# pbluc/avrecode-ms

Hardware: AMD Instinct MI355X
Metric: H.264 bytes/s recompressed (CABAC re-encode of recorded bin streams, bit-exact vs CPU) (higher is better)
Workload: dtype u32

## Files before the change

avrecode-ms_amd/__init__.py:

```python
from __future__ import annotations

import contextlib
import ctypes
import os
import shutil
import subprocess
import sys
from ctypes import POINTER, c_char_p, c_float, c_int, c_int32, c_size_t, c_uint8, c_uint16, c_uint32, c_uint64, c_void_p

_HERE = os.path.dirname(os.path.abspath(__file__))
_CSRC = os.path.join(_HERE, "csrc")
LIB_PATH = os.path.join(_HERE, "libavrecode_hip.so")
HOOKS_LIB_PATH = os.path.join(_HERE, "libavrecode_hip_hooks.so")
HEADER_PATH = os.path.join(os.path.dirname(_HERE), "include", "avrecode_ms_amd.h")

KIND_CABAC, KIND_RANGE, KIND_CABAC_CODES, KIND_CABAC8 = 0, 1, 2, 3
KIND_RANGE_KEYS, EST_KEYS = 4, 1026
SEL_BYPASS, SEL_TERMINATE = 1024, 1025
SEL8_BYPASS, SEL8_TERMINATE, MAX_STATES8 = 126, 127, 126
SLICE_OK, SLICE_ZERO_PROB, SLICE_OVERFLOW, SLICE_BAD_RECORD = 0, 1, 2, 3
NOP_CABAC, NOP_RANGE = 1026 << 1, 0
CHUNK_BINS, SORT_BLOCK_BINS = 1024, 4096

_SOURCES = ["avr_kernels.hip", "avr_k1p.hip", "avr_k2p.hip", "avr_est.hip", "avr_api.cpp"]
_DEPS = _SOURCES + ["avr_coder.h", "avr_est.h", "avr_div.h", "avr_internal.h", "avr_k1p.h", "avr_k2p.h", "avr_synth.h", "avr_tables.h"]


class AvrError(RuntimeError):
    """Raised for every negative return code of the C ABI (message = avr_last_error())."""


def build_native(force: bool = False, verbose: bool = False) -> str:
    deps = [os.path.join(_CSRC, d) for d in _DEPS] + [HEADER_PATH]
    if not force and os.path.exists(LIB_PATH) and os.path.exists(HOOKS_LIB_PATH):
        if all(min(os.path.getmtime(LIB_PATH), os.path.getmtime(HOOKS_LIB_PATH)) >= os.path.getmtime(d) for d in deps):
            return LIB_PATH
    hipcc = shutil.which("hipcc") or "/opt/rocm/bin/hipcc"
    if not os.path.exists(hipcc):
        if os.path.exists(LIB_PATH):
            return LIB_PATH
        raise AvrError("hipcc not found and no prebuilt libavrecode_hip.so")
    objdir = os.path.join(_HERE, "build")
    os.makedirs(objdir, exist_ok=True)
    flags = ["--offload-arch=gfx950", "-O3", "-std=c++17", "-fPIC", "-Wall"]
    jobs = []
    for variant, extra in (("", []), (".hooks", ["-DAVR_TEST_HOOKS"])):
        for src in _SOURCES:
            obj = os.path.join(objdir, src + variant + ".o")
            jobs.append((obj, [hipcc] + flags + extra + ["-c", "-o", obj, os.path.join(_CSRC, src)]))
    if verbose:
        for _, cmd in jobs:
            print(" ".join(cmd))
    procs = [subprocess.Popen(cmd) for _, cmd in jobs]
    if any(p.wait() != 0 for p in procs):
        raise AvrError("hipcc failed")
    for variant, path in (("", LIB_PATH), (".hooks", HOOKS_LIB_PATH)):
        objs = [os.path.join(objdir, src + variant + ".o") for src in _SOURCES]
        subprocess.run([hipcc, "--offload-arch=gfx950", "-shared", "-fPIC", "-o", path + ".tmp"] + objs, check=True)
        os.replace(path + ".tmp", path)
    return LIB_PATH


RECODE_PATH = os.path.join(_HERE, "recode")
_HOST = os.path.join(_CSRC, "host")


def build_recode(force: bool = False, verbose: bool = False) -> str:
    deps = [os.path.join(_HOST, f) for f in ("recode_main.cpp", "avr_h264.h", "avr_h264_tables.h", "avr_recode.h", "avr_host.h", "avr_model.h")]
    deps += [HEADER_PATH, LIB_PATH]
    if not force and os.path.exists(RECODE_PATH) and all(os.path.getmtime(RECODE_PATH) >= os.path.getmtime(d) for d in deps):
        return RECODE_PATH
    cxx = shutil.which("g++") or shutil.which("hipcc")
    if not cxx:
        if os.path.exists(RECODE_PATH):
            return RECODE_PATH
        raise AvrError("no C++ compiler and no prebuilt recode binary")
    cmd = [cxx, "-O2", "-pthread", "-std=c++17", "-I" + _CSRC, "-I/opt/rocm/include", "-D__HIP_PLATFORM_AMD__", "-o", RECODE_PATH + ".tmp",
           os.path.join(_HOST, "recode_main.cpp"), "-L" + _HERE, "-lavrecode_hip", "-Wl,-rpath,$ORIGIN"]
    if verbose:
        print(" ".join(cmd))
    subprocess.run(cmd, check=True)
    os.replace(RECODE_PATH + ".tmp", RECODE_PATH)
    return RECODE_PATH


class ChunkPlan(ctypes.Structure):
    _fields_ = [("res_off", c_void_p), ("chunk_base", c_void_p), ("chunk_slice", c_void_p), ("blk_base", c_void_p),
                ("blk_slice", c_void_p), ("dig_off", c_void_p), ("res_total", c_uint64), ("dig_total", c_uint64),
                ("total_chunks", c_uint32), ("total_blocks", c_uint32)]


class ChunkedPart(ctypes.Structure):
    _fields_ = [("rec_off", c_void_p), ("n_bins", c_void_p), ("n_slices", c_size_t), ("init_states", c_void_p),
                ("plan", c_void_p), ("workspace", c_void_p), ("workspace_bytes", c_size_t),
                ("out_off", c_void_p), ("out_len", c_void_p), ("status", c_void_p), ("final_states", c_void_p),
                ("rows_hint", c_uint32), ("counts", c_void_p)]


MAX_PARTS = 8


class SynthConfig(ctypes.Structure):
    _fields_ = [("workload", c_int), ("scale_permille", c_uint32), ("seed", c_uint64),
                ("first_slice", c_uint64), ("n_states", c_uint32)]


_lib = None

_u8p, _u16p, _u32p, _u64p, _i32p = (POINTER(c_uint8), POINTER(c_uint16), POINTER(c_uint32),
                                    POINTER(c_uint64), POINTER(c_int32))
SIGNATURES = {
    "avr_last_error": (c_char_p, []),
    "avr_version": (c_char_p, []),
    "avr_device_count": (c_int, []),
    "avr_cabac_lps_range_table": (_u8p, []),
    "avr_cabac_mlps_state_table": (_u8p, []),
    "avr_batch_create": (c_void_p, [c_int, c_size_t, c_size_t]),
    "avr_batch_destroy": (None, [c_void_p]),
    "avr_batch_reset": (c_int, [c_void_p]),
    "avr_batch_add_slice_cabac": (c_int, [c_void_p, c_void_p, c_size_t, c_void_p, c_size_t]),
    "avr_batch_add_slice_range": (c_int, [c_void_p, c_void_p, c_size_t]),
    "avr_batch_add_slice_codes": (c_int, [c_void_p, c_void_p, c_size_t]),
# ... 4 lines not shown
    "avr_range_resolve_workspace_bytes": (c_size_t, [c_size_t, c_size_t, c_void_p]),
    "avr_range_resolve_device": (c_int, [c_int, c_void_p, c_void_p, c_void_p, c_void_p, c_size_t, c_void_p, c_size_t, c_void_p, c_void_p,
                                         c_void_p, c_void_p, c_size_t, c_void_p, c_void_p]),
    "avr_batch_reserve_slice": (c_int, [c_void_p, c_int, c_size_t, c_void_p, c_size_t, POINTER(c_void_p)]),
    "avr_batch_submit": (c_int, [c_void_p]),
    "avr_batch_wait": (c_int, [c_void_p]),
    "avr_batch_run": (c_int, [c_void_p]),
    "avr_batch_get": (c_int, [c_void_p, c_size_t, POINTER(c_void_p), POINTER(c_size_t), POINTER(c_int)]),
    "avr_batch_get_states": (c_int, [c_void_p, c_size_t, POINTER(c_void_p), POINTER(c_size_t)]),
    "avr_batch_timings": (c_int, [c_void_p, POINTER(c_float)]),
    "avr_batch_run_info": (c_int, [c_void_p, POINTER(ctypes.c_uint32)]),
    "avr_multi_create": (c_void_p, [c_void_p, c_size_t, c_size_t, c_size_t]),
    "avr_multi_destroy": (None, [c_void_p]),
    "avr_multi_add_slice_cabac": (c_int, [c_void_p, c_void_p, c_size_t, c_void_p, c_size_t]),
    "avr_multi_add_slice_range": (c_int, [c_void_p, c_void_p, c_size_t]),
    "avr_multi_add_slice_codes": (c_int, [c_void_p, c_void_p, c_size_t]),
    "avr_multi_add_slice_cabac8": (c_int, [c_void_p, c_void_p, c_size_t, c_void_p, c_size_t]),
    "avr_multi_run": (c_int, [c_void_p]),
    "avr_multi_get": (c_int, [c_void_p, c_size_t, POINTER(c_void_p), POINTER(c_size_t), POINTER(c_int)]),
    "avr_multi_placement": (c_int, [c_void_p, c_size_t]),
    "avr_multi_load": (c_int, [c_void_p, c_void_p]),
    "avr_pack_tiles_device": (c_int, [c_int, c_void_p, c_int, c_size_t, c_void_p, c_void_p, c_void_p, c_void_p, c_size_t,
                                      c_void_p, c_void_p, c_void_p]),
    "avr_pack_tiles8_device": (c_int, [c_int, c_void_p, c_size_t, c_void_p, c_void_p, c_void_p, c_void_p, c_size_t,
                                       c_void_p, c_void_p, c_void_p]),
    "avr_cabac_encode_tiles_device": (c_int, [c_int, c_void_p, c_void_p, c_void_p, c_void_p, c_void_p, c_size_t,
                                              c_void_p, c_size_t, c_void_p, c_void_p, c_void_p, c_void_p, c_void_p]),
    "avr_pack_tiles8_narrow_device": (c_int, [c_int, c_void_p, c_size_t, c_void_p, c_void_p, c_void_p, c_void_p, c_size_t,
                                              c_void_p, c_void_p, c_void_p]),
    "avr_cabac8_encode_tiles_device": (c_int, [c_int, c_void_p, c_void_p, c_void_p, c_void_p, c_void_p, c_size_t,
                                               c_void_p, c_size_t, c_void_p, c_void_p, c_void_p, c_void_p, c_void_p]),
    "avr_range_encode_tiles_device": (c_int, [c_int, c_void_p, c_void_p, c_void_p, c_void_p, c_void_p, c_size_t,
                                              c_void_p, c_void_p, c_void_p, c_void_p]),
    "avr_cabac_chunked_workspace_bytes": (c_size_t, [c_size_t, c_size_t, c_void_p]),
    "avr_cabac_encode_chunked_device": (c_int, [c_int, c_void_p, c_void_p, c_void_p, c_void_p, c_size_t, c_void_p, c_size_t,
                                                c_void_p, c_void_p, c_size_t, c_void_p, c_void_p, c_void_p, c_void_p,
                                                c_void_p]),
    "avr_cabac8_chunked_workspace_bytes": (c_size_t, [c_size_t, c_size_t, c_void_p]),
    "avr_cabac8_encode_chunked_device": (c_int, [c_int, c_void_p, c_void_p, c_void_p, c_void_p, c_size_t, c_void_p, c_size_t,
                                                 c_void_p, c_void_p, c_size_t, c_void_p, c_void_p, c_void_p, c_void_p,
                                                 c_void_p]),
    "avr_cabac_encode_chunked_device_hinted": (c_int, [c_int, c_void_p, c_void_p, c_void_p, c_void_p, c_size_t, c_void_p, c_size_t,
                                                       c_void_p, c_void_p, c_size_t, c_void_p, c_void_p, c_void_p, c_void_p,
                                                       c_void_p, c_uint32, c_void_p]),
    "avr_cabac_encode_chunked_second_pass_device": (c_int, [c_int, c_void_p, c_void_p, c_void_p, c_void_p, c_size_t, c_void_p, c_size_t,
                                                            c_void_p, c_void_p, c_size_t, c_void_p, c_void_p, c_void_p, c_void_p,
                                                            c_void_p]),
    "avr_cabac_encode_tiles_device_hinted": (c_int, [c_int, c_void_p, c_void_p, c_void_p, c_void_p, c_void_p, c_size_t,
                                                     c_void_p, c_size_t, c_void_p, c_void_p, c_void_p, c_void_p, c_void_p,
                                                     c_uint32, c_void_p]),
    "avr_cabac_encode_chunked_device_parts": (c_int, [c_int, c_void_p, c_void_p, c_size_t, c_void_p, c_void_p, c_size_t]),
    "avr_range_chunked_workspace_bytes": (c_size_t, [c_size_t, c_void_p, ctypes.c_uint64]),
    "avr_range_encode_chunked_device": (c_int, [c_int, c_void_p, c_void_p, c_void_p, c_void_p, c_size_t, c_void_p, c_void_p, c_size_t,
                                                c_void_p, c_void_p, ctypes.c_uint64, c_void_p, c_void_p]),
    "avr_cabac_resolve_workspace_bytes": (c_size_t, [c_size_t, c_size_t, c_void_p]),
    "avr_cabac_resolve_device": (c_int, [c_int, c_void_p, c_void_p, c_void_p, c_void_p, c_size_t, c_void_p, c_size_t,
                                         c_void_p, c_void_p, c_size_t, c_void_p, c_void_p, c_void_p]),
    "avr_cabac_resolved_workspace_bytes": (c_size_t, [c_size_t, c_void_p]),
    "avr_cabac_encode_resolved_device": (c_int, [c_int, c_void_p, c_void_p, c_void_p, c_size_t, c_void_p, c_void_p, c_size_t,
                                                 c_void_p, c_void_p, c_void_p, c_void_p]),
    "avr_cabac_encode_codes_device": (c_int, [c_int, c_void_p, c_void_p, c_void_p, c_void_p, c_void_p, c_size_t,
                                              c_void_p, c_void_p, c_void_p, c_void_p]),
    "avr_cabac_encode_slices_device": (c_int, [c_int, c_void_p, c_void_p, c_void_p, c_void_p, c_void_p, c_size_t,
                                               c_void_p, c_size_t, c_void_p, c_void_p, c_void_p, c_void_p, c_void_p]),
    "avr_range_encode_slices_device": (c_int, [c_int, c_void_p, c_void_p, c_void_p, c_void_p, c_void_p, c_size_t,
                                               c_void_p, c_void_p, c_void_p, c_void_p]),
# ... 292 lines not shown
```

avrecode-ms_amd/csrc/avr_api.cpp:

```cpp
#include <hip/hip_runtime.h>

#include <algorithm>
#include <cstdarg>
#include <cstdio>
#include <cstdlib>
#include <cstring>
#include <mutex>
#include <new>
#include <numeric>
#include <string>
#include <thread>
#include <vector>

#include "avr_internal.h"
#include "avr_synth.h"
#include "avr_tables.h"

namespace {

thread_local char g_err[512] = "";

int fail(int code, const char *fmt, ...) {
    va_list ap;
    va_start(ap, fmt);
// ... 138 lines not shown
const Env &env() {
    static const Env e = [] {
        Env v{0, false, false};
        if (const char *p = getenv("AVR_K1_PATH")) v.k1_path = strcmp(p, "chunked") == 0 ? 2 : strcmp(p, "serial") == 0 ? 1 : 0;
        v.no_dense = getenv("AVR_NO_DENSE") != nullptr;
        v.no_hint = getenv("AVR_BATCH_NO_HINT") != nullptr;
        return v;
    }();
    return e;
}
#ifdef AVR_TEST_HOOKS
TestHooks &test_hooks() { static TestHooks h{}; return h; }
#endif
}

extern "C" {

#ifdef AVR_TEST_HOOKS
int avr_test_hook_set(const char *name, uint32_t value) {
    avr::TestHooks &h = avr::test_hooks();
    if (!name) return fail(AVR_ERR_INVALID, "null hook name");
    if (!strcmp(name, "k1p_force_retry_every")) h.k1p_force_retry_every = value;
    else if (!strcmp(name, "census_stride")) h.census_stride = value;
    else if (!strcmp(name, "chain_lanes")) h.chain_lanes = value;
    else if (!strcmp(name, "k1_form_ref")) h.k1_form_ref = value;
    else if (!strcmp(name, "k1_emit_lds")) h.k1_emit_lds = value;
    else if (!strcmp(name, "k1_path")) h.k1_path = value;
    else if (!strcmp(name, "no_dense")) h.no_dense = value;
    else if (!strcmp(name, "no_hint")) h.no_hint = value;
    else if (!strcmp(name, "k2p_seg_len")) h.k2p_seg_len = value;
    else if (!strcmp(name, "local_waves")) h.local_waves = value;
    else if (!strcmp(name, "k2p_wave")) h.k2p_wave = value;
    else if (!strcmp(name, "k1p_keep_retry")) h.k1p_keep_retry = value;
    else if (!strcmp(name, "k1_waves")) h.k1_waves = value;
    else if (!strcmp(name, "k1_fwd")) h.k1_fwd = value;
    else if (!strcmp(name, "k1_words8")) h.k1_words8 = value;
    else if (!strcmp(name, "chain_nsegs")) h.chain_nsegs = value;
    else if (!strcmp(name, "chain_whole")) h.chain_whole = value;
    else if (!strcmp(name, "chain_segments")) h.chain_segments = value;
    else if (!strcmp(name, "chain_force_redo")) h.chain_force_redo = value;
    else if (!strcmp(name, "reset")) h = avr::TestHooks{};
    else return fail(AVR_ERR_INVALID, "unknown test hook %s", name);
    return AVR_OK;
}
#endif

const char *avr_last_error(void) { return g_err; }
const char *avr_version(void) { return "avrecode-ms_amd 0.1 (gfx950)"; }

int avr_device_count(void) {
    int n = 0;
    if (hipGetDeviceCount(&n) != hipSuccess) return 0;
    return n;
}

const uint8_t *avr_cabac_lps_range_table(void) { return kTables.lps_range; }
const uint8_t *avr_cabac_mlps_state_table(void) { return kTables.mlps_state; }


avr_batch *avr_batch_create(int device, size_t max_slices, size_t max_bins) {
    if (max_slices == 0 || max_slices > 0x7fffffffu) { fail(AVR_ERR_INVALID, "max_slices out of range"); return nullptr; }
    if (select_device(device) != AVR_OK) return nullptr;
    avr_batch *b = new (std::nothrow) avr_batch;
    if (!b) { fail(AVR_ERR_NOMEM, "out of host memory"); return nullptr; }
    b->device = device;
    b->max_slices = max_slices;
// ... 269 lines not shown
    return AVR_OK;
}

static int submit_impl(avr_batch *b, bool use_hint) {
    const size_t n = b->n_bins.size();
    const uint32_t n32 = uint32_t(n);
    if (b->kind == AVR_KIND_CABAC_CODES) return submit_codes(b, n32);
    const size_t ns = b->n_states;
    const bool cabac = b->kind == AVR_KIND_CABAC;

    std::vector<uint32_t> order;
    std::vector<uint64_t> tile_off;
    std::vector<uint64_t> &out_off = b->out_off;
    out_off.assign(n + 1, 0);
    plan_tiles(b->n_bins, order, tile_off, b->recs8 ? 16 : 8);
    for (size_t i = 0; i < n; i++) out_off[i + 1] = out_off[i] + ((uint64_t(b->n_bins[i]) + 16 + 7) & ~uint64_t(7));
    const uint64_t total_recs = b->rec_off.back(), total_chunks = tile_off.back(), total_out = out_off.back();
    const size_t n_tiles = tile_off.size() - 1;
    bool chunked = n <= 32768 && b->total_bins / n >= 8192;
    if (avr::k1_path()) chunked = avr::k1_path() == 2;
    b->last_path = chunked;

    int rc;
    if ((b->recs8 ? (rc = b->d_recs8.reserve(total_recs + 16)) : (rc = b->d_recs.reserve(total_recs))) || (!chunked && (rc = b->d_tiles.reserve(total_chunks))) ||
        (rc = b->d_rec_off.reserve(n + 1)) || (rc = b->d_tile_off.reserve(n_tiles + 1)) ||
        (rc = b->d_out_off.reserve(n + 1)) || (rc = b->d_dense_off.reserve(n + 1)) ||
        (rc = b->d_n_bins.reserve(n)) || (rc = b->d_order.reserve(n)) || (rc = b->d_out_len.reserve(n)) ||
        (rc = b->d_status.reserve(n)) || (rc = b->d_out.reserve(total_out)) ||
        (rc = b->h_out_len.reserve(n)) || (rc = b->h_status.reserve(n)) || (rc = b->h_ndense.reserve(16)))
        return rc;
    if (cabac && ((rc = b->d_states.reserve(n * std::max<size_t>(ns, 1))) || (rc = b->d_final.reserve(n * std::max<size_t>(ns, 1))) ||
                  (rc = b->h_final.reserve(n * std::max<size_t>(ns, 1)))))
        return rc;
    const size_t n_chunks_max = size_t(b->total_bins / AVR_CHUNK_BINS) + n + 1, n_blks_max = size_t(b->total_bins / AVR_SORT_BLOCK_BINS) + n + 1;
    const size_t n_groups = b->group_first.size();
    if ((rc = b->h_plan.reserve(64 * 16 + (n + 1) * 64 + (n_tiles + 1) * 8 + (chunked ? (n_chunks_max + n_blks_max) * 4 : 0) +
                                (b->keys ? (n_chunks_max + n + n_groups + 3) * 4 + 256 : 0)))) return rc;
    if (b->keys && (rc = b->d_keys.reserve(total_recs))) return rc;

    hipStream_t s = b->stream;
    b->plan_used = 0;
    const avr::DenseHint hint{use_hint ? std::min<uint32_t>(b->dense_hint, uint32_t(ns)) : 0u, b->h_ndense.p, b->h_ndense.p + 1};
    b->hint_used = hint.rows;
    b->h_ndense.p[0] = b->h_ndense.p[1] = 0;
    if (b->recs8) {
        b->hint_used = 0;
        b->h_ndense.p[0] = uint32_t(ns);
    }
    AVR_HIP(hipEventRecord(b->ev[0], s));
    if (b->recs8) AVR_HIP(hipMemcpyAsync(b->d_recs8.p, b->h_recs.p, total_recs, hipMemcpyHostToDevice, s));
    else AVR_HIP(hipMemcpyAsync(b->keys ? b->d_keys.p : b->d_recs.p, b->h_recs.p, total_recs * sizeof(uint16_t), hipMemcpyHostToDevice, s));
    AVR_STAGE(b->d_rec_off.p, b->rec_off.data(), n + 1);
    AVR_STAGE(b->d_out_off.p, out_off.data(), n + 1);
    AVR_STAGE(b->d_n_bins.p, b->n_bins.data(), n);
    if (!chunked) {
        AVR_STAGE(b->d_tile_off.p, tile_off.data(), n_tiles + 1);
        AVR_STAGE(b->d_order.p, order.data(), n);
    }
    if (cabac && ns) AVR_HIP(hipMemcpyAsync(b->d_states.p, b->h_states.p, n * ns, hipMemcpyHostToDevice, s));
    AVR_HIP(hipEventRecord(b->ev[1], s));
    AVR_HIP(hipMemsetAsync(b->d_status.p, 0, n * sizeof(int32_t), s));
    if (b->keys && (rc = resolve_keys(b, n32))) return rc;
    if (chunked && !cabac) {
        std::vector<uint32_t> chunk_base(n + 1, 0), chunk_slice;
        for (size_t i = 0; i < n; i++) {
            const uint32_t nc = uint32_t(std::max<uint64_t>(1, (uint64_t(b->n_bins[i]) + AVR_CHUNK_BINS - 1) / AVR_CHUNK_BINS));
            chunk_base[i + 1] = chunk_base[i] + nc;
            chunk_slice.insert(chunk_slice.end(), nc, uint32_t(i));
        }
        const size_t ws = avr::k2p_workspace_bytes(n, chunk_base.back(), total_out);
        if ((rc = b->d_chunk_base.reserve(n + 1)) || (rc = b->d_chunk_slice.reserve(chunk_slice.size())) || (rc = b->d_workspace.reserve(ws + 256)))
            return rc;
        AVR_STAGE(b->d_chunk_base.p, chunk_base.data(), n + 1);
        AVR_STAGE(b->d_chunk_slice.p, chunk_slice.data(), chunk_slice.size());
        AVR_HIP(hipEventRecord(b->ev[2], s));
        uint8_t *wsp = reinterpret_cast<uint8_t *>((reinterpret_cast<uintptr_t>(b->d_workspace.p) + 255) & ~uintptr_t(255));
        AVR_HIP(avr::launch_k2p(s, b->d_recs.p, b->d_rec_off.p, b->d_n_bins.p, n32, b->d_chunk_base.p, b->d_chunk_slice.p,
                                chunk_base.back(), total_out, wsp, b->d_out.p, b->d_out_off.p, b->d_out_len.p, b->d_status.p));
    } else if (chunked) {
        std::vector<uint64_t> res_off(n + 1, 0), dig_off(n + 1, 0);
        std::vector<uint32_t> chunk_base(n + 1, 0), blk_base(n + 1, 0), chunk_slice, blk_slice;
        for (size_t i = 0; i < n; i++) {
            const uint64_t nb = b->n_bins[i];
            res_off[i + 1] = res_off[i] + ((nb + 15) & ~uint64_t(15)) + 16;
            dig_off[i + 1] = dig_off[i] + nb / 2 + 8;
            const uint32_t nc = uint32_t(std::max<uint64_t>(1, (nb + AVR_CHUNK_BINS - 1) / AVR_CHUNK_BINS));
            const uint32_t nk = uint32_t(std::max<uint64_t>(1, (nb + AVR_SORT_BLOCK_BINS - 1) / AVR_SORT_BLOCK_BINS));
            chunk_base[i + 1] = chunk_base[i] + nc;
            blk_base[i + 1] = blk_base[i] + nk;
            chunk_slice.insert(chunk_slice.end(), nc, uint32_t(i));
            blk_slice.insert(blk_slice.end(), nk, uint32_t(i));
        }
        if ((rc = b->d_res_off.reserve(n + 1)) || (rc = b->d_dig_off.reserve(n + 1)) || (rc = b->d_chunk_base.reserve(n + 1)) ||
            (rc = b->d_blk_base.reserve(n + 1)) || (rc = b->d_chunk_slice.reserve(chunk_slice.size())) ||
            (rc = b->d_blk_slice.reserve(blk_slice.size())))
            return rc;
        avr_chunk_plan plan{b->d_res_off.p, b->d_chunk_base.p, b->d_chunk_slice.p, b->d_blk_base.p, b->d_blk_slice.p, b->d_dig_off.p,
                            res_off.back(), dig_off.back(), chunk_base.back(), blk_base.back()};
        const size_t ws = avr::k1p_workspace_bytes(n, uint32_t(ns), &plan);
        if ((rc = b->d_workspace.reserve(ws + 256))) return rc;
        b->plan = plan;
        AVR_STAGE(b->d_res_off.p, res_off.data(), n + 1);
        AVR_STAGE(b->d_dig_off.p, dig_off.data(), n + 1);
        AVR_STAGE(b->d_chunk_base.p, chunk_base.data(), n + 1);
        AVR_STAGE(b->d_blk_base.p, blk_base.data(), n + 1);
        AVR_STAGE(b->d_chunk_slice.p, chunk_slice.data(), chunk_slice.size());
        AVR_STAGE(b->d_blk_slice.p, blk_slice.data(), blk_slice.size());
        AVR_HIP(hipEventRecord(b->ev[2], s));
        uint8_t *wsp = reinterpret_cast<uint8_t *>((reinterpret_cast<uintptr_t>(b->d_workspace.p) + 255) & ~uintptr_t(255));
        if (b->recs8)
            AVR_HIP(avr::launch_k1p8(s, b->d_recs8.p, b->d_rec_off.p, b->d_n_bins.p, n32, b->d_states.p, uint32_t(ns), &plan, wsp,
                                     b->d_out.p, b->d_out_off.p, b->d_out_len.p, b->d_status.p, b->d_final.p));
        else
            AVR_HIP(avr::launch_k1p(s, b->d_recs.p, b->d_rec_off.p, b->d_n_bins.p, n32, b->d_states.p, uint32_t(ns), &plan, wsp,
                                    b->d_out.p, b->d_out_off.p, b->d_out_len.p, b->d_status.p, b->d_final.p, &hint));
    } else {
        if (b->recs8)
            AVR_HIP(avr::launch_pack_tiles8_narrow(s, uint32_t(ns), b->d_recs8.p, b->d_rec_off.p, b->d_n_bins.p, b->d_order.p, n32,
                                                   b->d_tile_off.p, b->d_tiles.p, b->d_status.p));
        else
            AVR_HIP(avr::launch_pack_tiles(s, b->kind, uint32_t(ns), b->d_recs.p, b->d_rec_off.p, b->d_n_bins.p, b->d_order.p, n32,
                                           b->d_tile_off.p, b->d_tiles.p, b->d_status.p));
        AVR_HIP(hipEventRecord(b->ev[2], s));
        if (b->recs8)
            AVR_HIP(avr::launch_cabac8_encode(s, b->d_tiles.p, b->d_tile_off.p, b->d_n_bins.p, b->d_order.p, n32, b->d_states.p,
                                              uint32_t(ns), b->d_out.p, b->d_out_off.p, b->d_out_len.p, b->d_status.p, b->d_final.p));
        else if (cabac)
            AVR_HIP(avr::launch_cabac_encode(true, s, b->d_tiles.p, b->d_tile_off.p, b->d_n_bins.p, b->d_order.p, n32, b->d_states.p,
                                             uint32_t(ns), b->d_out.p, b->d_out_off.p, b->d_out_len.p, b->d_status.p, b->d_final.p,
                                             AVR_SLICE_OK, true, &hint));
        else
// ... 329 lines not shown
                                   uint8_t *out, const uint64_t *out_off, uint32_t *out_len, int32_t *status, uint8_t *final_states) {
    if (int rc = check_common(tile_off, n_bins, out_off, n_slices)) return rc;
    if (n_states > AVR_MAX_STATES8)
        return fail(AVR_ERR_INVALID, "n_states %zu > %d: one-byte records name at most %d contexts", n_states, AVR_MAX_STATES8, AVR_MAX_STATES8);
    if (n_slices && (!tiles || !out || !out_len || !status || (n_states && !init_states))) return fail(AVR_ERR_INVALID, "null device pointer");
    if (reinterpret_cast<uintptr_t>(tiles) & 15) return fail(AVR_ERR_INVALID, "tiles is not 16-byte aligned");
    if (int rc = select_device(device)) return rc;
    AVR_HIP(avr::launch_cabac8_encode(static_cast<hipStream_t>(stream), tiles, tile_off, n_bins, order, uint32_t(n_slices), init_states,
                                      uint32_t(n_states), out, out_off, out_len, status, final_states));
    return AVR_OK;
}

int avr_cabac_encode_tiles_device(int device, void *stream, const void *tiles, const uint64_t *tile_off, const uint32_t *n_bins,
                                  const uint32_t *order, size_t n_slices, const uint8_t *init_states, size_t n_states,
                                  uint8_t *out, const uint64_t *out_off, uint32_t *out_len, int32_t *status, uint8_t *final_states) {
    if (int rc = check_common(tile_off, n_bins, out_off, n_slices)) return rc;
    if (n_states > AVR_MAX_STATES) return fail(AVR_ERR_INVALID, "n_states %zu > %d", n_states, AVR_MAX_STATES);
    if (int rc = select_device(device)) return rc;
    AVR_HIP(avr::launch_cabac_encode(true, static_cast<hipStream_t>(stream), tiles, tile_off, n_bins, order, uint32_t(n_slices),
                                     init_states, uint32_t(n_states), out, out_off, out_len, status, final_states));
    return AVR_OK;
}

int avr_range_encode_tiles_device(int device, void *stream, const void *tiles, const uint64_t *tile_off, const uint32_t *n_bins,
                                  const uint32_t *order, size_t n_slices, uint8_t *out, const uint64_t *out_off,
                                  uint32_t *out_len, int32_t *status) {
    if (int rc = check_common(tile_off, n_bins, out_off, n_slices)) return rc;
    if (int rc = select_device(device)) return rc;
    AVR_HIP(avr::launch_range_encode(true, static_cast<hipStream_t>(stream), tiles, tile_off, n_bins, order, uint32_t(n_slices),
                                     out, out_off, out_len, status));
    return AVR_OK;
}

size_t avr_cabac_chunked_workspace_bytes(size_t n_slices, size_t n_states, const avr_chunk_plan *plan) {
    if (!plan || n_states > AVR_MAX_STATES) return 0;
    return avr::k1p_workspace_bytes(n_slices, uint32_t(n_states), plan);
}

int avr_cabac_encode_chunked_device(int device, void *stream, const uint16_t *recs, const uint64_t *rec_off, const uint32_t *n_bins,
                                    size_t n_slices, const uint8_t *init_states, size_t n_states, const avr_chunk_plan *plan,
                                    void *workspace, size_t workspace_bytes, uint8_t *out, const uint64_t *out_off,
                                    uint32_t *out_len, int32_t *status, uint8_t *final_states) {
    if (int rc = check_common(rec_off, n_bins, out_off, n_slices)) return rc;
    if (n_states > AVR_MAX_STATES) return fail(AVR_ERR_INVALID, "n_states %zu > %d", n_states, AVR_MAX_STATES);
    if (!plan || (n_slices && (!plan->res_off || !plan->chunk_base || !plan->chunk_slice || !plan->blk_base || !plan->blk_slice ||
                               !plan->dig_off || !workspace || !status)))
        return fail(AVR_ERR_INVALID, "null plan pointer");
    if (workspace_bytes < avr::k1p_workspace_bytes(n_slices, uint32_t(n_states), plan))
        return fail(AVR_ERR_CAPACITY, "workspace of %zu bytes is smaller than avr_cabac_chunked_workspace_bytes()", workspace_bytes);
    if (int rc = select_device(device)) return rc;
    AVR_HIP(avr::launch_k1p(static_cast<hipStream_t>(stream), recs, rec_off, n_bins, uint32_t(n_slices), init_states,
                            uint32_t(n_states), plan, workspace, out, out_off, out_len, status, final_states));
    return AVR_OK;
}

size_t avr_cabac8_chunked_workspace_bytes(size_t n_slices, size_t n_states, const avr_chunk_plan *plan) {
    if (!plan || n_states > AVR_MAX_STATES8) return 0;
    return avr::k1p_workspace_bytes(n_slices, uint32_t(n_states), plan);
}

int avr_cabac8_encode_chunked_device(int device, void *stream, const uint8_t *recs8, const uint64_t *rec_off, const uint32_t *n_bins,
                                     size_t n_slices, const uint8_t *init_states, size_t n_states, const avr_chunk_plan *plan,
                                     void *workspace, size_t workspace_bytes, uint8_t *out, const uint64_t *out_off,
                                     uint32_t *out_len, int32_t *status, uint8_t *final_states) {
    if (int rc = check_common(rec_off, n_bins, out_off, n_slices)) return rc;
    if (int rc = check_recs8(recs8, rec_off, n_states)) return rc;
    if (n_slices && (!recs8 || !out || !out_len || (n_states && !init_states))) return fail(AVR_ERR_INVALID, "null device pointer");
    if (!plan || (n_slices && (!plan->res_off || !plan->chunk_base || !plan->chunk_slice || !plan->dig_off || !workspace || !status)))
        return fail(AVR_ERR_INVALID, "null plan pointer");
    if (workspace_bytes < avr::k1p_workspace_bytes(n_slices, uint32_t(n_states), plan))
        return fail(AVR_ERR_CAPACITY, "workspace of %zu bytes is smaller than avr_cabac8_chunked_workspace_bytes()", workspace_bytes);
    if (int rc = select_device(device)) return rc;
    AVR_HIP(avr::launch_k1p8(static_cast<hipStream_t>(stream), recs8, rec_off, n_bins, uint32_t(n_slices), init_states,
                             uint32_t(n_states), plan, workspace, out, out_off, out_len, status, final_states));
    return AVR_OK;
}

static int check_chunked(const uint64_t *rec_off, const uint32_t *n_bins, const uint64_t *out_off, size_t n_slices, size_t n_states,
                         const avr_chunk_plan *plan, void *workspace, size_t workspace_bytes, const int32_t *status) {
    if (int rc = check_common(rec_off, n_bins, out_off, n_slices)) return rc;
    if (n_states > AVR_MAX_STATES) return fail(AVR_ERR_INVALID, "n_states %zu > %d", n_states, AVR_MAX_STATES);
    if (!plan || (n_slices && (!plan->res_off || !plan->chunk_base || !plan->chunk_slice || !plan->blk_base || !plan->blk_slice ||
                               !plan->dig_off || !workspace || !status)))
        return fail(AVR_ERR_INVALID, "null plan pointer");
    if (workspace_bytes < avr::k1p_workspace_bytes(n_slices, uint32_t(n_states), plan))
        return fail(AVR_ERR_CAPACITY, "workspace of %zu bytes is smaller than avr_cabac_chunked_workspace_bytes()", workspace_bytes);
    return AVR_OK;
}

int avr_cabac_encode_chunked_device_hinted(int device, void *stream, const uint16_t *recs, const uint64_t *rec_off, const uint32_t *n_bins,
                                           size_t n_slices, const uint8_t *init_states, size_t n_states, const avr_chunk_plan *plan,
                                           void *workspace, size_t workspace_bytes, uint8_t *out, const uint64_t *out_off,
                                           uint32_t *out_len, int32_t *status, uint8_t *final_states, uint32_t rows_hint, uint32_t *counts) {
    if (!counts) return fail(AVR_ERR_INVALID, "null counts");
    if (int rc = check_chunked(rec_off, n_bins, out_off, n_slices, n_states, plan, workspace, workspace_bytes, status)) return rc;
    if (int rc = select_device(device)) return rc;
    counts[0] = counts[1] = 0;
    if (n_slices == 0) return AVR_OK;
    const avr::DenseHint hint{std::min<uint32_t>(rows_hint, uint32_t(n_states)), counts, counts + 1};
    AVR_HIP(avr::launch_k1p(static_cast<hipStream_t>(stream), recs, rec_off, n_bins, uint32_t(n_slices), init_states,
                            uint32_t(n_states), plan, workspace, out, out_off, out_len, status, final_states, &hint));
    return AVR_OK;
}

int avr_cabac_encode_chunked_second_pass_device(int device, void *stream, const uint16_t *recs, const uint64_t *rec_off, const uint32_t *n_bins,
                                                size_t n_slices, const uint8_t *init_states, size_t n_states, const avr_chunk_plan *plan,
                                                void *workspace, size_t workspace_bytes, uint8_t *out, const uint64_t *out_off,
                                                uint32_t *out_len, int32_t *status, uint8_t *final_states) {
    if (int rc = check_chunked(rec_off, n_bins, out_off, n_slices, n_states, plan, workspace, workspace_bytes, status)) return rc;
    if (int rc = select_device(device)) return rc;
    if (n_slices == 0) return AVR_OK;
    AVR_HIP(avr::launch_k1p_retry(static_cast<hipStream_t>(stream), recs, rec_off, n_bins, uint32_t(n_slices), init_states,
                                  uint32_t(n_states), plan, workspace, out, out_off, out_len, status, final_states));
    return AVR_OK;
}

int avr_cabac_encode_tiles_device_hinted(int device, void *stream, const void *tiles, const uint64_t *tile_off, const uint32_t *n_bins,
// ... 58 lines not shown

int avr_cabac_encode_chunked_device_parts(int device, void *stream, const uint16_t *recs, size_t n_states, uint8_t *out,
                                          const avr_chunked_part *parts, size_t n_parts) {
    if (!parts || n_parts == 0 || n_parts > AVR_MAX_PARTS) return fail(AVR_ERR_INVALID, "1 .. %d parts", AVR_MAX_PARTS);
    for (size_t i = 0; i < n_parts; i++) {
        const avr_chunked_part &q = parts[i];
        if (!q.counts) return fail(AVR_ERR_INVALID, "part %zu: null counts", i);
        if (int rc = check_chunked(q.rec_off, q.n_bins, q.out_off, q.n_slices, n_states, q.plan, q.workspace, q.workspace_bytes, q.status)) return rc;
    }
    if (int rc = select_device(device)) return rc;
    hipStream_t main = static_cast<hipStream_t>(stream);
    PartStreams *ps = nullptr;
    if (n_parts > 1) {
        AVR_HIP(part_streams(main, &ps));
        AVR_HIP(hipEventRecord(ps->fork, main));
    }
    for (size_t i = 0; i < n_parts; i++) {
        const avr_chunked_part &q = parts[i];
        hipStream_t s = i == 0 ? main : ps->side[i - 1];
        if (i) AVR_HIP(hipStreamWaitEvent(s, ps->fork, 0));
        q.counts[0] = q.counts[1] = 0;
        if (q.n_slices) {
            const avr::DenseHint hint{std::min<uint32_t>(q.rows_hint, uint32_t(n_states)), q.counts, q.counts + 1, uint32_t(n_parts)};
            AVR_HIP(avr::launch_k1p(s, recs, q.rec_off, q.n_bins, uint32_t(q.n_slices), q.init_states, uint32_t(n_states), q.plan,
                                    q.workspace, out, q.out_off, q.out_len, q.status, q.final_states, &hint));
        }
        if (i) AVR_HIP(hipEventRecord(ps->done[i - 1], s));
    }
    for (size_t i = 1; i < n_parts; i++) AVR_HIP(hipStreamWaitEvent(main, ps->done[i - 1], 0));
    return AVR_OK;
}

size_t avr_range_chunked_workspace_bytes(size_t n_slices, const avr_chunk_plan *plan, uint64_t out_total) {
    if (!plan) return 0;
    return avr::k2p_workspace_bytes(n_slices, plan->total_chunks, out_total);
}

int avr_range_encode_chunked_device(int device, void *stream, const uint16_t *recs, const uint64_t *rec_off, const uint32_t *n_bins,
                                    size_t n_slices, const avr_chunk_plan *plan, void *workspace, size_t workspace_bytes,
                                    uint8_t *out, const uint64_t *out_off, uint64_t out_total, uint32_t *out_len, int32_t *status) {
    if (int rc = check_common(rec_off, n_bins, out_off, n_slices)) return rc;
    if (!plan || (n_slices && (!plan->chunk_base || !plan->chunk_slice || !workspace || !status || !out || !out_len)))
        return fail(AVR_ERR_INVALID, "null plan / workspace / output pointer");
    if (workspace_bytes < avr::k2p_workspace_bytes(n_slices, plan->total_chunks, out_total))
        return fail(AVR_ERR_CAPACITY, "workspace of %zu bytes is smaller than avr_range_chunked_workspace_bytes()", workspace_bytes);
    if (int rc = select_device(device)) return rc;
    AVR_HIP(avr::launch_k2p(static_cast<hipStream_t>(stream), recs, rec_off, n_bins, uint32_t(n_slices), plan->chunk_base,
                            plan->chunk_slice, plan->total_chunks, out_total, workspace, out, out_off, out_len, status));
    return AVR_OK;
}

size_t avr_range_resolve_workspace_bytes(size_t n_slices, size_t n_groups, const avr_chunk_plan *plan) {
    if (!plan) return 0;
    return avr::est_workspace_bytes(n_slices, n_groups, plan->total_chunks);
}

int avr_range_resolve_device(int device, void *stream, const uint16_t *keys, const uint64_t *rec_off, const uint32_t *n_bins,
                             size_t n_slices, const uint32_t *group_first, size_t n_groups, const uint8_t *est_in, uint8_t *est_out,
                             const avr_chunk_plan *plan, void *workspace, size_t workspace_bytes, uint16_t *recs_out, int32_t *status) {
    if (int rc = check_common(rec_off, n_bins, keys, n_slices)) return rc;
    if (n_groups > 0x7fffffffu) return fail(AVR_ERR_INVALID, "n_groups out of range");
    if (n_slices && (n_groups == 0 || n_groups > n_slices))
        return fail(AVR_ERR_INVALID, "n_groups %zu: a batch of %zu slices has between 1 and %zu groups", n_groups, n_slices, n_slices);
    if (n_slices && (!group_first || !recs_out || !status)) return fail(AVR_ERR_INVALID, "null device pointer");
    if (!plan || (n_slices && (!plan->chunk_base || !plan->chunk_slice))) return fail(AVR_ERR_INVALID, "null plan pointer");
    if (n_slices && !workspace) return fail(AVR_ERR_INVALID, "null workspace");
    if (workspace_bytes < avr::est_workspace_bytes(n_slices, n_groups, plan->total_chunks))
        return fail(AVR_ERR_INVALID, "workspace of %zu bytes is smaller than avr_range_resolve_workspace_bytes()", workspace_bytes);
    if (n_slices && recs_out == keys) return fail(AVR_ERR_INVALID, "recs_out must not alias keys");
    if ((reinterpret_cast<uintptr_t>(keys) | reinterpret_cast<uintptr_t>(recs_out)) & 15)
        return fail(AVR_ERR_INVALID, "keys / recs_out not 16-byte aligned");
    if ((reinterpret_cast<uintptr_t>(est_in) | reinterpret_cast<uintptr_t>(est_out)) & 1)
        return fail(AVR_ERR_INVALID, "est_in / est_out not 2-byte aligned");
    if (reinterpret_cast<uintptr_t>(workspace) & 255) return fail(AVR_ERR_INVALID, "workspace not 256-byte aligned");
    if (int rc = select_device(device)) return rc;
    AVR_HIP(avr::launch_est_resolve(static_cast<hipStream_t>(stream), keys, rec_off, n_bins, uint32_t(n_slices), group_first,
                                    uint32_t(n_groups), est_in, est_out, plan->chunk_base, plan->chunk_slice, plan->total_chunks,
                                    workspace, recs_out, status));
    return AVR_OK;
}

static int check_plan(const avr_chunk_plan *plan, size_t n_slices, bool need_blocks) {
    if (!plan || (n_slices && (!plan->res_off || !plan->chunk_base || !plan->chunk_slice || !plan->dig_off ||
                               (need_blocks && (!plan->blk_base || !plan->blk_slice)))))
        return fail(AVR_ERR_INVALID, "null plan pointer");
    return AVR_OK;
}

size_t avr_cabac_resolve_workspace_bytes(size_t n_slices, size_t n_states, const avr_chunk_plan *plan) {
    if (!plan || n_states > AVR_MAX_STATES) return 0;
    return avr::k1p_resolve_workspace_bytes(n_slices, uint32_t(n_states), plan);
}

int avr_cabac_resolve_device(int device, void *stream, const uint16_t *recs, const uint64_t *rec_off, const uint32_t *n_bins,
                             size_t n_slices, const uint8_t *init_states, size_t n_states, const avr_chunk_plan *plan,
                             void *workspace, size_t workspace_bytes, uint8_t *codes, int32_t *status, uint8_t *final_states) {
    if (int rc = check_common(rec_off, n_bins, codes, n_slices)) return rc;
    if (n_states > AVR_MAX_STATES) return fail(AVR_ERR_INVALID, "n_states %zu > %d", n_states, AVR_MAX_STATES);
    if (int rc = check_plan(plan, n_slices, true)) return rc;
    if (n_slices && (!workspace || !status)) return fail(AVR_ERR_INVALID, "null workspace / status");
    if (workspace_bytes < avr::k1p_resolve_workspace_bytes(n_slices, uint32_t(n_states), plan))
        return fail(AVR_ERR_CAPACITY, "workspace smaller than avr_cabac_resolve_workspace_bytes()");
    if (int rc = select_device(device)) return rc;
    AVR_HIP(avr::launch_k1p_resolve(static_cast<hipStream_t>(stream), recs, rec_off, n_bins, uint32_t(n_slices), init_states,
                                    uint32_t(n_states), plan, workspace, codes, status, final_states));
    return AVR_OK;
}

size_t avr_cabac_resolved_workspace_bytes(size_t n_slices, const avr_chunk_plan *plan) {
    return plan ? avr::k1p_code_workspace_bytes(n_slices, plan) : 0;
}

int avr_cabac_encode_resolved_device(int device, void *stream, const uint8_t *codes, const uint32_t *n_bins, size_t n_slices,
                                     const avr_chunk_plan *plan, void *workspace, size_t workspace_bytes, uint8_t *out,
                                     const uint64_t *out_off, uint32_t *out_len, int32_t *status) {
    if (int rc = check_common(codes, n_bins, out_off, n_slices)) return rc;
    if (int rc = check_plan(plan, n_slices, false)) return rc;
    if (n_slices && (!workspace || !status)) return fail(AVR_ERR_INVALID, "null workspace / status");
    if (workspace_bytes < avr::k1p_code_workspace_bytes(n_slices, plan))
        return fail(AVR_ERR_CAPACITY, "workspace smaller than avr_cabac_resolved_workspace_bytes()");
    if (int rc = select_device(device)) return rc;
    AVR_HIP(avr::launch_k1p_code(static_cast<hipStream_t>(stream), codes, n_bins, uint32_t(n_slices), plan, workspace, out, out_off,
                                 out_len, status));
    return AVR_OK;
}

int avr_cabac_encode_codes_device(int device, void *stream, const uint8_t *codes, const uint64_t *res_off, const uint32_t *n_bins,
                                  const uint32_t *order, size_t n_slices, uint8_t *out, const uint64_t *out_off,
                                  uint32_t *out_len, int32_t *status) {
    if (int rc = check_common(codes, n_bins, out_off, n_slices)) return rc;
    if (n_slices && (!res_off || !status || !out_len)) return fail(AVR_ERR_INVALID, "null device pointer");
    if (int rc = select_device(device)) return rc;
    AVR_HIP(avr::launch_cabac_encode_codes(static_cast<hipStream_t>(stream), codes, res_off, n_bins, order, uint32_t(n_slices), out,
                                           out_off, out_len, status));
    return AVR_OK;
}

int avr_cabac_encode_slices_device(int device, void *stream, const uint16_t *recs, const uint64_t *rec_off, const uint32_t *n_bins,
                                   const uint32_t *order, size_t n_slices, const uint8_t *init_states, size_t n_states,
                                   uint8_t *out, const uint64_t *out_off, uint32_t *out_len, int32_t *status, uint8_t *final_states) {
    if (int rc = check_common(rec_off, n_bins, out_off, n_slices)) return rc;
    if (n_states > AVR_MAX_STATES) return fail(AVR_ERR_INVALID, "n_states %zu > %d", n_states, AVR_MAX_STATES);
    if (int rc = select_device(device)) return rc;
// ... 132 lines not shown
```

avrecode-ms_amd/csrc/avr_internal.h:

```cpp
#pragma once
#include <hip/hip_runtime.h>
#include <stdint.h>

#include "../../include/avrecode_ms_amd.h"

#define AVR_NOP_CABAC2  (AVR_NOP_CABAC | (AVR_NOP_CABAC << 16))
#define AVR_SLICE_RETRY_SERIAL 100
#define AVR_SLICE_RETRY_CENSUS 101
#define AVR_SLICE_DONE         102

namespace avr {

struct Env { int k1_path; bool no_dense, no_hint; };
const Env &env();
struct TestHooks {
    uint32_t k1p_force_retry_every;
    uint32_t census_stride;
    uint32_t chain_lanes;
    uint32_t k1_form_ref;
    uint32_t k1_emit_lds;
    uint32_t k1_path, no_dense, no_hint;
    uint32_t chain_segments;
    uint32_t chain_whole;
    uint32_t chain_force_redo;
    uint32_t k2p_seg_len;
    uint32_t local_waves;
    uint32_t chain_nsegs;
    uint32_t k1_fwd;
    uint32_t k1_words8;
    uint32_t k1_waves;
    uint32_t k2p_wave;
    uint32_t k1p_keep_retry;
};
#ifdef AVR_TEST_HOOKS
TestHooks &test_hooks();
#else
inline const TestHooks &test_hooks() { static const TestHooks none{}; return none; }
#endif
inline int k1_path() { return test_hooks().k1_path ? int(test_hooks().k1_path) : env().k1_path; }
inline bool no_dense() { return test_hooks().no_dense || env().no_dense; }
inline bool no_hint() { return test_hooks().no_hint || env().no_hint; }

struct DenseHint { uint32_t rows; uint32_t *host_count; uint32_t *host_retry; uint32_t sharing = 0; };

void forget_stream(hipStream_t s);
void forget_part_streams(hipStream_t s);

hipError_t launch_cabac_encode(bool tiled, hipStream_t s, const void *recs, const uint64_t *off,
                               const uint32_t *n_bins, const uint32_t *order, uint32_t n_slices,
                               const uint8_t *init_states, uint32_t n_states, uint8_t *out,
                               const uint64_t *out_off, uint32_t *out_len, int32_t *status,
                               uint8_t *final_states, int32_t want_status = AVR_SLICE_OK, bool dense = true,
                               const DenseHint *hint = nullptr);
hipError_t launch_densemap(hipStream_t s, const uint32_t *used, uint16_t *table, uint16_t *index, uint32_t *n_dense);
hipError_t launch_range_encode(bool tiled, hipStream_t s, const void *recs, const uint64_t *off,
                               const uint32_t *n_bins, const uint32_t *order, uint32_t n_slices,
                               uint8_t *out, const uint64_t *out_off, uint32_t *out_len,
                               int32_t *status);
hipError_t launch_pack_tiles(hipStream_t s, int kind, uint32_t n_states, const uint16_t *recs,
                             const uint64_t *rec_off, const uint32_t *n_bins, const uint32_t *order,
                             uint32_t n_slices, const uint64_t *tile_off, void *tiles, int32_t *status);
hipError_t launch_synth_count(hipStream_t s, int workload, uint32_t scale, uint64_t seed,
                              uint64_t first_slice, int kind, uint32_t n_slices, uint32_t *n_bins);
hipError_t launch_synth_tiles(hipStream_t s, int workload, uint32_t scale, uint64_t seed,
                              uint64_t first_slice, int kind, uint32_t n_slices, const uint32_t *order,
                              const uint64_t *tile_off, void *tiles, uint8_t *init_states,
                              uint32_t n_states);

hipError_t launch_pack_tiles8(hipStream_t s, uint32_t n_states, const uint8_t *recs8, const uint64_t *rec_off, const uint32_t *n_bins,
                              const uint32_t *order, uint32_t n_slices, const uint64_t *tile_off, void *tiles, int32_t *status);
hipError_t launch_pack_tiles8_narrow(hipStream_t s, uint32_t n_states, const uint8_t *recs8, const uint64_t *rec_off, const uint32_t *n_bins,
                                     const uint32_t *order, uint32_t n_slices, const uint64_t *tile_off, void *tiles, int32_t *status);
hipError_t launch_cabac8_encode(hipStream_t s, const void *tiles, const uint64_t *tile_off, const uint32_t *n_bins, const uint32_t *order,
                                uint32_t n_slices, const uint8_t *init_states, uint32_t n_states, uint8_t *out, const uint64_t *out_off,
                                uint32_t *out_len, int32_t *status, uint8_t *final_states);
hipError_t launch_context_census(hipStream_t s, const uint16_t *recs, uint64_t n, uint32_t *bitmap);
hipError_t launch_context_remap(hipStream_t s, uint16_t *recs, uint64_t n, const uint16_t *table);
hipError_t launch_states_permute(hipStream_t s, const uint8_t *src, uint32_t n_src, uint8_t *dst, uint32_t n_dst,
                                 const uint16_t *index, uint32_t n_index, uint64_t n_slices, int scatter);
hipError_t launch_compact(hipStream_t s, const uint8_t *out, const uint64_t *out_off, const uint32_t *out_len,
                          const uint64_t *dense_off, uint32_t n_slices, uint8_t *dense);

size_t k1p_workspace_bytes(size_t n_slices, uint32_t n_states, const avr_chunk_plan *pl);
hipError_t launch_k1p(hipStream_t s, const uint16_t *recs, const uint64_t *rec_off, const uint32_t *n_bins,
                      uint32_t n_slices, const uint8_t *init_states, uint32_t n_states, const avr_chunk_plan *pl,
                      void *workspace, uint8_t *out, const uint64_t *out_off, uint32_t *out_len, int32_t *status,
                      uint8_t *final_states, const DenseHint *hint = nullptr);
hipError_t launch_k1p_retry(hipStream_t s, const uint16_t *recs, const uint64_t *rec_off, const uint32_t *n_bins,
                            uint32_t n_slices, const uint8_t *init_states, uint32_t n_states, const avr_chunk_plan *pl,
                            void *workspace, uint8_t *out, const uint64_t *out_off, uint32_t *out_len, int32_t *status,
                            uint8_t *final_states);
hipError_t launch_k1p8(hipStream_t s, const uint8_t *recs8, const uint64_t *rec_off, const uint32_t *n_bins,
                       uint32_t n_slices, const uint8_t *init_states, uint32_t n_states, const avr_chunk_plan *pl,
                       void *workspace, uint8_t *out, const uint64_t *out_off, uint32_t *out_len, int32_t *status,
                       uint8_t *final_states);
size_t k1p_resolve_workspace_bytes(size_t n_slices, uint32_t n_states, const avr_chunk_plan *pl);
hipError_t launch_k1p_resolve(hipStream_t s, const uint16_t *recs, const uint64_t *rec_off, const uint32_t *n_bins,
                              uint32_t n_slices, const uint8_t *init_states, uint32_t n_states, const avr_chunk_plan *pl,
                              void *workspace, uint8_t *codes, int32_t *status, uint8_t *final_states);
size_t k1p_code_workspace_bytes(size_t n_slices, const avr_chunk_plan *pl);
hipError_t launch_k1p_code(hipStream_t s, const uint8_t *codes, const uint32_t *n_bins, uint32_t n_slices,
                           const avr_chunk_plan *pl, void *workspace, uint8_t *out, const uint64_t *out_off,
                           uint32_t *out_len, int32_t *status);
hipError_t launch_cabac_encode_codes(hipStream_t s, const uint8_t *codes, const uint64_t *res_off, const uint32_t *n_bins,
                                     const uint32_t *order, uint32_t n_slices, uint8_t *out, const uint64_t *out_off,
                                     uint32_t *out_len, int32_t *status, int32_t want_status = AVR_SLICE_OK);
size_t k2p_workspace_bytes(size_t n_slices, uint32_t total_chunks, uint64_t out_total);
hipError_t launch_k2p(hipStream_t s, const uint16_t *recs, const uint64_t *rec_off, const uint32_t *n_bins, uint32_t n_slices,
                      const uint32_t *chunk_base, const uint32_t *chunk_slice, uint32_t total_chunks, uint64_t out_total,
                      void *workspace, uint8_t *out, const uint64_t *out_off, uint32_t *out_len, int32_t *status);
size_t est_workspace_bytes(size_t n_slices, size_t n_groups, uint32_t total_chunks);
hipError_t launch_est_resolve(hipStream_t s, const uint16_t *keys, const uint64_t *rec_off, const uint32_t *n_bins, uint32_t n_slices,
                              const uint32_t *group_first, uint32_t n_groups, const uint8_t *est_in, uint8_t *est_out,
                              const uint32_t *chunk_base, const uint32_t *chunk_slice, uint32_t total_chunks, void *workspace,
                              uint16_t *recs_out, int32_t *status);
// ... 6 lines not shown
```

avrecode-ms_amd/csrc/avr_k1p.h:

```cpp
#pragma once
#include <stdint.h>

#if defined(__HIPCC__)
#define AVR_HD __host__ __device__ inline
#else
#define AVR_HD inline
#endif

namespace avr {
namespace k1p {

#if defined(__HIP_DEVICE_COMPILE__)
#define AVR_PIN2(a, b) asm volatile("" : "+v"(a), "+v"(b))
#else
#define AVR_PIN2(a, b) ((void)0)
#endif

constexpr uint32_t kChunk = 1024;
constexpr uint32_t kNone = 0xffffffffu;
constexpr uint32_t kMaxStretch = 16 * kChunk;
constexpr uint32_t kCodeBypass = 252;
constexpr uint32_t kCodePad = 252;

struct alignas(16) U4 { uint32_t x, y, z, w; };

AVR_HD int clz32(uint32_t x) {
#if defined(__HIP_DEVICE_COMPILE__)
    return __clz(x);
#else
    return x ? __builtin_clz(x) : 32;
#endif
}

AVR_HD uint32_t code_sym(uint32_t c) { return ((c >> 1) ^ c) & 1u; }
AVR_HD bool code_is_bypass(uint32_t c) { return (c >> 1) == 126u; }
AVR_HD bool code_is_boundary(uint32_t c) { return code_sym(c) && !code_is_bypass(c); }
AVR_HD uint32_t code_terminate(uint32_t b) { return 255u - b; }
AVR_HD uint32_t code_context(uint32_t s, uint32_t bin) { return s >= 126 ? 255u - ((bin ^ s) & 1u) : (s << 1) | bin; }

AVR_HD uint32_t post_lps_range(uint32_t row, uint32_t q, uint32_t *shift) {
    const uint32_t rl = (row >> (8 * q)) & 0xffu;
    const uint32_t sh = uint32_t(clz32(rl)) - 23;
    *shift = sh;
    return rl << sh;
}

struct CodeEntry { uint32_t row, meta; };
AVR_HD CodeEntry code_entry(uint32_t c, const uint32_t *rows ) {
    if (code_is_bypass(c)) return CodeEntry{0u, 0x100u | ((c & 1u) << 1)};
    return CodeEntry{rows[c >> 2], code_sym(c) * 3u};
}
// ... 21 lines not shown
    *R = x << sh;
    return sh + (e.meta >> 8);
}

struct alignas(16) CodeEntryC { uint32_t row, side, k, adj; };
AVR_HD CodeEntryC code_entry_c(const CodeEntry &e) {
    const uint32_t sym = e.meta & 1u, adds = (e.meta >> 1) & 1u, byp = e.meta >> 8;
    return CodeEntryC{e.row, sym ? ~0u : 0u, adds ? (byp ? 1u : 2u) : 0u, byp - 23u};
}
AVR_HD uint32_t step_range_c(const CodeEntryC &e, uint32_t *R, uint32_t *v) {
    const uint32_t rl = lps_range(e.row, *R);
    const uint32_t rm = *R - rl;
    const uint32_t x = (rl & e.side) | (rm & ~e.side);
    const uint32_t lz = uint32_t(clz32_nz(x));
    *v = mul24(rm, e.k);
    *R = x << (lz - 23);
    return lz + e.adj;
}


struct Stretch {
    uint32_t first;
    uint32_t end;
    uint32_t t_exit[4];
    uint16_t r_exit[4];
    uint8_t exit_q;
    uint8_t too_long;
    uint8_t pad[2];
};

struct LinearCodes {
    const uint8_t *p;
    AVR_HD U4 load16(uint32_t i) const { return *reinterpret_cast<const U4 *>(p + i); }
    AVR_HD uint32_t byte(uint32_t i) const { return p[i]; }
};

template <class Src, class F>
AVR_HD void for_codes_in(const Src &src, uint32_t from, uint32_t n, F &&f) {
    for (uint32_t base = from & ~15u; base < n; base += 16) {
        const U4 v = src.load16(base);
        uint32_t w0 = v.x, w1 = v.y, w2 = v.z, w3 = v.w;
#if defined(__HIP_DEVICE_COMPILE__)
#pragma unroll 1
#endif
        for (uint32_t k = 0; k < 4; k++) {
            const uint32_t d = w0;
            w0 = w1; w1 = w2; w2 = w3;
            const uint32_t i = base + 4 * k;
            if (i + 0 - from < n - from && f(i + 0, d & 0xffu)) return;
            if (i + 1 - from < n - from && f(i + 1, (d >> 8) & 0xffu)) return;
            if (i + 2 - from < n - from && f(i + 2, (d >> 16) & 0xffu)) return;
            if (i + 3 - from < n - from && f(i + 3, d >> 24)) return;
        }
    }
}
template <class F>
AVR_HD void for_codes(const uint8_t *res, uint32_t from, uint32_t n, F &&f) { for_codes_in(LinearCodes{res}, from, n, f); }

template <class G, class G4>
AVR_HD void for_codes_all(const uint8_t *res, uint32_t from, uint32_t to, G &&g, G4 &&g4) {
    if (from >= to) return;
    auto group16 = [&](const U4 &v) {
        uint32_t w0 = v.x, w1 = v.y, w2 = v.z, w3 = v.w;
#if defined(__HIP_DEVICE_COMPILE__)
#pragma unroll 1
#endif
// ... 1 lines not shown
            const uint32_t d = w0;
            w0 = w1; w1 = w2; w2 = w3;
            g4(d);
        }
    };
    const uint32_t head_end = ((from + 15) & ~15u) < to ? ((from + 15) & ~15u) : to;
    for_codes(res, from, head_end, [&](uint32_t, uint32_t c) { g(c); return false; });
    uint32_t base = head_end;
    for (; (base & 63) && base + 16 <= to; base += 16) group16(*reinterpret_cast<const U4 *>(res + base));
    if (base + 64 <= to) {
        const U4 *p = reinterpret_cast<const U4 *>(res + base);
        U4 v0 = p[0], v1 = p[1], v2 = p[2], v3 = p[3];
        for (; base + 64 <= to; base += 64) {
            const U4 *q = reinterpret_cast<const U4 *>(res + (base + 128 <= to ? base + 64 : base));
            const U4 n0 = q[0], n1 = q[1], n2 = q[2], n3 = q[3];
            group16(v0); group16(v1); group16(v2); group16(v3);
            v0 = n0; v1 = n1; v2 = n2; v3 = n3;
        }
    }
    for (; base + 16 <= to; base += 16) group16(*reinterpret_cast<const U4 *>(res + base));
    if (base < to) for_codes(res, base, to, [&](uint32_t, uint32_t c) { g(c); return false; });
}

AVR_HD void code_entries4(const CodeEntry *codes, uint32_t d, CodeEntry e[4]) {
    e[0] = codes[d & 0xffu]; e[1] = codes[(d >> 8) & 0xffu]; e[2] = codes[(d >> 16) & 0xffu]; e[3] = codes[d >> 24];
    AVR_PIN2(e[0].row, e[0].meta); AVR_PIN2(e[1].row, e[1].meta); AVR_PIN2(e[2].row, e[2].meta); AVR_PIN2(e[3].row, e[3].meta);
}
AVR_HD void code_entries4(const CodeEntryC *codes, uint32_t d, CodeEntryC e[4]) {
    e[0] = codes[d & 0xffu]; e[1] = codes[(d >> 8) & 0xffu]; e[2] = codes[(d >> 16) & 0xffu]; e[3] = codes[d >> 24];
    AVR_PIN2(e[0].row, e[0].side); AVR_PIN2(e[1].row, e[1].side); AVR_PIN2(e[2].row, e[2].side); AVR_PIN2(e[3].row, e[3].side);
}

AVR_HD void b1_stretch(const uint8_t *res, uint32_t n, uint32_t chunk, const CodeEntry *codes, uint32_t max_stretch,
                       Stretch *o) {
    const uint32_t lo = chunk * kChunk, limit = lo + kChunk;
    uint32_t R[4], T[4] = {0, 0, 0, 0};
    uint32_t i;
    o->too_long = 0;
    o->exit_q = 0;
    o->pad[0] = o->pad[1] = 0;
    if (chunk == 0) {
        o->first = 0;
        R[0] = R[1] = R[2] = R[3] = 510;
        i = 0;
    } else {
        uint32_t f = kNone;
        const uint32_t hi = limit < n ? limit : n;
        for_codes(res, lo, hi, [&](uint32_t idx, uint32_t c) { if (code_is_boundary(c)) { f = idx; return true; } return false; });
        if (f == kNone) {
            o->first = kNone; o->end = 0;
            for (int q = 0; q < 4; q++) { o->t_exit[q] = 0; o->r_exit[q] = 0; }
            return;
        }
        o->first = f;
        const uint32_t row = codes[res[f]].row;
        for (uint32_t q = 0; q < 4; q++) { uint32_t sh; R[q] = post_lps_range(row, q, &sh); }
        i = f + 1;
    }
    bool closed = false;
    auto merged = [&]() { return R[0] == R[1] && R[1] == R[2] && R[2] == R[3]; };
    auto code_by_code = [&](uint32_t stop) {
        if (i >= stop) return;
        uint32_t i_next = stop;
        for_codes(res, i, stop, [&](uint32_t idx, uint32_t c) {
            if (merged()) { i_next = idx; return true; }
            const bool closing = idx >= limit && code_is_boundary(c);
            if (closing)
                for (uint32_t q = 0; q < 4; q++) o->exit_q |= uint8_t(((R[q] >> 6) & 3) << (2 * q));
// ... 115 lines not shown
    };
    auto digits = [&]() {
        while (sp >= 15) {
            const uint32_t d = uint32_t(L2 >> (sp + 1));
            L2 &= (uint64_t(2) << sp) - 1;
            put(d);
            sp -= 16;
        }
    };
    auto digits2 = [&]() {
        const int s1 = sp + 1;
        const uint32_t nd = uint32_t(s1 > 0 ? s1 : 0) >> 4, ks = 16 + (uint32_t(s1) & 15u);
        const uint64_t t = L2 >> ks;
        const uint32_t a = nd == 2 ? uint32_t(t >> 16) : uint32_t(t), b = uint32_t(t) & 0xffffu;
        L2 = uint32_t(L2) & (nd ? (1u << ks) - 1 : ~0u);
        sp -= int(16 * nd);
        if constexpr (staged) { S.push2(nd, a, b); j += nd; S.look(g0 + j); }
        else { if (nd) put(a); if (nd == 2) put(b); }
    };
    const uint32_t to = st.end;
    if (from < to) {
        auto four = [&](uint32_t d) {
            CodeEntryC e[4];
            code_entries4(codes, d, e);
            bin_e(e[0]); bin_e(e[1]); bin_e(e[2]); bin_e(e[3]);
            digits2();
        };
        auto group16 = [&](const U4 &v) { four(v.x); four(v.y); four(v.z); four(v.w); };
        const uint32_t head_end = ((from + 15) & ~15u) < to ? ((from + 15) & ~15u) : to;
        for_codes_in(src, from, head_end, [&](uint32_t, uint32_t c) { bin(c); digits(); return false; });
        uint32_t base = head_end;
        for (; (base & 63) && base + 16 <= to; base += 16) group16(src.load16(base));
        U4 v0{0, 0, 0, 0}, v1 = v0, v2 = v0, v3 = v0;
        if (base + 64 <= to) { v0 = src.load16(base); v1 = src.load16(base + 16); v2 = src.load16(base + 32); v3 = src.load16(base + 48); }
        for (; base + 64 <= to; base += 64) {
            const uint32_t w[16] = {v0.x, v0.y, v0.z, v0.w, v1.x, v1.y, v1.z, v1.w, v2.x, v2.y, v2.z, v2.w, v3.x, v3.y, v3.z, v3.w};
            const uint32_t nb = base + 128 <= to ? base + 64 : base;
            v0 = src.load16(nb); v1 = src.load16(nb + 16); v2 = src.load16(nb + 32); v3 = src.load16(nb + 48);
#if defined(__HIP_DEVICE_COMPILE__)
#pragma unroll 4
#endif
            for (uint32_t k = 0; k < 16; k++) four(w[k]);
        }
        for (; base + 16 <= to; base += 16) group16(src.load16(base));
        if (base < to) for_codes_in(src, base, to, [&](uint32_t, uint32_t c) { bin(c); digits(); return false; });
    }
    if constexpr (staged) S.flush(g0 + j);
    else S.flush();
    if (sp >= 0) {
        S.add(g0 + j, uint32_t(L2 >> (sp + 1)));
        S.add(g0 + j + 1, uint32_t(L2 & ((uint64_t(2) << sp) - 1)) << (15 - sp));
    } else {
        S.add(g0 + j, uint32_t(L2 << (-sp - 1)) );
    }
}

template <class Adder>
AVR_HD void c_stretch(const uint8_t *res, const Stretch &st, const Entry &en, uint32_t chunk,
                      const CodeEntryC *codes, Adder &S) {
    c_stretch_in(LinearCodes{res}, st, en, chunk, codes, S);
}


AVR_HD uint32_t d_finish(uint32_t low, uint32_t range, uint8_t tail[5], uint32_t *carry) {
    for (uint32_t stop = 1u << 30; stop > 0; stop >>= 1) {
        const uint32_t x = (low | stop) & ~(stop - 1);
        if (stop < range && low <= x && x < uint32_t(low + range)) { low = x; break; }
    }
    uint32_t n = 0, cy = 0;
    while (low != 0 && n < 5) {
        if (low >= 0x80000000u) { cy = 1; low -= 0x80000000u; }
// ... 28 lines not shown
```

avrecode-ms_amd/csrc/avr_k1p.hip:

```cpp
#include <hip/hip_runtime.h>

#include <mutex>
#include <stdint.h>
#include <stdlib.h>
#include <type_traits>

#include "avr_coder.h"
#include "avr_internal.h"
#include "avr_k1p.h"
#include "avr_tables.h"

namespace avr {

static __device__ const CabacTables d_tables = make_cabac_tables();

using namespace k1p;

constexpr uint32_t kSortBlock = AVR_SORT_BLOCK_BINS;

struct Plan {
    const uint16_t *recs;
    const uint64_t *rec_off;
    const uint32_t *n_bins;
    const uint64_t *res_off;
    const uint32_t *chunk_base, *chunk_slice;
    const uint32_t *blk_base, *blk_slice;
    const uint64_t *dig_off;
    uint32_t n_states;
    uint32_t ns_full;
    const uint16_t *table;
    const uint16_t *index;
    const uint8_t *recs8;
};
constexpr uint32_t kNotUsed = 0xffffu;

struct TileCodes {
    const uint8_t *base;
    uint32_t chunk0;
    __device__ __forceinline__ size_t at(uint32_t i) const {
        const uint32_t gc = chunk0 + (i >> 10), g = (i >> 4) & 63u;
        return ((size_t(gc >> 6) * 64 + g) * 64 + (gc & 63u)) * 16;
    }
    __device__ __forceinline__ U4 load16(uint32_t i) const { return *reinterpret_cast<const U4 *>(base + at(i)); }
    __device__ __forceinline__ uint32_t byte(uint32_t i) const { return base[at(i) + (i & 15u)]; }
};
__host__ __device__ inline uint64_t tile_codes_bytes(uint32_t total_chunks) { return (uint64_t(total_chunks) + 63) / 64 * 64 * 1024; }


constexpr uint32_t kCensusBlocks = 32;
__global__ __launch_bounds__(256) void k_k1p_census(Plan p, uint32_t total_blocks, const int32_t *status, uint32_t *used, uint32_t stride) {
    __shared__ uint8_t flag[AVR_MAX_STATES];
    __shared__ uint32_t bm[32];
    for (uint32_t k = threadIdx.x; k < AVR_MAX_STATES / 4; k += 256) reinterpret_cast<uint32_t *>(flag)[k] = 0;
    if (threadIdx.x < 32) bm[threadIdx.x] = 0;
    __syncthreads();
    const uint32_t b = blockIdx.x * kCensusBlocks + (threadIdx.x >> 3), t = threadIdx.x & 7, nk = p.ns_full;
    if (b < total_blocks) {
        const uint32_t s = p.blk_slice[b];
        if (status[s] == AVR_SLICE_OK) {
            const uint32_t n = p.n_bins[s], i0 = (b - p.blk_base[s]) * kSortBlock;
            const uint32_t i1 = i0 + kSortBlock < n ? i0 + kSortBlock : n;
            const uint16_t *r = p.recs + p.rec_off[s];
            for (uint32_t l = b % stride; l < kSortBlock / 64; l += stride) {
                const uint32_t i = i0 + l * 64 + t * 8;
                if (i >= i1) continue;
                const uint4 v = *reinterpret_cast<const uint4 *>(r + i);
                const uint32_t w[4] = {v.x, v.y, v.z, v.w};
#pragma unroll
                for (uint32_t j = 0; j < 8; j++) {
                    const uint32_t sel = ((w[j >> 1] >> ((j & 1) * 16)) & 0xffffu) >> 1;
                    if (i + j < i1 && sel < nk) flag[sel] = 1;
                }
            }
        }
    }
    __syncthreads();
// ... 86 lines not shown
template <class SelT, bool R8>
__global__ __launch_bounds__(512) void k_k1p_local(Plan p, uint32_t total_chunks, int32_t *status, uint32_t *lbits,
                                                   uint16_t *lend, uint32_t *n_retry) {
    extern __shared__ uint32_t local_lds[];
    constexpr uint32_t kSelTab = R8 ? 128 : 2048;
    __shared__ SelT sel_tab[kSelTab];
    const uint32_t nk = p.n_states, lane = threadIdx.x & 63, wv = threadIdx.x >> 6;
    const uint32_t cnt_rows = (nk + 5) / 2;
    const uint32_t wave_dwords = (33 + cnt_rows) * 64;
    uint32_t *bits = local_lds + wv * wave_dwords;
    uint32_t *cnt = bits + 33 * 64;
    for (uint32_t sel = threadIdx.x; sel < kSelTab; sel += blockDim.x) {
        uint32_t k;
        if (R8) k = sel < nk ? sel : sel == AVR_SEL8_TERMINATE ? nk : sel == AVR_SEL8_BYPASS ? nk + 1 : nk + 3;
        else if (sel < 1024u) {
            const uint32_t d = p.table[sel];
            k = d < nk ? d : sel < p.ns_full ? nk + 2 : nk + 3;
        } else k = sel == AVR_SEL_TERMINATE ? nk : sel == AVR_SEL_BYPASS ? nk + 1 : nk + 3;
        sel_tab[sel] = SelT((k >> 1) * 256u | (k & 1u) * 16u);
    }
    for (uint32_t i = lane; i < wave_dwords; i += 64) bits[i] = 0;
    __syncthreads();
    const uint32_t gc0 = (blockIdx.x * (blockDim.x >> 6) + wv) * 64, gc = gc0 + lane;
    uint32_t i0 = 0, i1 = 0, n = 0, s = 0;
    bool mine = false;
    const uint16_t *r = p.recs;
    const uint8_t *r8 = p.recs8;
    uint32_t misaligned = 0;
    if (gc < total_chunks) {
        s = p.chunk_slice[gc];
        if (status[s] == AVR_SLICE_OK) {
            mine = true;
            n = p.n_bins[s];
            i0 = (gc - p.chunk_base[s]) * kChunk;
            i1 = i0 + kChunk < n ? i0 + kChunk : n;
            if (i0 > i1) i0 = i1;
            if (R8) {
                const uint64_t off = p.rec_off[s];
                misaligned = uint32_t(off & 15u);
                r8 = p.recs8 + (off & ~uint64_t(15));
            } else {
                r = p.recs + p.rec_off[s];
            }
        }
    }
    uint32_t *my_cnt = cnt + lane;
    uint32_t *my_bits = bits + lane;
    uint8_t *cnt_b = reinterpret_cast<uint8_t *>(my_cnt), *bits_b = reinterpret_cast<uint8_t *>(my_bits);
    auto for_groups = [&](auto &&f) { for_record_groups(r, i0, i1, f); };
    uint32_t high = 0;
    const uint32_t k_pad = nk + 1;
    const uint32_t e_pad = (k_pad >> 1) * 256u | (k_pad & 1u) * 16u;
    auto group8 = [&](uint32_t base, const U4 &v, auto masked, uint32_t e[16], uint32_t bin[16]) {
        const uint32_t w[4] = {v.x, v.y, v.z, v.w};
#pragma unroll
        for (uint32_t j = 0; j < 16; j++) {
            const uint32_t b = (w[j >> 2] >> (8 * (j & 3))) & 0xffu;
            e[j] = sel_tab[b >> 1];
            if (decltype(masked)::value) e[j] = base + j < i1 ? e[j] : e_pad;
            bin[j] = b & 1u;
        }
    };
    if (R8) for_record_groups8(r8, i0, i1, [&](uint32_t base, const U4 &v, auto masked) {
        uint32_t e[16], bin[16];
        group8(base, v, masked, e, bin);
#pragma unroll
        for (uint32_t j = 0; j < 16; j++)
            __hip_atomic_fetch_add(reinterpret_cast<uint32_t *>(cnt_b + (e[j] & ~255u)), 1u << (e[j] & 31u), __ATOMIC_RELAXED,
// ... 79 lines not shown
    }
    {
        uint32_t *dst = lbits + size_t(gc0) * 32;
        const uint32_t lim = gc0 < total_chunks ? (total_chunks - gc0 < 64 ? total_chunks - gc0 : 64) * 32 : 0;
        for (uint32_t f = lane; f < lim; f += 64) dst[f] = bits[64 * (f & 31u) + (f >> 5)];
    }
    if (nk) {
        uint16_t *dst = lend + size_t(gc0) * nk;
        const uint32_t lim = gc0 < total_chunks ? (total_chunks - gc0 < 64 ? total_chunks - gc0 : 64) * nk : 0;
        uint32_t ch = lane / nk, k = lane - ch * nk;
        const uint32_t dch = 64 / nk, dk = 64 - dch * nk;
        for (uint32_t f = lane; f < lim; f += 64) {
            dst[f] = uint16_t(cnt[64 * (k >> 1) + ch] >> (16 * (k & 1u)));
            ch += dch; k += dk;
            if (k >= nk) { k -= nk; ch++; }
        }
    }
}

constexpr uint32_t kChainLanes = 22, kChainWaves = 8;
__global__ __launch_bounds__(64 * kChainWaves) void k_k1p_ctxchain(Plan p, uint32_t n_slices, uint32_t groups, uint32_t chain_lanes, const int32_t *status,
                                                      const uint8_t *tng, const uint32_t *lbits, const uint16_t *lend,
                                                      const uint8_t *init_states, uint8_t *est, uint8_t *final_states) {
    __shared__ uint8_t tn[kTnBytes];
    for (uint32_t i = threadIdx.x; i < kTnBytes / 16; i += 64 * kChainWaves) reinterpret_cast<uint4 *>(tn)[i] = reinterpret_cast<const uint4 *>(tng)[i];
    __syncthreads();
    const uint32_t wave = blockIdx.x * kChainWaves + (threadIdx.x >> 6), lane = threadIdx.x & 63;
    const uint32_t nk = p.n_states, pair = wave * 64 + lane;
    const uint32_t s = groups ? wave / groups : pair / nk, k = groups ? (wave - s * groups) + lane * groups : pair - s * nk;
    if ((groups && lane >= chain_lanes) || s >= n_slices || status[s] != AVR_SLICE_OK || k >= nk) return;
    const uint32_t col = p.index ? p.index[k] : k, row4 = ((nk + 3) >> 2) << 2;
    if (col >= p.ns_full) return;
    uint32_t st = init_states[size_t(s) * p.ns_full + col] & 127u;
    const uint32_t c0 = p.chunk_base[s], nc = (p.n_bins[s] + kChunk - 1) / kChunk;
    const uint16_t *le = lend + size_t(c0) * nk + k;
    const uint32_t *bw_ahead = lbits + size_t(c0) * 32;
    const uint32_t *bw_cur = bw_ahead;
    uint8_t *eo = est + size_t(c0) * row4 + k;
    auto ends = [&]() {
        const uint32_t e1 = le[0], em = le[-1];
        le += nk;
        return make_uint2(k ? em : 0u, e1);
    };
    auto window = [&](const uint32_t *bw, uint32_t pos) {
        const uint32_t wi = (pos >> 5) & 31u;
        return make_uint4(bw[wi], bw[wi + 1], bw[wi + 2], bw[wi + 3]);
    };
    uint2 e0 = ends(), e1 = ends(), e2 = ends(), e3 = ends();
    uint4 w0 = window(bw_ahead, e0.x), w1 = window(bw_ahead + 32, e1.x);
    bw_ahead += 64;
    for (uint32_t c = 0; c < nc; c++) {
        const uint2 e4 = ends();
        const uint4 w2 = window(bw_ahead, e2.x);
        bw_ahead += 32;
        *eo = uint8_t(st);
        eo += row4;
        uint32_t pos = e0.x;
        const uint32_t end = e0.y;
        uint32_t left = (end > pos && st < 126) ? end - pos : 0u;
        const uint32_t sh = pos & 31u;
        auto four = [&](uint32_t avail) {
#pragma unroll
            for (uint32_t i = 0; i < 4; i++) {
                if (i && !__any(left != 0)) break;
                const uint32_t n = left < 8u ? left : 8u;
                uint32_t off = (128u << n) - 128u + (avail & ((1u << n) - 1u));
                asm volatile("" : "+v"(off));
// ... 62 lines not shown
    four(__builtin_amdgcn_alignbit(w0.y, w0.x, sh));
    if (__any(left != 0)) {
        four(__builtin_amdgcn_alignbit(w0.z, w0.y, sh));
        if (__any(left != 0)) {
            pos += 64;
            uint32_t avail = __builtin_amdgcn_alignbit(w0.w, w0.z, sh);
            uint32_t have = 32;
            while (left) {
                if (have == 0) {
                    const uint32_t wi = (pos >> 5) & 31u;
                    avail = __builtin_amdgcn_alignbit(bw_cur[wi + 1], bw_cur[wi], pos & 31u);
                    have = 32;
                }
                const uint32_t n = left < 8u ? left : 8u;
                uint32_t off = (128u << n) - 128u + (avail & ((1u << n) - 1u));
                asm volatile("" : "+v"(off));
#pragma unroll
                for (int q = 0; q < NS; q++) st[q] = tn[(st[q] << n) + off];
                avail >>= 8;
                left -= n; pos += n; have -= 8;
            }
        }
    }
}

struct ChainLane { uint32_t s, k, seg, c_begin, c_end, nc, col; };
__device__ __forceinline__ bool chain_lane(const Plan &p, uint32_t n_slices, uint32_t n_segs, const int32_t *status, ChainLane *o) {
    const uint32_t wave = blockIdx.x * kSegWaves + (threadIdx.x >> 6), lane = threadIdx.x & 63, nk = p.n_states;
    const uint32_t seg = wave % n_segs, pair = (wave / n_segs) * 64 + lane;
    const uint32_t s = pair / nk, k = pair - s * nk;
    if (s >= n_slices || status[s] != AVR_SLICE_OK) return false;
    const uint32_t col = p.index ? p.index[k] : k;
    if (col >= p.ns_full) return false;
    const uint32_t nc = (p.n_bins[s] + kChunk - 1) / kChunk, seg_len = (nc + n_segs - 1) / n_segs;
    const uint32_t c_begin = seg * seg_len < nc ? seg * seg_len : nc, c_end = c_begin + seg_len < nc ? c_begin + seg_len : nc;
    *o = ChainLane{s, k, seg, c_begin, c_end, nc, col};
    return true;
}

__global__ __launch_bounds__(64 * kSegWaves) void k_k1p_chain_seg(Plan p, uint32_t n_slices, uint32_t n_segs, const int32_t *status,
                                                       const uint8_t *tng, const uint32_t *lbits, const uint16_t *lend, uint8_t *est, SegSummary *summ) {
    __shared__ uint8_t tn[kTnBytes];
    for (uint32_t i = threadIdx.x; i < kTnBytes / 16; i += 64 * kSegWaves) reinterpret_cast<uint4 *>(tn)[i] = reinterpret_cast<const uint4 *>(tng)[i];
    __syncthreads();
    ChainLane L;
    if (!chain_lane(p, n_slices, n_segs, status, &L)) return;
    const uint32_t nk = p.n_states, row4 = ((nk + 3) >> 2) << 2, k = L.k;
    const uint32_t c0 = p.chunk_base[L.s] + L.c_begin, n_ch = L.c_end - L.c_begin;
    const uint16_t *le = lend + size_t(c0) * nk + k;
    const uint32_t *bw_ahead = lbits + size_t(c0) * 32, *bw_cur = bw_ahead;
    uint8_t *eo = est + size_t(c0) * row4 + k;
    auto ends = [&]() { const uint32_t e1 = le[0], em = le[-1]; le += nk; return make_uint2(k ? em : 0u, e1); };
    auto window = [&](const uint32_t *bw, uint32_t pos) { const uint32_t wi = (pos >> 5) & 31u; return make_uint4(bw[wi], bw[wi + 1], bw[wi + 2], bw[wi + 3]); };
    uint2 e0 = ends(), e1 = ends(), e2 = ends(), e3 = ends();
    uint4 w0 = window(bw_ahead, e0.x), w1 = window(bw_ahead + 32, e1.x);
    bw_ahead += 64;
    uint32_t st[2] = {124u, 125u};
    uint32_t met_chunk = n_ch, n_bins = 0;
    uint64_t bits0 = 0, bits1 = 0;
    for (uint32_t c = 0; c < n_ch; c++) {
        const uint2 e4 = ends();
        const uint4 w2 = window(bw_ahead, e2.x);
        bw_ahead += 32;
        if (st[0] == st[1]) {
            *eo = uint8_t(st[0]);
            met_chunk = met_chunk < c ? met_chunk : c;
        }
// ... 82 lines not shown
    const uint32_t exit_state = chain_chunks<true>(tn, lbits, lend, est, nk, row4, k, c_slice + L.c_begin, stop, entry);
    if (final_states && (L.c_end == L.nc) && (L.c_begin < L.nc || L.seg == 0))
        final_states[size_t(L.s) * p.ns_full + L.col] = uint8_t(stop < n_ch ? me.exit_state : exit_state);
}

__device__ __forceinline__ CodeEntry device_code_entry(uint32_t c);
__device__ __forceinline__ uint2 device_codes2(uint32_t c);

constexpr uint32_t kStBypass = 128, kStTerminate = 129, kStPad = 130, kStNone = 131, kReplayStates = 132;

typedef uint16_t u16x2 __attribute__((ext_vector_type(2)));
__device__ __forceinline__ uint32_t pk_sub(uint32_t a, uint32_t b) { return __builtin_bit_cast(uint32_t, __builtin_bit_cast(u16x2, a) - __builtin_bit_cast(u16x2, b)); }
__device__ __forceinline__ uint32_t pk_add(uint32_t a, uint32_t b) { return __builtin_bit_cast(uint32_t, __builtin_bit_cast(u16x2, a) + __builtin_bit_cast(u16x2, b)); }
__device__ __forceinline__ uint32_t pk_shl(uint32_t a, uint32_t b) { return __builtin_bit_cast(uint32_t, __builtin_bit_cast(u16x2, a) << __builtin_bit_cast(u16x2, b)); }
__device__ __forceinline__ uint32_t pk_shr8(uint32_t a) { return (a >> 8) & 0x00ff00ffu; }
__device__ __forceinline__ uint32_t step_pair(uint32_t &Rp, uint32_t row, uint32_t rown, uint32_t shrow, bool sym, uint32_t extra) {
    const uint32_t sel = ((Rp >> 6) & 0x00030003u) | 0x0c000c00u;
    const uint32_t rl = __builtin_amdgcn_perm(row, row, sel);
    const uint32_t rm = pk_sub(Rp, rl);
    const uint32_t shm = pk_shr8(rm) ^ 0x00010001u;
    const uint32_t rn = __builtin_amdgcn_perm(rown, rown, sel) | 0x01000100u;
    const uint32_t shl = __builtin_amdgcn_perm(shrow, shrow, sel);
    Rp = sym ? rn : pk_shl(rm, shm);
    return (sym ? shl : shm) + extra;
}

struct B1Walk {
    uint32_t i0, i1, limit, n, max_stretch;
    const uint2 *codes2;
    uint32_t mode, Rp0, Rp1, Tp0, Tp1, T[4], Rm, Tm, end;
    bool merged;
    Stretch o;

    __device__ __forceinline__ void init(uint32_t chunk, uint32_t i0_, uint32_t i1_, uint32_t n_, uint32_t max_stretch_, const uint2 *codes2_) {
        i0 = i0_; i1 = i1_; limit = i0_ + kChunk; n = n_; max_stretch = max_stretch_; codes2 = codes2_;
        mode = 0; Rp0 = Rp1 = 0x01fe01feu; Tp0 = Tp1 = 0; T[0] = T[1] = T[2] = T[3] = 0; Rm = 510; Tm = 0; end = 0;
        merged = false;
        o.first = kNone; o.end = 0; o.exit_q = 0; o.too_long = 0; o.pad[0] = o.pad[1] = 0;
        for (int q = 0; q < 4; q++) { o.t_exit[q] = 0; o.r_exit[q] = 0; }
        if (chunk == 0) { o.first = 0; mode = 2; merged = true; }
    }
    __device__ __forceinline__ void flush_t() {
        T[0] += Tp0 & 0xffffu; T[1] += Tp0 >> 16; T[2] += Tp1 & 0xffffu; T[3] += Tp1 >> 16;
        Tp0 = Tp1 = 0;
    }
    __device__ __forceinline__ bool met() const { return Rp0 == Rp1 && (Rp0 >> 16) == (Rp0 & 0xffffu); }
    __device__ __forceinline__ void one(uint32_t idx, const uint4 &e) {
        const CodeEntry ce{e.x, e.y >> 16};
        const bool boundary = ce.meta & 1u;
        if (mode == 0) {
            if (idx < i1 && boundary) {
                o.first = idx;
                const uint32_t rown = codes2[(e.y >> 8) & 0xffu].x;
                Rp0 = __builtin_amdgcn_perm(rown, rown, 0x0c010c00u) | 0x01000100u;
                Rp1 = __builtin_amdgcn_perm(rown, rown, 0x0c030c02u) | 0x01000100u;
                mode = 1;
            }
        } else if (mode == 1) {
            const bool closing = idx >= limit && boundary;
            if (closing)
                o.exit_q |= uint8_t(((Rp0 >> 6) & 3u) | ((Rp0 >> 22) & 3u) << 2 | ((Rp1 >> 6) & 3u) << 4 | ((Rp1 >> 22) & 3u) << 6);
            const uint2 e2 = codes2[(e.y >> 8) & 0xffu];
            const uint32_t extra = (ce.meta >> 8) * 0x00010001u;
            Tp0 = pk_add(Tp0, step_pair(Rp0, ce.row, e2.x, e2.y, boundary, extra));
            Tp1 = pk_add(Tp1, step_pair(Rp1, ce.row, e2.x, e2.y, boundary, extra));
            if (closing) { end = idx + 1; mode = 3; }
            else if (met()) { Rm = Rp0 & 0xffffu; mode = 2; merged = true; }
        } else if (mode == 2) {
// ... 62 lines not shown
        if (R8) {
            kk = sel < nk ? sel : sel == AVR_SEL8_BYPASS ? nk + 1 : sel == AVR_SEL8_TERMINATE ? nk + 2 : nk + 4;
        } else {
            const uint32_t over = (sel < 1023u ? 1023u : sel > 1027u ? 1027u : sel) - 1023u;
            const uint32_t dense = sel < 1024u ? uint32_t(p.table[sel]) : kNotUsed;
            kk = (dense < nk ? dense : nk) + over;
        }
        sel_off[sel] = ((kk & ~3u) << 6) + (kk & 3u);
    }
    for (uint32_t i = threadIdx.x; i < 2 * kReplayStates; i += blockDim.x) {
        const uint32_t st = i >> 1, bin = i & 1u;
        uint32_t next, code;
        if (st < 128) {
            const uint32_t nx = d_tables.packed[st][1];
            next = ((bin ^ st) & 1u) ? (nx >> 8) & 0xffu : nx & 0xffu;
            code = code_context(st, bin);
        } else {
            next = st;
            code = st == kStBypass ? kCodeBypass | bin : st == kStTerminate ? code_terminate(bin) : kCodePad;
        }
        const CodeEntry ce = device_code_entry(code);
        const CodeEntryC cc = code_entry_c(ce);
        info[i] = make_uint4(ce.row, next | code << 8 | ce.meta << 16, cc.side, cc.adj);
    }
    __syncthreads();
    const uint32_t gc = blockIdx.x * blockDim.x + threadIdx.x;
    if (gc >= total_chunks) return;
    const uint32_t s = p.chunk_slice[gc];
    Stretch o;
    o.first = kNone; o.end = 0; o.exit_q = 0; o.too_long = 0; o.pad[0] = o.pad[1] = 0;
    for (int q = 0; q < 4; q++) { o.t_exit[q] = 0; o.r_exit[q] = 0; }
    if (status[s] != AVR_SLICE_OK) { stretch[gc] = o; return; }
    const uint32_t c = gc - p.chunk_base[s];
    const uint32_t n = p.n_bins[s], i0 = c * kChunk;
    const uint32_t i1 = i0 + kChunk < n ? i0 + kChunk : n;
    {
        const uint32_t nkw = (nk + 3) >> 2;
        const uint32_t *e = est + size_t(gc) * nkw;
        for (uint32_t kw = 0; kw < nkw; kw++) *reinterpret_cast<uint32_t *>(stb + kw * 256) = e[kw];
        const uint32_t pseudo[5] = {kStNone, kStBypass, kStTerminate, kStPad, kStNone};
#pragma unroll
        for (uint32_t j = 0; j < 5; j++) stb[((nk + j) >> 2) * 256 + ((nk + j) & 3)] = uint8_t(pseudo[j]);
    }
    const uint16_t *r = p.recs + p.rec_off[s];
    uint8_t *ro = TILE_CODES ? res + ((size_t(gc >> 6) * 64) * 64 + (gc & 63u)) * 16 : res + p.res_off[s];
    auto put16 = [&](uint32_t i, const U4 &v) {
        if (TILE_CODES) *reinterpret_cast<U4 *>(ro + size_t((i - i0) >> 4) * 1024) = v;
        else *reinterpret_cast<U4 *>(ro + i) = v;
    };
    B1Walk b1;
    b1.init(c, i0, i1, n, max_stretch, codes2);
    auto eight = [&](const U4 &v, uint32_t &c0, uint32_t &c1, uint4 e[8]) {
        const uint32_t w[4] = {v.x, v.y, v.z, v.w};
        uint32_t off[8];
#pragma unroll
        for (uint32_t j = 0; j < 8; j++) off[j] = sel_off[((w[j >> 1] >> ((j & 1) * 16)) >> 1) & 0x7ffu];
#pragma unroll
        for (uint32_t j = 0; j < 8; j++) {
            const uint32_t bin = (w[j >> 1] >> ((j & 1) * 16)) & 1u;
            uint8_t *sp = stb + off[j];
            const uint32_t st = *sp;
            e[j] = info[(st << 1) | bin];
            *sp = uint8_t(e[j].y);
        }
        c0 = __builtin_amdgcn_perm(e[1].y, e[0].y, 0x0c0c0501u) | __builtin_amdgcn_perm(e[3].y, e[2].y, 0x05010c0cu);
        c1 = __builtin_amdgcn_perm(e[5].y, e[4].y, 0x0c0c0501u) | __builtin_amdgcn_perm(e[7].y, e[6].y, 0x05010c0cu);
    };
    if (R8) {
        const uint32_t pad_off = (((nk + 3) & ~3u) << 6) + ((nk + 3) & 3u);
        auto eight8 = [&](uint32_t lo, uint32_t hi, uint32_t base, uint32_t lim, auto masked, uint32_t &c0, uint32_t &c1, uint4 e[8]) {
            uint32_t off[8], bin[8];
#pragma unroll
            for (uint32_t j = 0; j < 8; j++) {
                const uint32_t b = ((j < 4 ? lo : hi) >> (8 * (j & 3))) & 0xffu;
                off[j] = sel_off[b >> 1];
                if (decltype(masked)::value) off[j] = base + j < lim ? off[j] : pad_off;
                bin[j] = b & 1u;
            }
#pragma unroll
            for (uint32_t j = 0; j < 8; j++) {
                uint8_t *sp = stb + off[j];
                const uint32_t st = *sp;
                e[j] = info[(st << 1) | bin[j]];
                *sp = uint8_t(e[j].y);
            }
            c0 = __builtin_amdgcn_perm(e[1].y, e[0].y, 0x0c0c0501u) | __builtin_amdgcn_perm(e[3].y, e[2].y, 0x05010c0cu);
            c1 = __builtin_amdgcn_perm(e[5].y, e[4].y, 0x0c0c0501u) | __builtin_amdgcn_perm(e[7].y, e[6].y, 0x05010c0cu);
        };
        auto sixteen8 = [&](uint32_t base, const U4 &v, auto masked) {
            U4 a;
            uint4 e[8];
            eight8(v.x, v.y, base, i1, masked, a.x, a.y, e); b1.group(base, e);
            eight8(v.z, v.w, base + 8, i1, masked, a.z, a.w, e); b1.group(base + 8, e);
            put16(base, a);
        };
        const uint8_t *r8 = p.recs8 + (p.rec_off[s] & ~uint64_t(15));
        if (i0 < n) {
            for_record_groups8(r8, i0, i1, sixteen8);
            b1.chunk_done();
            for (uint32_t i = i0 + kChunk; b1.mode != 3 && i < n; i += 8) {
                const uint2 v = *reinterpret_cast<const uint2 *>(r8 + i);
                uint32_t c0, c1;
                uint4 e[8];
                eight8(v.x, v.y, i, n, std::true_type{}, c0, c1, e);
                b1.tail(i, e);
            }
        }
        stretch[gc] = b1.finish();
        return;
    }
    uint32_t i = i0;
    if (i0 < n) {
        U4 v0{0, 0, 0, 0}, v1 = v0, v2 = v0, v3 = v0;
        const uint32_t last = i + 32 <= i1 ? i0 + ((i1 - i0) / 32u - 1u) * 32u : i0;
        if (i + 32 <= i1) {
            const U4 *q = reinterpret_cast<const U4 *>(r + i);
            v0 = q[0]; v1 = q[1]; v2 = q[2]; v3 = q[3];
        }
        for (; i + 32 <= i1; i += 32) {
            const U4 *qn = reinterpret_cast<const U4 *>(r + (i + 32 <= last ? i + 32 : last));
            const U4 n0 = qn[0], n1 = qn[1], n2 = qn[2], n3 = qn[3];
            U4 a, b;
            uint4 e[8];
            eight(v0, a.x, a.y, e); b1.group(i, e);
            eight(v1, a.z, a.w, e); b1.group(i + 8, e);
            eight(v2, b.x, b.y, e); b1.group(i + 16, e);
            eight(v3, b.z, b.w, e); b1.group(i + 24, e);
            put16(i, a);
            put16(i + 16, b);
            v0 = n0; v1 = n1; v2 = n2; v3 = n3;
        }
        for (; i < i1; i += 16) {
            const U4 *q = reinterpret_cast<const U4 *>(r + i);
            const U4 nop{AVR_NOP_CABAC2, AVR_NOP_CABAC2, AVR_NOP_CABAC2, AVR_NOP_CABAC2};
            const U4 t0 = q[0], t1 = i + 8 < i1 ? q[1] : nop;
            U4 a;
            uint4 e[8];
            eight(t0, a.x, a.y, e); b1.group(i, e);
            eight(t1, a.z, a.w, e); b1.group(i + 8, e);
            put16(i, a);
        }
        b1.chunk_done();
        for (i = i0 + kChunk; b1.mode != 3 && i < n; i += 8) {
            uint32_t c0, c1;
            uint4 e[8];
            eight(*reinterpret_cast<const U4 *>(r + i), c0, c1, e);
            b1.tail(i, e);
        }
    }
    stretch[gc] = b1.finish();
}


__device__ __forceinline__ CodeEntry device_code_entry(uint32_t c) {
    if (code_is_bypass(c)) return CodeEntry{0u, 0x100u | ((c & 1u) << 1)};
    return CodeEntry{d_tables.packed[2 * (c >> 2)][0], code_sym(c) * 3u};
}

__device__ __forceinline__ uint2 device_codes2(uint32_t c) {
    const uint32_t row = device_code_entry(c).row;
    uint32_t rown = 0, shrow = 0;
    for (uint32_t q = 0; q < 4; q++) {
        const uint32_t rl = (row >> (8 * q)) & 0xffu;
        if (rl) { uint32_t sh; const uint32_t rn = post_lps_range(row, q, &sh); rown |= (rn & 0xffu) << (8 * q); shrow |= sh << (8 * q); }
    }
    return make_uint2(rown, shrow);
}

__global__ __launch_bounds__(256) void k_k1p_b1(Plan p, uint32_t total_chunks, const uint8_t *res,
                                                const int32_t *status, Stretch *st, uint32_t max_stretch, uint8_t *tile) {
    __shared__ uint4 cinfo[256];
    __shared__ uint2 codes2[256];
    {
        const CodeEntry ce = device_code_entry(threadIdx.x);
        const CodeEntryC cc = code_entry_c(ce);
        cinfo[threadIdx.x] = make_uint4(ce.row, threadIdx.x << 8 | ce.meta << 16, cc.side, cc.adj);
        codes2[threadIdx.x] = device_codes2(threadIdx.x);
    }
    __syncthreads();
    const uint32_t gc = blockIdx.x * 256 + threadIdx.x;
    if (gc >= total_chunks) return;
    const uint32_t slice = p.chunk_slice[gc];
    if (status[slice] != AVR_SLICE_OK) { st[gc].first = kNone; st[gc].too_long = 0; return; }
    const uint32_t c = gc - p.chunk_base[slice], n = p.n_bins[slice], i0 = c * kChunk;
    const uint32_t i1 = i0 + kChunk < n ? i0 + kChunk : n;
    const uint8_t *r = res + p.res_off[slice];
    B1Walk b1;
    b1.init(c, i0, i1, n, max_stretch, codes2);
    auto eight = [&](uint32_t lo, uint32_t hi, uint4 e[8]) {
#pragma unroll
        for (uint32_t j = 0; j < 8; j++) e[j] = cinfo[((j < 4 ? lo : hi) >> (8 * (j & 3))) & 0xffu];
    };
    uint8_t *to = tile ? tile + ((size_t(gc >> 6) * 64) * 64 + (gc & 63u)) * 16 : nullptr;
    auto sixteen = [&](uint32_t base, const U4 &v) {
        if (to) *reinterpret_cast<U4 *>(to + size_t((base - i0) >> 4) * 1024) = v;
        uint4 e[8];
        eight(v.x, v.y, e); b1.group(base, e);
        eight(v.z, v.w, e); b1.group(base + 8, e);
    };
    uint32_t i = i0;
    if (i0 < n) {
        U4 v0{0, 0, 0, 0}, v1 = v0, v2 = v0, v3 = v0;
        if (i + 64 <= i1) { const U4 *q = reinterpret_cast<const U4 *>(r + i); v0 = q[0]; v1 = q[1]; v2 = q[2]; v3 = q[3]; }
        for (; i + 64 <= i1; i += 64) {
            const U4 *qn = reinterpret_cast<const U4 *>(r + (i + 128 <= i1 ? i + 64 : i));
            const U4 n0 = qn[0], n1 = qn[1], n2 = qn[2], n3 = qn[3];
            sixteen(i, v0); sixteen(i + 16, v1); sixteen(i + 32, v2); sixteen(i + 48, v3);
            v0 = n0; v1 = n1; v2 = n2; v3 = n3;
        }
        for (; i < i1; i += 16) sixteen(i, *reinterpret_cast<const U4 *>(r + i));
        b1.chunk_done();
        for (i = i0 + kChunk; b1.mode != 3 && i < n; i += 16) {
            const U4 v = *reinterpret_cast<const U4 *>(r + i);
            uint4 e[8];
            eight(v.x, v.y, e); b1.tail(i, e);
            if (b1.mode != 3) { eight(v.z, v.w, e); b1.tail(i + 8, e); }
        }
    }
    st[gc] = b1.finish();
}

constexpr uint32_t kB2Tile = 1024, kB2Seg = 16;

__global__ __launch_bounds__(256) void k_k1p_b2(Plan p, const int32_t *status, const Stretch *st, Entry *en,
                                                SliceTotals *tot, uint32_t *S) {
    __shared__ Stretch tile[kB2Tile];
    __shared__ Entry ent[kB2Tile];
    __shared__ uint8_t xq[kB2Tile], qin[kB2Tile];
    __shared__ uint8_t segmap[256], segin[kB2Tile / kB2Seg];
    __shared__ uint32_t wsum[4];
    __shared__ uint32_t carry[4];
    const uint32_t s = blockIdx.x, t = threadIdx.x, lane = t & 63, w = t >> 6;
    if (status[s] != AVR_SLICE_OK) {
        if (t == 0) { tot[s].t_total = 0; tot[s].r_final = 510; tot[s].bad = 0; tot[s].pad = 0; }
        return;
    }
    const uint32_t c0 = p.chunk_base[s], nc = p.chunk_base[s + 1] - c0;
    if (t == 0) { carry[0] = 0; carry[1] = 0; carry[2] = 510; carry[3] = 0; }
    for (uint32_t base = 0; base < nc; base += kB2Tile) {
        const uint32_t cnt = nc - base < kB2Tile ? nc - base : kB2Tile;
        const uint32_t *src = reinterpret_cast<const uint32_t *>(st + c0 + base);
        uint32_t *dst = reinterpret_cast<uint32_t *>(tile);
        for (uint32_t i = t; i < cnt * (sizeof(Stretch) / 4); i += 256) dst[i] = src[i];
        __syncthreads();
        for (uint32_t c = t; c < kB2Tile; c += 256) xq[c] = c < cnt && tile[c].first != kNone ? tile[c].exit_q : uint8_t(0xE4);
// ... 88 lines not shown
            LdsWord *r = ring + k * 64;
            if (first + k < g0 + 2) { atomicAdd((uint32_t *)&S[first + k], r[0]); k++; }
            else if (a == 0 && left >= 4) { *(uint4 *)(S + first + k) = make_uint4(r[0], r[64], r[128], r[192]); k += 4; }
            else if (last || (a != 0 && left >= 4 - a)) { S[first + k] = r[0]; k++; }
            else break;
        }
        cnt -= k;
        if (k != 0) {
#pragma unroll 1
            for (uint32_t m = 0; m < cnt; m++) ring[m * 64] = ring[(k + m) * 64];
        }
        return cnt;
    }
    __device__ void add(uint32_t i, uint32_t v) { atomicAdd(&S[i], v); }
};

template <bool TILE_CODES>
__global__ __launch_bounds__(256, 7) void k_k1p_c(Plan p, uint32_t total_chunks, const uint8_t *res,
                                                  const Stretch *st, const Entry *en, const SliceTotals *tot,
                                                  uint32_t *S) {
    __shared__ CodeEntryC codes[256];
    __shared__ uint32_t ring[kRing * 256];
    codes[threadIdx.x] = code_entry_c(device_code_entry(threadIdx.x));
    __syncthreads();
    const uint32_t gc = blockIdx.x * 256 + threadIdx.x;
    if (gc >= total_chunks) return;
    const Stretch o = st[gc];
    if (o.first == kNone) return;
    const uint32_t slice = p.chunk_slice[gc];
    if (tot[slice].bad) return;
    DeviceAdder add;
    add.S = S + p.dig_off[slice];
    add.ring = ring + (threadIdx.x >> 6) * (kRing * 64) + (threadIdx.x & 63u);
    if (TILE_CODES) c_stretch_in(TileCodes{res, p.chunk_base[slice]}, o, en[gc], gc - p.chunk_base[slice], codes, add);
    else c_stretch(res + p.res_off[slice], o, en[gc], gc - p.chunk_base[slice], codes, add);
}


constexpr uint32_t kSeg = 33;
constexpr uint32_t kTile = 256 * kSeg;

__global__ __launch_bounds__(256) void k_k1p_d(Plan p, const SliceTotals *tot, const uint32_t *S,
                                               uint8_t *out, const uint64_t *out_off, uint32_t *out_len,
                                               int32_t *status, uint32_t force_retry_every) {
    __shared__ uint32_t dig[kTile];
    __shared__ uint32_t seg_g[256], seg_cin[256];
    __shared__ uint64_t seg_gm[4], seg_pm[4];
    __shared__ uint32_t sh_carry;
    const uint32_t s = blockIdx.x, t = threadIdx.x;
    if (status[s] != AVR_SLICE_OK) { if (t == 0 && status[s] != AVR_SLICE_DONE) out_len[s] = 0; return; }
    const SliceTotals T = tot[s];
    if (T.bad || (force_retry_every && s % force_retry_every == 0)) { if (t == 0) status[s] = AVR_SLICE_RETRY_SERIAL; return; }
    const uint32_t *Ss = S + p.dig_off[s];
    uint8_t *o = out + out_off[s];
    const uint32_t cap = uint32_t(out_off[s + 1] - out_off[s]);
    const uint32_t nd = ref_digits(T.t_total);
    if (t == 0) {
        const uint32_t low = uint32_t((uint64_t(Ss[nd]) << 15) + (Ss[nd + 1] >> 1));
        const uint32_t range = T.r_final << (22 - T.t_total + 16 * nd);
        uint8_t tail[5];
        uint32_t carry;
        const uint32_t n_tail = d_finish(low, range, tail, &carry);
        for (uint32_t k = 0; k < n_tail; k++) {
            if (2 * nd + k < cap) o[2 * nd + k] = tail[k];
        }
        sh_carry = carry;
        out_len[s] = 2 * nd + n_tail;
// ... 24 lines not shown
            if (v == (t >> 6)) recv = (__builtin_bitreverse64(sum ^ a ^ b2) >> (t & 63)) & 1;
            into = uint32_t(((a & b2) | ((a | b2) & ~sum)) >> 63);
        }
        seg_g[t] = c + ((all_ones && recv) ? 1u : 0u);
        __syncthreads();
        const uint32_t n_seg = (cnt + kSeg - 1) / kSeg;
        seg_cin[t] = t + 1 >= n_seg ? carry_in : seg_g[t + 1];
        if (t == 0) sh_carry = seg_g[0];
        __syncthreads();
        if (t < n_seg && seg_cin[t]) {
            uint32_t c2 = seg_cin[t];
            for (uint32_t i = b; i-- > a && c2;) {
                const uint32_t v = dig[i] + c2;
                dig[i] = v & 0xffffu;
                c2 = v >> 16;
            }
            if (c2 != ((all_ones && recv) ? 1u : 0u)) status[s] = AVR_SLICE_RETRY_SERIAL;
        }
        __syncthreads();
        for (uint32_t i = t; i < cnt; i += 256) {
            const uint32_t v = dig[i], at = 2 * (lo + i);
            if (at + 1 < cap) *reinterpret_cast<uint16_t *>(o + at) = uint16_t((v >> 8) | (v << 8));
        }
        carry_in = sh_carry;
        hi = lo;
        __syncthreads();
    }
}

template <bool TILE>
__global__ __launch_bounds__(64) void k_cabac_encode_codes(const uint8_t *codes_in, const uint64_t *res_off, const uint32_t *chunk_base,
                                                           const uint32_t *n_bins, const uint32_t *order, uint32_t n_slices, uint8_t *out,
                                                           const uint64_t *out_off, uint32_t *out_len, int32_t *status,
                                                           int32_t want_status) {
    __shared__ CodeEntry codes[256];
    for (uint32_t c = threadIdx.x; c < 256; c += 64) codes[c] = device_code_entry(c);
    __syncthreads();
    const uint32_t g = blockIdx.x * 64 + threadIdx.x;
    if (g >= n_slices) return;
    const uint32_t slice = order ? order[g] : g;
    if (status[slice] != want_status) {
        if (want_status == AVR_SLICE_OK) out_len[slice] = 0;
        return;
    }
    const uint32_t n = n_bins[slice];
    const uint8_t *res = TILE ? codes_in : codes_in + res_off[slice];
    const TileCodes tiled{codes_in, TILE ? chunk_base[slice] : 0u};
    auto load16 = [&](uint32_t i) { return TILE ? tiled.load16(i) : *reinterpret_cast<const U4 *>(res + i); };
    auto byte = [&](uint32_t i) { return TILE ? tiled.byte(i) : uint32_t(res[i]); };
    const uint64_t o0 = out_off[slice];
    const uint32_t cap = uint32_t(out_off[slice + 1] - o0);
    CabacEncoder e;
    e.init(0x7F800000u, out + o0, cap);
    auto bin = [&](uint32_t c) {
        const CodeEntry ce = codes[c];
        const int norm = 23 - __builtin_clz(e.range);
        const uint32_t q = (e.range >> (norm + 6)) & 3;
        const uint32_t r_tab = ((ce.row >> (8 * q)) & 0xffu) << norm;
        const uint32_t r1 = (ce.meta >> 8) ? e.range >> 1 : r_tab;
        const uint32_t sym = (ce.meta >> 1) & 1u;
        const uint32_t r0 = e.range - r1;
        e.low += sym ? r0 : 0u;
        e.range = sym ? r1 : r0;
        if (e.range < 0x200u) e.emit_digit();
    };
    uint32_t i = 0;
    if (n >= 16) {
        U4 v = load16(0);
        for (; i + 16 <= n; i += 16) {
            const U4 nx = i + 32 <= n ? load16(i + 16) : v;
            uint32_t w0 = v.x, w1 = v.y, w2 = v.z, w3 = v.w;
#pragma unroll 1
            for (uint32_t k = 0; k < 4; k++) {
                const uint32_t d = w0;
                w0 = w1; w1 = w2; w2 = w3;
                bin(d & 0xffu); bin((d >> 8) & 0xffu); bin((d >> 16) & 0xffu); bin(d >> 24);
            }
            v = nx;
        }
    }
// ... 15 lines not shown
static inline ResolveLayout resolve_layout(size_t n_slices, uint32_t ns, const avr_chunk_plan *pl) {
    ResolveLayout L;
    uint64_t at = 0;
    auto take = [&](uint64_t bytes) { const uint64_t o = at; at += up256(bytes); return o; };
    L.lbits = take(uint64_t(pl->total_chunks + 64) * 128);
    L.lend = take(uint64_t(pl->total_chunks + 64) * ns * 2 + 256) + 128;
    L.est = take(uint64_t(pl->total_chunks) * ((ns + 3) / 4) * 4 + 16);
    L.stretch = take(uint64_t(pl->total_chunks) * sizeof(Stretch));
    L.meta = take(256 + 2048 + 2048 + kTnBytes);
    L.summ = take(uint64_t(n_slices) * ns * kMaxChainSegs * sizeof(SegSummary));
    L.total = at;
    return L;
}

static hipError_t tn_table(hipStream_t s, const uint8_t **out) {
    struct Slot { uint8_t *p = nullptr; hipEvent_t ready = nullptr; };
    static Slot slots[16];
    static std::mutex mu;
    int dev = 0;
    hipError_t e = hipGetDevice(&dev);
    if (e != hipSuccess) return e;
    std::lock_guard<std::mutex> lock(mu);
    Slot &x = slots[dev & 15];
    if (!x.p) {
        uint8_t *buf = nullptr;
        if ((e = hipMalloc(reinterpret_cast<void **>(&buf), kTnBytes + 256)) != hipSuccess) return e;
        if ((e = hipEventCreateWithFlags(&x.ready, hipEventDisableTiming)) != hipSuccess) return e;
        hipLaunchKernelGGL(k_k1p_tn, dim3((kTnBytes + 255) / 256), dim3(256), 0, s, buf);
        if ((e = hipEventRecord(x.ready, s)) != hipSuccess) return e;
        x.p = buf;
    }
    *out = x.p;
    return hipStreamWaitEvent(s, x.ready, 0);
}

static hipError_t launch_resolve(hipStream_t s, Plan p, uint32_t n_slices, const uint8_t *init_states,
                                 const avr_chunk_plan *pl, uint8_t *w, uint8_t *res, int32_t *status, uint8_t *final_states,
                                 uint32_t max_stretch, const Stretch **stretch_out, const DenseHint *hint = nullptr,
                                 uint32_t stride = 1, bool second_pass = false, uint32_t *retry_count = nullptr,
                                 bool tile_codes = false, bool r8 = false) {
    const uint32_t ns = p.ns_full;
    const ResolveLayout L = resolve_layout(n_slices, ns, pl);
    uint32_t *lbits = reinterpret_cast<uint32_t *>(w + L.lbits);
    uint16_t *lend = reinterpret_cast<uint16_t *>(w + L.lend);
    uint8_t *est = w + L.est;
    Stretch *stretch = reinterpret_cast<Stretch *>(w + L.stretch);
    if (stretch_out) *stretch_out = stretch;
    uint32_t *used = reinterpret_cast<uint32_t *>(w + L.meta);
    uint32_t *n_dense = used + 32, *n_retry = used + 33;
    uint16_t *table = reinterpret_cast<uint16_t *>(w + L.meta + 256), *index = table + 1024;
    const uint8_t *tn = nullptr;
    p.table = table;
    p.index = index;
    hipError_t e;
    if ((e = hipMemsetAsync(used, 0, 256, s)) != hipSuccess) return e;
    if (final_states && ns && !second_pass &&
        (e = hipMemcpyAsync(final_states, init_states, size_t(n_slices) * ns, hipMemcpyDeviceToDevice, s)) != hipSuccess)
        return e;
    uint32_t n_states = 0;
    if (r8) {
        n_states = ns;
        p.table = nullptr;
        p.index = nullptr;
        if ((e = tn_table(s, &tn)) != hipSuccess) return e;
    } else {
        hipLaunchKernelGGL(k_k1p_census, dim3((pl->total_blocks + kCensusBlocks - 1) / kCensusBlocks), dim3(256), 0, s, p, pl->total_blocks, status, used, stride);
        hipLaunchKernelGGL(k_k1p_densemap, dim3(1), dim3(1024), 0, s, used, table, index, n_dense);
        if ((e = tn_table(s, &tn)) != hipSuccess) return e;
        if (hint && hint->rows) {
            n_states = hint->rows < ns ? hint->rows : ns;
            if (hint->host_count && (e = hipMemcpyAsync(hint->host_count, n_dense, 4, hipMemcpyDeviceToHost, s)) != hipSuccess) return e;
        } else {
            if ((e = hipMemcpyAsync(&n_states, n_dense, 4, hipMemcpyDeviceToHost, s)) != hipSuccess) return e;
            if ((e = hipStreamSynchronize(s)) != hipSuccess) return e;
            if (hint && hint->host_count) *hint->host_count = n_states;
        }
    }
    p.n_states = n_states;
    {
        const uint32_t per_wave = (33 + (n_states + 5) / 2) * 64 * 4;
        const bool narrow = n_states <= 500;
        const uint32_t kLdsPerCu = 160 * 1024, kStatic = r8 ? 128 * 2 : narrow ? 2048 * 2 : 2048 * 4;
        auto local = r8 ? k_k1p_local<uint16_t, true> : narrow ? k_k1p_local<uint16_t, false> : k_k1p_local<uint32_t, false>;
        uint32_t waves = 1, best = 0;
        for (uint32_t w = 1; w <= 8; w++) {
            const uint32_t need = w * per_wave + kStatic;
            if (need > kLdsPerCu) break;
            const uint32_t resident = kLdsPerCu / need * w;
            if (resident > best) { best = resident; waves = w; }
        }
        if (const uint32_t v = test_hooks().local_waves) waves = v;
        uint32_t lds = waves * per_wave;
        if (lds > 60 * 1024) {
            e = hipFuncSetAttribute(reinterpret_cast<const void *>(local), hipFuncAttributeMaxDynamicSharedMemorySize, int(lds));
            if (e != hipSuccess && waves > 1) {
                (void)hipGetLastError();
                waves = per_wave * 2 <= 60 * 1024 ? 2 : 1;
                lds = waves * per_wave;
                e = lds > 60 * 1024 ? hipFuncSetAttribute(reinterpret_cast<const void *>(local), hipFuncAttributeMaxDynamicSharedMemorySize, int(lds))
                                    : hipSuccess;
            }
            if (e != hipSuccess) return e;
        }
        hipLaunchKernelGGL(local, dim3((pl->total_chunks + 64 * waves - 1) / (64 * waves)), dim3(64 * waves), lds, s, p,
                           pl->total_chunks, status, lbits, lend, n_retry);
        if (stride > 1 && !second_pass) {
            if (hint && hint->rows && hint->host_retry) {
                if ((e = hipMemcpyAsync(hint->host_retry, n_retry, 4, hipMemcpyDeviceToHost, s)) != hipSuccess) return e;
            } else if (retry_count) {
                if ((e = hipMemcpyAsync(retry_count, n_retry, 4, hipMemcpyDeviceToHost, s)) != hipSuccess) return e;
                if ((e = hipStreamSynchronize(s)) != hipSuccess) return e;
            }
        }
    }
    if (n_states > 0) {
        uint32_t chain_lanes = uint32_t((uint64_t(n_slices) * n_states + 2047) / 2048);
        chain_lanes = chain_lanes < kChainLanes ? kChainLanes : chain_lanes > 64 ? 64 : chain_lanes;
        if (const uint32_t v = test_hooks().chain_lanes) chain_lanes = v <= 64 ? v : 64;
        const bool packed = chain_lanes == 64;
        const uint32_t groups = packed ? 0u : (n_states + chain_lanes - 1) / chain_lanes;
        const uint32_t whole_waves = packed ? uint32_t((uint64_t(n_slices) * n_states + 63) / 64) : n_slices * groups;
        const dim3 whole((whole_waves + kChainWaves - 1) / kChainWaves), block(64 * kChainWaves);
        const bool few_lanes = uint64_t(n_slices) * n_states <= 49152;
        const uint32_t pair_waves = uint32_t((uint64_t(n_slices) * n_states + 63) / 64);
        uint32_t n_segs = kChainWaveSlots / (pair_waves * (hint && hint->sharing ? hint->sharing : 1u));
        n_segs = n_segs > kMaxChainSegs ? kMaxChainSegs : n_segs;
        const uint64_t by_length = uint64_t(pl->total_chunks) / (uint64_t(n_slices) * 4);
        if (n_segs > by_length) n_segs = uint32_t(by_length);
        if (const uint32_t v = test_hooks().chain_nsegs) n_segs = v < kMaxChainSegs ? v : kMaxChainSegs;
        if (n_segs >= 2 && !test_hooks().chain_whole && (few_lanes || test_hooks().chain_segments)) {
            SegSummary *summ = reinterpret_cast<SegSummary *>(w + L.summ);
            const dim3 seg_grid((pair_waves * n_segs + kSegWaves - 1) / kSegWaves), seg_block(64 * kSegWaves);
            hipLaunchKernelGGL(k_k1p_chain_seg, seg_grid, seg_block, 0, s, p, n_slices, n_segs, status, tn, lbits, lend, est, summ);
            hipLaunchKernelGGL(k_k1p_chain_fix, seg_grid, seg_block, 0, s, p, n_slices, n_segs, status, tn, lbits, lend, init_states, est, summ,
                               final_states, test_hooks().chain_force_redo);
        } else {
            hipLaunchKernelGGL(k_k1p_ctxchain, whole, block, 0, s, p, n_slices, groups, chain_lanes, status, tn, lbits, lend, init_states, est, final_states);
        }
    }
    const uint32_t per_wave = ((n_states + 8) / 4) * 256;
    const uint32_t replay_waves = per_wave * 4 <= 48 * 1024 ? 4 : per_wave * 2 <= 48 * 1024 ? 2 : 1;
    const uint32_t replay_lds = replay_waves * per_wave;
    auto replay = r8 ? k_k1p_replay<true, true> : tile_codes ? k_k1p_replay<true, false> : k_k1p_replay<false, false>;
    if (replay_lds > 48 * 1024) {
        e = hipFuncSetAttribute(reinterpret_cast<const void *>(replay), hipFuncAttributeMaxDynamicSharedMemorySize, int(replay_lds));
        if (e != hipSuccess) return e;
    }
    hipLaunchKernelGGL(replay, dim3((pl->total_chunks + 64 * replay_waves - 1) / (64 * replay_waves)), dim3(64 * replay_waves),
                       replay_lds, s, p, pl->total_chunks, reinterpret_cast<const uint32_t *>(est), res, status, stretch, max_stretch);
    return hipGetLastError();
}

static hipError_t launch_code(hipStream_t s, const Plan &p, uint32_t n_slices, const avr_chunk_plan *pl, uint8_t *w,
                              const uint8_t *res, uint32_t max_stretch, uint8_t *out, const uint64_t *out_off,
                              uint32_t *out_len, int32_t *status, const Stretch *have = nullptr, bool tile_codes = false) {
    Stretch *st_own = reinterpret_cast<Stretch *>(w);        w += up256(uint64_t(pl->total_chunks) * sizeof(Stretch));
    const Stretch *st = have ? have : st_own;
    Entry *en = reinterpret_cast<Entry *>(w);                w += up256(uint64_t(pl->total_chunks) * sizeof(Entry));
    SliceTotals *tot = reinterpret_cast<SliceTotals *>(w);   w += up256(n_slices * sizeof(SliceTotals));
    uint32_t *S = reinterpret_cast<uint32_t *>(w);               w += up256(pl->dig_total * 4 + 16);
    const uint32_t chunk_blocks = (pl->total_chunks + 255) / 256;
    if (!have) {
        uint8_t *tile = w;
        hipLaunchKernelGGL(k_k1p_b1, dim3(chunk_blocks), dim3(256), 0, s, p, pl->total_chunks, res, status, st_own, max_stretch, tile);
        res = tile;
        tile_codes = true;
    }
    hipLaunchKernelGGL(k_k1p_b2, dim3(n_slices), dim3(256), 0, s, p, status, st, en, tot, S);
    if (tile_codes) hipLaunchKernelGGL(k_k1p_c<true>, dim3(chunk_blocks), dim3(256), 0, s, p, pl->total_chunks, res, st, en, tot, S);
    else hipLaunchKernelGGL(k_k1p_c<false>, dim3(chunk_blocks), dim3(256), 0, s, p, pl->total_chunks, res, st, en, tot, S);
    const uint32_t force_retry_every = test_hooks().k1p_force_retry_every;
    hipLaunchKernelGGL(k_k1p_d, dim3(n_slices), dim3(256), 0, s, p, tot, S, out, out_off, out_len, status, force_retry_every);
    return hipGetLastError();
}

hipError_t launch_densemap(hipStream_t s, const uint32_t *used, uint16_t *table, uint16_t *index, uint32_t *n_dense) {
    hipLaunchKernelGGL(k_k1p_densemap, dim3(1), dim3(1024), 0, s, used, table, index, n_dense);
    return hipGetLastError();
}

hipError_t launch_cabac_encode_codes(hipStream_t s, const uint8_t *codes, const uint64_t *res_off, const uint32_t *n_bins,
                                     const uint32_t *order, uint32_t n_slices, uint8_t *out, const uint64_t *out_off,
                                     uint32_t *out_len, int32_t *status, int32_t want_status) {
    if (n_slices == 0) return hipSuccess;
    hipLaunchKernelGGL(k_cabac_encode_codes<false>, dim3((n_slices + 63) / 64), dim3(64), 0, s, codes, res_off, nullptr, n_bins, order,
                       n_slices, out, out_off, out_len, status, want_status);
    return hipGetLastError();
}

static inline uint64_t resolve_ws_bytes(size_t n_slices, uint32_t n_states, const avr_chunk_plan *pl) {
    return resolve_layout(n_slices, n_states, pl).total;
}

size_t k1p_code_workspace_bytes(size_t n_slices, const avr_chunk_plan *pl);
static inline uint64_t codes_bytes(const avr_chunk_plan *pl) {
    const uint64_t tiled = tile_codes_bytes(pl->total_chunks), linear = pl->res_total + 32;
    return tiled > linear ? tiled : linear;
}
size_t k1p_workspace_bytes(size_t n_slices, uint32_t n_states, const avr_chunk_plan *pl) {
    return size_t(up256(codes_bytes(pl)) + resolve_ws_bytes(n_slices, n_states, pl)) + k1p_code_workspace_bytes(n_slices, pl);
}

constexpr uint32_t kK1pCensusStride = 16;

static uint32_t census_stride() {
    return test_hooks().census_stride ? test_hooks().census_stride : kK1pCensusStride;
}

static hipError_t k1p_pass(hipStream_t s, const Plan &p, uint32_t n_slices, const uint8_t *init_states, uint32_t n_states,
                           const avr_chunk_plan *pl, uint8_t *w, uint8_t *res, uint8_t *out, const uint64_t *out_off, uint32_t *out_len,
                           int32_t *status, uint8_t *final_states, const DenseHint *hint, uint32_t stride, bool second_pass,
                           uint32_t *retry_count) {
    const Stretch *st = nullptr;
    hipError_t e = launch_resolve(s, p, n_slices, init_states, pl, w, res, status, final_states, kMaxStretch, &st, hint, stride, second_pass,
                                  retry_count, true);
    if (e != hipSuccess) return e;
    w += resolve_ws_bytes(n_slices, n_states, pl);
    e = launch_code(s, p, n_slices, pl, w, res, kMaxStretch, out, out_off, out_len, status, st, true);
    if (e != hipSuccess || test_hooks().k1p_keep_retry) return e;
    return launch_cabac_encode(false, s, p.recs, p.rec_off, p.n_bins, nullptr, n_slices, init_states, n_states, out, out_off,
                               out_len, status, nullptr, AVR_SLICE_RETRY_SERIAL);
}

static hipError_t k1p_second_pass(hipStream_t s, const Plan &p, uint32_t n_slices, const uint8_t *init_states, uint32_t n_states,
                                  const avr_chunk_plan *pl, uint8_t *w, uint8_t *res, uint8_t *out, const uint64_t *out_off,
                                  uint32_t *out_len, int32_t *status, uint8_t *final_states, bool code) {
    const dim3 grid((n_slices + 255) / 256), block(256);
    hipLaunchKernelGGL(k_k1p_swap, grid, block, 0, s, status, n_slices, AVR_SLICE_OK, AVR_SLICE_DONE, AVR_SLICE_RETRY_CENSUS, AVR_SLICE_OK);
    hipError_t e = code ? k1p_pass(s, p, n_slices, init_states, n_states, pl, w, res, out, out_off, out_len, status, final_states, nullptr, 1,
                                   true, nullptr)
                        : launch_resolve(s, p, n_slices, init_states, pl, w, res, status, final_states, kMaxStretch, nullptr, nullptr, 1, true);
    if (e != hipSuccess) return e;
    hipLaunchKernelGGL(k_k1p_swap, grid, block, 0, s, status, n_slices, AVR_SLICE_DONE, AVR_SLICE_OK, AVR_SLICE_DONE, AVR_SLICE_OK);
    return hipGetLastError();
}

hipError_t launch_k1p(hipStream_t s, const uint16_t *recs, const uint64_t *rec_off, const uint32_t *n_bins,
                      uint32_t n_slices, const uint8_t *init_states, uint32_t n_states, const avr_chunk_plan *pl,
                      void *workspace, uint8_t *out, const uint64_t *out_off, uint32_t *out_len, int32_t *status,
                      uint8_t *final_states, const DenseHint *hint) {
    if (n_slices == 0) return hipSuccess;
    uint8_t *w = static_cast<uint8_t *>(workspace);
    uint8_t *res = w;                                        w += up256(codes_bytes(pl));
    const Plan p{recs, rec_off, n_bins, pl->res_off, pl->chunk_base, pl->chunk_slice, pl->blk_base, pl->blk_slice,
                 pl->dig_off, 0, n_states, nullptr, nullptr};
    const uint32_t stride = census_stride();
    uint32_t retry = 0;
    if (hint && hint->host_retry) *hint->host_retry = 0;
    hipError_t e = k1p_pass(s, p, n_slices, init_states, n_states, pl, w, res, out, out_off, out_len, status, final_states, hint, stride, false,
                            &retry);
    if (e != hipSuccess || !retry) return e;
    return k1p_second_pass(s, p, n_slices, init_states, n_states, pl, w, res, out, out_off, out_len, status, final_states, true);
}

hipError_t launch_k1p_retry(hipStream_t s, const uint16_t *recs, const uint64_t *rec_off, const uint32_t *n_bins,
                            uint32_t n_slices, const uint8_t *init_states, uint32_t n_states, const avr_chunk_plan *pl,
                            void *workspace, uint8_t *out, const uint64_t *out_off, uint32_t *out_len, int32_t *status,
                            uint8_t *final_states) {
    if (n_slices == 0) return hipSuccess;
    uint8_t *w = static_cast<uint8_t *>(workspace);
    uint8_t *res = w;                                        w += up256(codes_bytes(pl));
    const Plan p{recs, rec_off, n_bins, pl->res_off, pl->chunk_base, pl->chunk_slice, pl->blk_base, pl->blk_slice,
                 pl->dig_off, 0, n_states, nullptr, nullptr};
    return k1p_second_pass(s, p, n_slices, init_states, n_states, pl, w, res, out, out_off, out_len, status, final_states, true);
}

size_t k1p_resolve_workspace_bytes(size_t n_slices, uint32_t n_states, const avr_chunk_plan *pl) {
    return size_t(resolve_ws_bytes(n_slices, n_states, pl));
}
hipError_t launch_k1p_resolve(hipStream_t s, const uint16_t *recs, const uint64_t *rec_off, const uint32_t *n_bins,
                              uint32_t n_slices, const uint8_t *init_states, uint32_t n_states, const avr_chunk_plan *pl,
                              void *workspace, uint8_t *codes, int32_t *status, uint8_t *final_states) {
    if (n_slices == 0) return hipSuccess;
    const Plan p{recs, rec_off, n_bins, pl->res_off, pl->chunk_base, pl->chunk_slice, pl->blk_base, pl->blk_slice,
                 pl->dig_off, 0, n_states, nullptr, nullptr};
    uint8_t *w = static_cast<uint8_t *>(workspace);
    const uint32_t stride = census_stride();
    uint32_t retry = 0;
    hipError_t e = launch_resolve(s, p, n_slices, init_states, pl, w, codes, status, final_states, kMaxStretch, nullptr, nullptr, stride, false,
                                  &retry);
    if (e != hipSuccess || !retry) return e;
    return k1p_second_pass(s, p, n_slices, init_states, n_states, pl, w, codes, nullptr, nullptr, nullptr, status, final_states, false);
}
hipError_t launch_k1p8(hipStream_t s, const uint8_t *recs8, const uint64_t *rec_off, const uint32_t *n_bins,
                       uint32_t n_slices, const uint8_t *init_states, uint32_t n_states, const avr_chunk_plan *pl,
                       void *workspace, uint8_t *out, const uint64_t *out_off, uint32_t *out_len, int32_t *status,
                       uint8_t *final_states) {
    if (n_slices == 0) return hipSuccess;
    uint8_t *w = static_cast<uint8_t *>(workspace);
    uint8_t *res = w;                                        w += up256(codes_bytes(pl));
    const Plan p{nullptr, rec_off, n_bins, pl->res_off, pl->chunk_base, pl->chunk_slice, pl->blk_base, pl->blk_slice,
                 pl->dig_off, n_states, n_states, nullptr, nullptr, recs8};
    const Stretch *st = nullptr;
    hipError_t e = launch_resolve(s, p, n_slices, init_states, pl, w, res, status, final_states, kMaxStretch, &st, nullptr, 1, false,
                                  nullptr, true, true);
    if (e != hipSuccess) return e;
    w += resolve_ws_bytes(n_slices, n_states, pl);
    e = launch_code(s, p, n_slices, pl, w, res, kMaxStretch, out, out_off, out_len, status, st, true);
    if (e != hipSuccess || test_hooks().k1p_keep_retry) return e;
    hipLaunchKernelGGL(k_cabac_encode_codes<true>, dim3((n_slices + 63) / 64), dim3(64), 0, s, res, nullptr, pl->chunk_base, n_bins,
                       nullptr, n_slices, out, out_off, out_len, status, int32_t(AVR_SLICE_RETRY_SERIAL));
    return hipGetLastError();
}

size_t k1p_code_workspace_bytes(size_t n_slices, const avr_chunk_plan *pl) {
    return size_t(up256(uint64_t(pl->total_chunks) * sizeof(Stretch)) + up256(uint64_t(pl->total_chunks) * sizeof(Entry)) +
                  up256(n_slices * sizeof(SliceTotals)) + up256(pl->dig_total * 4 + 16) + up256(tile_codes_bytes(pl->total_chunks)));
}
hipError_t launch_k1p_code(hipStream_t s, const uint8_t *codes, const uint32_t *n_bins, uint32_t n_slices,
                           const avr_chunk_plan *pl, void *workspace, uint8_t *out, const uint64_t *out_off,
                           uint32_t *out_len, int32_t *status) {
    if (n_slices == 0) return hipSuccess;
    const Plan p{nullptr, nullptr, n_bins, pl->res_off, pl->chunk_base, pl->chunk_slice, pl->blk_base, pl->blk_slice,
                 pl->dig_off, 0, 0, nullptr, nullptr};
    hipError_t e = launch_code(s, p, n_slices, pl, static_cast<uint8_t *>(workspace), codes, 0xffffffffu, out, out_off, out_len, status);
    if (e != hipSuccess || test_hooks().k1p_keep_retry) return e;
    return launch_cabac_encode_codes(s, codes, pl->res_off, n_bins, nullptr, n_slices, out, out_off, out_len, status,
                                     AVR_SLICE_RETRY_SERIAL);
}

}
```

avrecode-ms_amd/device.py:

```python
from __future__ import annotations

import ctypes

from . import EST_KEYS, KIND_CABAC, KIND_CABAC8, KIND_RANGE, KIND_RANGE_KEYS, MAX_STATES8, NOP_CABAC, NOP_RANGE, AvrError, SynthConfig, _check, lib


def synth_config(workload: int, scale_permille: int = 1000, first_slice: int = 0) -> SynthConfig:
    cfg = SynthConfig()
    _check(lib().avr_synth_config_init(ctypes.byref(cfg), workload, scale_permille, first_slice))
    return cfg


def _stream_ptr(torch):
    return ctypes.c_void_p(torch.cuda.current_stream().cuda_stream)


def plan_tiles(n_bins, records_per_chunk=8):
    import torch
    n = n_bins.numel()
    order = torch.argsort(n_bins.to(torch.int64), descending=True, stable=True)
    chunks = (n_bins.to(torch.int64)[order] + records_per_chunk - 1) // records_per_chunk
    tile_max = chunks[::64]
    tile_off = torch.zeros(tile_max.numel() + 1, dtype=torch.int64, device=n_bins.device)
    tile_off[1:] = torch.cumsum(tile_max * 64, 0)
# ... 259 lines not shown
                rec_off.data_ptr() + 8 * a, self.n_bins.data_ptr() + 4 * a, p["n"], self.init_states.data_ptr() + ns * a,
                ctypes.addressof(p["plan"]), (p["ws"].data_ptr() + 255) // 256 * 256, p["ws_bytes"],
                self.out_off.data_ptr() + 8 * a, self.out_len.data_ptr() + 4 * a, self.status.data_ptr() + 4 * a,
                (self.final_states.data_ptr() + ns * a) if self.final_states is not None else None,
                rows_hint, self._part_counts.data_ptr() + 8 * i)
        return arr

    def settle(self):
        import torch
        if self._counts is None or self._hinted_path is None:
            return {"rows": 0, "hint": 0, "redone": False}
        if self._hinted_path == "parts":
            used, redone = self.rows_hint, False
            rows = max(int(self._part_counts[2 * i]) for i in range(self.n_parts))
            if used and rows > used:
                self.status.copy_(self._status_before)
                self.rows_hint = 0
                self.encode_chunked()
                torch.cuda.synchronize(self.n_bins.device)
                rows, redone = max(int(self._part_counts[2 * i]) for i in range(self.n_parts)), True
            recs, rec_off = self._slice_major()
            for i, p in enumerate(self._parts):
                if int(self._part_counts[2 * i + 1]):
                    q = self._part_args[i]
                    _check(lib().avr_cabac_encode_chunked_second_pass_device(
                        self.device_index, _stream_ptr(torch), recs.data_ptr(), q.rec_off, q.n_bins, q.n_slices, q.init_states,
                        self.n_states, q.plan, q.workspace, q.workspace_bytes, self.out.data_ptr(), q.out_off, q.out_len, q.status,
                        q.final_states))
                    redone = True
            if redone:
                torch.cuda.synchronize(self.n_bins.device)
            if rows:
                self.rows_hint = min(self.n_states, rows + 8)
            return {"rows": rows, "hint": used, "redone": redone, "parts": self.n_parts}
        rows, left, used = int(self._counts[0]), int(self._counts[1]), self.rows_hint
        redone = False
        if self._hinted_path == "chunked" and used and rows > used:
            self.status.copy_(self._status_before)
            self.rows_hint = 0
            self.encode_chunked()
            torch.cuda.synchronize(self.n_bins.device)
            rows, left, redone = int(self._counts[0]), int(self._counts[1]), True
        if self._hinted_path == "chunked" and left:
            recs, rec_off = self._slice_major()
            p = self._chunk_plan()
            ws_ptr = (p["ws"].data_ptr() + 255) // 256 * 256
            _check(lib().avr_cabac_encode_chunked_second_pass_device(
                self.device_index, _stream_ptr(torch), recs.data_ptr(), rec_off.data_ptr(), self.n_bins.data_ptr(),
                self.n_slices, self.init_states.data_ptr(), self.n_states, ctypes.byref(p["plan"]), ws_ptr, p["ws_bytes"],
                self.out.data_ptr(), self.out_off.data_ptr(), self.out_len.data_ptr(), self.status.data_ptr(),
                self.final_states.data_ptr() if self.final_states is not None else None))
            torch.cuda.synchronize(self.n_bins.device)
            redone = True
        if rows:
            self.rows_hint = min(self.n_states, rows + 8)
        return {"rows": rows, "hint": used, "redone": redone}

    def densify(self):
        import numpy as np
        import torch
        if self.kind != KIND_CABAC or getattr(self, "dense_index", None) is not None:
            return self
        L = lib()
        dev = self.n_bins.device
        sp = _stream_ptr(torch)
        bitmap = torch.zeros(32, dtype=torch.int32, device=dev)
        n_tile_recs = self.tiles.numel() // 2
        _check(L.avr_context_census_device(self.device_index, sp, self.tiles.data_ptr(), n_tile_recs, bitmap.data_ptr()))
        bits = np.unpackbits(bitmap.cpu().numpy().view(np.uint8), bitorder="little")[:1024]
        used = np.nonzero(bits)[0].astype(np.uint16)
        used = used[used < self.n_states] if self.n_states else used
        table = np.zeros(1024, dtype=np.uint16)
        table[used] = np.arange(used.size, dtype=np.uint16)
        d_table = torch.from_numpy(table.view(np.int16)).to(dev)
        d_index = torch.from_numpy(used.view(np.int16)).to(dev)
        _check(L.avr_context_remap_device(self.device_index, sp, self.tiles.data_ptr(), n_tile_recs, d_table.data_ptr()))
        if getattr(self, "rec_flat", None) is not None:
            _check(L.avr_context_remap_device(self.device_index, sp, self.rec_flat.data_ptr(),
                                              int(self.rec_off[-1]), d_table.data_ptr()))
        n_dense = max(int(used.size), 1)
        dense_init = torch.zeros(self.n_slices * n_dense, dtype=torch.uint8, device=dev)
        _check(L.avr_states_permute_device(self.device_index, sp, self.init_states.data_ptr(), self.n_states,
                                           dense_init.data_ptr(), n_dense, d_index.data_ptr(), int(used.size), self.n_slices, 0))
        torch.cuda.synchronize(dev)
        self.full_n_states, self.full_init_states = self.n_states, self.init_states
        self.dense_index, self.init_states, self.n_states = d_index, dense_init, n_dense
        self.final_states = torch.empty(self.n_slices * n_dense, dtype=torch.uint8, device=dev)
        self._plan = None
# ... 2 lines not shown
    def final_states_full(self):
        import torch
        if getattr(self, "dense_index", None) is None:
            return self.final_states
        full = self.full_init_states.clone()
        _check(lib().avr_states_permute_device(self.device_index, _stream_ptr(torch), self.final_states.data_ptr(), self.n_states,
                                               full.data_ptr(), self.full_n_states, self.dense_index.data_ptr(),
                                               self.dense_index.numel(), self.n_slices, 1))
        return full

    def _slice_major(self):
        import torch
        if self.kind == KIND_CABAC8:
            return self.rec8_flat, self.rec8_off
        if getattr(self, "rec_flat", None) is None:
            dev = self.n_bins.device
            nb = self.n_bins.to(torch.int64)
            self.rec_off = torch.cat([torch.zeros(1, dtype=torch.int64, device=dev), torch.cumsum((nb + 7) // 8 * 8, 0)])
            self.rec_flat = torch.empty(int(self.rec_off[-1]) + 8, dtype=torch.int16, device=dev)
            _check(lib().avr_synth_generate_slices_device(
                self.device_index, _stream_ptr(torch), ctypes.byref(self.cfg), self.kind, self.n_slices,
                self.rec_off.data_ptr(), self.rec_flat.data_ptr(), None))
            if getattr(self, "dense_index", None) is not None:
                import numpy as np
                table = np.zeros(1024, dtype=np.uint16)
                idx = self.dense_index.cpu().numpy().view(np.uint16)
                table[idx] = np.arange(idx.size, dtype=np.uint16)
                d_table = torch.from_numpy(table.view(np.int16)).to(dev)
                _check(lib().avr_context_remap_device(self.device_index, _stream_ptr(torch), self.rec_flat.data_ptr(),
                                                      int(self.rec_off[-1]), d_table.data_ptr()))
                torch.cuda.synchronize(dev)
        return self.rec_flat, self.rec_off

    def _plan_of(self, a, b):
        import torch
        from . import CHUNK_BINS, SORT_BLOCK_BINS, ChunkPlan
        dev = self.n_bins.device
        nb = self.n_bins[a:b].to(torch.int64)
        zero = torch.zeros(1, dtype=torch.int64, device=dev)
        ar = torch.arange(b - a, device=dev)
        res_off = torch.cat([zero, torch.cumsum((nb + 15) // 16 * 16 + 16, 0)])
        n_chunks = torch.clamp((nb + CHUNK_BINS - 1) // CHUNK_BINS, min=1)
        n_blocks = torch.clamp((nb + SORT_BLOCK_BINS - 1) // SORT_BLOCK_BINS, min=1)
        chunk_base = torch.cat([zero, torch.cumsum(n_chunks, 0)]).to(torch.int32)
        blk_base = torch.cat([zero, torch.cumsum(n_blocks, 0)]).to(torch.int32)
        dig_off = torch.cat([zero, torch.cumsum(nb // 2 + 8, 0)])
        t = dict(res_off=res_off, chunk_base=chunk_base, blk_base=blk_base, dig_off=dig_off,
                 chunk_slice=torch.repeat_interleave(ar, n_chunks).to(torch.int32),
                 blk_slice=torch.repeat_interleave(ar, n_blocks).to(torch.int32))
        plan = ChunkPlan(t["res_off"].data_ptr(), t["chunk_base"].data_ptr(), t["chunk_slice"].data_ptr(),
                         t["blk_base"].data_ptr(), t["blk_slice"].data_ptr(), t["dig_off"].data_ptr(),
                         int(res_off[-1]), int(dig_off[-1]), int(chunk_base[-1]), int(blk_base[-1]))
        p = dict(tensors=t, plan=plan, first=a, n=b - a)
        if self.kind == KIND_CABAC:
            ws_bytes = lib().avr_cabac_chunked_workspace_bytes(b - a, self.n_states, ctypes.byref(plan))
            p.update(ws_bytes=ws_bytes, ws=torch.empty(ws_bytes + 256, dtype=torch.uint8, device=dev))
        return p

    def set_parts(self, n_parts, weights=None):
        import torch
        from . import CHUNK_BINS, MAX_PARTS
        nb = self.n_bins.to(torch.int64)
        chunks = torch.clamp((nb + CHUNK_BINS - 1) // CHUNK_BINS, min=1)
        total = int(chunks.sum())
        if n_parts == 0:
            waves = (total + 63) // 64
            n_parts = 2 if (waves >= 2048 and self.n_slices >= 64) else 1
        n_parts = max(1, min(int(n_parts), MAX_PARTS, self.n_slices))
        self._parts = None
        self.n_parts = n_parts
        if n_parts > 1 and self.kind == KIND_CABAC and self._counts is not None:
            csum = torch.cumsum(chunks, 0).cpu().numpy()
            import numpy as np
            share = np.cumsum(np.asarray(weights if weights else [1.0] * n_parts, dtype=np.float64))
            share = share / share[-1]
            cuts = [0] + [int(np.searchsorted(csum, total * share[i])) + 1 for i in range(n_parts - 1)] + [self.n_slices]
            cuts = sorted(set(min(max(c, 0), self.n_slices) for c in cuts))
            self._parts = [self._plan_of(a, b) for a, b in zip(cuts[:-1], cuts[1:]) if b > a]
            self.n_parts = len(self._parts)
            self._part_counts = torch.zeros(2 * self.n_parts, dtype=torch.int32).pin_memory()
        return self.n_parts

    def _chunk_plan(self):
        import torch
        from . import CHUNK_BINS, SORT_BLOCK_BINS, ChunkPlan
        if getattr(self, "_plan", None) is None:
            dev = self.n_bins.device
            nb = self.n_bins.to(torch.int64)
            zero = torch.zeros(1, dtype=torch.int64, device=dev)
            ar = torch.arange(self.n_slices, device=dev)
            res_off = torch.cat([zero, torch.cumsum((nb + 15) // 16 * 16 + 16, 0)])
            n_chunks = torch.clamp((nb + CHUNK_BINS - 1) // CHUNK_BINS, min=1)
            n_blocks = torch.clamp((nb + SORT_BLOCK_BINS - 1) // SORT_BLOCK_BINS, min=1)
            chunk_base = torch.cat([zero, torch.cumsum(n_chunks, 0)]).to(torch.int32)
            blk_base = torch.cat([zero, torch.cumsum(n_blocks, 0)]).to(torch.int32)
            dig_off = torch.cat([zero, torch.cumsum(nb // 2 + 8, 0)])
            t = dict(res_off=res_off, chunk_base=chunk_base, blk_base=blk_base, dig_off=dig_off,
                     chunk_slice=torch.repeat_interleave(ar, n_chunks).to(torch.int32),
                     blk_slice=torch.repeat_interleave(ar, n_blocks).to(torch.int32))
            plan = ChunkPlan(t["res_off"].data_ptr(), t["chunk_base"].data_ptr(), t["chunk_slice"].data_ptr(),
                             t["blk_base"].data_ptr(), t["blk_slice"].data_ptr(), t["dig_off"].data_ptr(),
                             int(res_off[-1]), int(dig_off[-1]), int(chunk_base[-1]), int(blk_base[-1]))
            self._plan = dict(tensors=t, plan=plan)
            if self.kind in (KIND_CABAC, KIND_CABAC8):
                ws_of = lib().avr_cabac8_chunked_workspace_bytes if self.kind == KIND_CABAC8 else lib().avr_cabac_chunked_workspace_bytes
                ws_bytes = ws_of(self.n_slices, self.n_states, ctypes.byref(plan))
                self._plan.update(ws_bytes=ws_bytes, ws=torch.empty(ws_bytes + 256, dtype=torch.uint8, device=dev))
        return self._plan

    def encode_chunked(self):
        import torch
        recs, rec_off = self._slice_major()
        p = self._chunk_plan()
        if self.kind == KIND_CABAC8:
            _check(lib().avr_cabac8_encode_chunked_device(
                self.device_index, _stream_ptr(torch), recs.data_ptr(), rec_off.data_ptr(), self.n_bins.data_ptr(),
                self.n_slices, self.init_states.data_ptr(), self.n_states, ctypes.byref(p["plan"]), (p["ws"].data_ptr() + 255) // 256 * 256,
                p["ws_bytes"], self.out.data_ptr(), self.out_off.data_ptr(), self.out_len.data_ptr(), self.status.data_ptr(),
                self.final_states.data_ptr()))
            return
        if self.kind != KIND_CABAC:
            L = lib()
            out_total = int(self.out_off[-1].item()) if "out_total" not in p else p["out_total"]
            p["out_total"] = out_total
            if "ws_k2" not in p:
                n = L.avr_range_chunked_workspace_bytes(self.n_slices, ctypes.byref(p["plan"]), out_total)
                p["ws_k2"] = torch.empty(n + 256, dtype=torch.uint8, device=self.n_bins.device)
                p["ws_k2_bytes"] = n
            ws_ptr = (p["ws_k2"].data_ptr() + 255) // 256 * 256
            _check(L.avr_range_encode_chunked_device(
                self.device_index, _stream_ptr(torch), recs.data_ptr(), rec_off.data_ptr(), self.n_bins.data_ptr(), self.n_slices,
                ctypes.byref(p["plan"]), ws_ptr, p["ws_k2_bytes"], self.out.data_ptr(), self.out_off.data_ptr(), out_total,
                self.out_len.data_ptr(), self.status.data_ptr()))
            return
        ws_ptr = (p["ws"].data_ptr() + 255) // 256 * 256
# ... 95 lines not shown
```

include/avrecode_ms_amd.h:

```cpp
#ifndef AVRECODE_MS_AMD_H
#define AVRECODE_MS_AMD_H

#include <stddef.h>
#include <stdint.h>

#ifdef __cplusplus
extern "C" {
#endif

#define AVR_OK              0
#define AVR_ERR_INVALID    -1
#define AVR_ERR_NO_DEVICE  -2
#define AVR_ERR_HIP        -3
#define AVR_ERR_NOMEM      -4
#define AVR_ERR_CAPACITY   -5

#define AVR_SLICE_OK          0
#define AVR_SLICE_ZERO_PROB   1
#define AVR_SLICE_OVERFLOW    2
#define AVR_SLICE_BAD_RECORD  3

#define AVR_SEL_BYPASS     1024
#define AVR_SEL_TERMINATE  1025
#define AVR_MAX_STATES     1024
// ... 62 lines not shown
                          const uint32_t *order, size_t n_slices,
                          const uint64_t *tile_off, void *tiles, int32_t *status);

int avr_pack_tiles8_device(int device, void *stream, size_t n_states,
                           const uint8_t *recs8, const uint64_t *rec_off, const uint32_t *n_bins,
                           const uint32_t *order, size_t n_slices,
                           const uint64_t *tile_off, void *tiles, int32_t *status);

int avr_cabac_encode_tiles_device(int device, void *stream,
                                  const void *tiles, const uint64_t *tile_off,
                                  const uint32_t *n_bins, const uint32_t *order, size_t n_slices,
                                  const uint8_t *init_states, size_t n_states,
                                  uint8_t *out, const uint64_t *out_off,
                                  uint32_t *out_len, int32_t *status, uint8_t *final_states);

int avr_pack_tiles8_narrow_device(int device, void *stream, size_t n_states,
                                  const uint8_t *recs8, const uint64_t *rec_off, const uint32_t *n_bins,
                                  const uint32_t *order, size_t n_slices,
                                  const uint64_t *tile_off, void *tiles, int32_t *status);
int avr_cabac8_encode_tiles_device(int device, void *stream,
                                   const void *tiles, const uint64_t *tile_off,
                                   const uint32_t *n_bins, const uint32_t *order, size_t n_slices,
                                   const uint8_t *init_states, size_t n_states,
                                   uint8_t *out, const uint64_t *out_off,
                                   uint32_t *out_len, int32_t *status, uint8_t *final_states);

int avr_range_encode_tiles_device(int device, void *stream,
                                  const void *tiles, const uint64_t *tile_off,
                                  const uint32_t *n_bins, const uint32_t *order, size_t n_slices,
                                  uint8_t *out, const uint64_t *out_off,
                                  uint32_t *out_len, int32_t *status);

#define AVR_CHUNK_BINS       1024
#define AVR_SORT_BLOCK_BINS  4096
typedef struct {
    const uint64_t *res_off;
    const uint32_t *chunk_base;
    const uint32_t *chunk_slice;
    const uint32_t *blk_base;
    const uint32_t *blk_slice;
    const uint64_t *dig_off;
    uint64_t res_total;
    uint64_t dig_total;
    uint32_t total_chunks;
    uint32_t total_blocks;
} avr_chunk_plan;

size_t avr_cabac_chunked_workspace_bytes(size_t n_slices, size_t n_states, const avr_chunk_plan *plan);
int avr_cabac_encode_chunked_device(int device, void *stream,
                                    const uint16_t *recs, const uint64_t *rec_off,
                                    const uint32_t *n_bins, size_t n_slices,
                                    const uint8_t *init_states, size_t n_states,
                                    const avr_chunk_plan *plan, void *workspace, size_t workspace_bytes,
                                    uint8_t *out, const uint64_t *out_off,
                                    uint32_t *out_len, int32_t *status, uint8_t *final_states);

size_t avr_cabac8_chunked_workspace_bytes(size_t n_slices, size_t n_states, const avr_chunk_plan *plan);
int avr_cabac8_encode_chunked_device(int device, void *stream,
                                     const uint8_t *recs8, const uint64_t *rec_off,
                                     const uint32_t *n_bins, size_t n_slices,
                                     const uint8_t *init_states, size_t n_states,
                                     const avr_chunk_plan *plan, void *workspace, size_t workspace_bytes,
                                     uint8_t *out, const uint64_t *out_off,
                                     uint32_t *out_len, int32_t *status, uint8_t *final_states);

int avr_cabac_encode_tiles_device_hinted(int device, void *stream,
                                         const void *tiles, const uint64_t *tile_off,
                                         const uint32_t *n_bins, const uint32_t *order, size_t n_slices,
                                         const uint8_t *init_states, size_t n_states,
                                         uint8_t *out, const uint64_t *out_off,
                                         uint32_t *out_len, int32_t *status, uint8_t *final_states,
                                         uint32_t rows_hint, uint32_t *counts);
int avr_cabac_encode_chunked_device_hinted(int device, void *stream,
                                           const uint16_t *recs, const uint64_t *rec_off,
                                           const uint32_t *n_bins, size_t n_slices,
                                           const uint8_t *init_states, size_t n_states,
                                           const avr_chunk_plan *plan, void *workspace, size_t workspace_bytes,
                                           uint8_t *out, const uint64_t *out_off,
                                           uint32_t *out_len, int32_t *status, uint8_t *final_states,
// ... 105 lines not shown
```

Measured before the change: 24.85 billion.

## Pick per-batch CABAC chunk length from a cost model of device wave slots

Makes the chunk length of the chunked CABAC path variable: a multiple of 64 between 512 and 1024, chosen by a host cost model that weighs local and replay wave counts against device wave-slot capacity and the longest per-slice chunk chain. The kernels now index tiles with a reciprocal-multiply division instead of a fixed shift, and grouped 64-byte loads are issued through a single load64 helper. Shorter chunks are meant to fill more wave slots when the batch under-occupies the GPU. The cost is more chunk boundaries, extra index arithmetic in the hot load path, and replanning when the row hint changes.

```diff
diff --git a/avrecode-ms_amd/__init__.py b/avrecode-ms_amd/__init__.py
--- a/avrecode-ms_amd/__init__.py
+++ b/avrecode-ms_amd/__init__.py
@@ -21,6 +21,7 @@
 SLICE_OK, SLICE_ZERO_PROB, SLICE_OVERFLOW, SLICE_BAD_RECORD = 0, 1, 2, 3
 NOP_CABAC, NOP_RANGE = 1026 << 1, 0
 CHUNK_BINS, SORT_BLOCK_BINS = 1024, 4096
+CHUNK_BINS_MIN, CHUNK_BINS_STEP = 512, 64
 
 _SOURCES = ["avr_kernels.hip", "avr_k1p.hip", "avr_k2p.hip", "avr_est.hip", "avr_api.cpp"]
 _DEPS = _SOURCES + ["avr_coder.h", "avr_est.h", "avr_div.h", "avr_internal.h", "avr_k1p.h", "avr_k2p.h", "avr_synth.h", "avr_tables.h"]
@@ -87,7 +88,7 @@
 class ChunkPlan(ctypes.Structure):
     _fields_ = [("res_off", c_void_p), ("chunk_base", c_void_p), ("chunk_slice", c_void_p), ("blk_base", c_void_p),
                 ("blk_slice", c_void_p), ("dig_off", c_void_p), ("res_total", c_uint64), ("dig_total", c_uint64),
-                ("total_chunks", c_uint32), ("total_blocks", c_uint32)]
+                ("total_chunks", c_uint32), ("total_blocks", c_uint32), ("chunk_bins", c_uint32)]
 
 
 class ChunkedPart(ctypes.Structure):
@@ -158,6 +159,7 @@
                                                c_void_p, c_size_t, c_void_p, c_void_p, c_void_p, c_void_p, c_void_p]),
     "avr_range_encode_tiles_device": (c_int, [c_int, c_void_p, c_void_p, c_void_p, c_void_p, c_void_p, c_size_t,
                                               c_void_p, c_void_p, c_void_p, c_void_p]),
+    "avr_cabac_chunk_bins": (c_uint32, [c_int, c_void_p, c_size_t, c_size_t, c_int, c_void_p]),
     "avr_cabac_chunked_workspace_bytes": (c_size_t, [c_size_t, c_size_t, c_void_p]),
     "avr_cabac_encode_chunked_device": (c_int, [c_int, c_void_p, c_void_p, c_void_p, c_void_p, c_size_t, c_void_p, c_size_t,
                                                 c_void_p, c_void_p, c_size_t, c_void_p, c_void_p, c_void_p, c_void_p,
diff --git a/avrecode-ms_amd/csrc/avr_api.cpp b/avrecode-ms_amd/csrc/avr_api.cpp
--- a/avrecode-ms_amd/csrc/avr_api.cpp
+++ b/avrecode-ms_amd/csrc/avr_api.cpp
@@ -194,6 +194,7 @@
     else if (!strcmp(name, "local_waves")) h.local_waves = value;
     else if (!strcmp(name, "k2p_wave")) h.k2p_wave = value;
     else if (!strcmp(name, "k1p_keep_retry")) h.k1p_keep_retry = value;
+    else if (!strcmp(name, "chunk_bins")) h.chunk_bins = value;
     else if (!strcmp(name, "k1_waves")) h.k1_waves = value;
     else if (!strcmp(name, "k1_fwd")) h.k1_fwd = value;
     else if (!strcmp(name, "k1_words8")) h.k1_words8 = value;
@@ -529,7 +530,7 @@
     if (cabac && ((rc = b->d_states.reserve(n * std::max<size_t>(ns, 1))) || (rc = b->d_final.reserve(n * std::max<size_t>(ns, 1))) ||
                   (rc = b->h_final.reserve(n * std::max<size_t>(ns, 1)))))
         return rc;
-    const size_t n_chunks_max = size_t(b->total_bins / AVR_CHUNK_BINS) + n + 1, n_blks_max = size_t(b->total_bins / AVR_SORT_BLOCK_BINS) + n + 1;
+    const size_t n_chunks_max = size_t(b->total_bins / AVR_CHUNK_BINS_MIN) + n + 1, n_blks_max = size_t(b->total_bins / AVR_SORT_BLOCK_BINS) + n + 1;
     const size_t n_groups = b->group_first.size();
     if ((rc = b->h_plan.reserve(64 * 16 + (n + 1) * 64 + (n_tiles + 1) * 8 + (chunked ? (n_chunks_max + n_blks_max) * 4 : 0) +
                                 (b->keys ? (n_chunks_max + n + n_groups + 3) * 4 + 256 : 0)))) return rc;
@@ -577,11 +578,13 @@
     } else if (chunked) {
         std::vector<uint64_t> res_off(n + 1, 0), dig_off(n + 1, 0);
         std::vector<uint32_t> chunk_base(n + 1, 0), blk_base(n + 1, 0), chunk_slice, blk_slice;
+        uint32_t chunk_bins = avr_cabac_chunk_bins(b->device, b->n_bins.data(), n, b->recs8 || !hint.rows ? ns : hint.rows, b->recs8 ? 1 : 2, nullptr);
+        if (!chunk_bins) chunk_bins = AVR_CHUNK_BINS;
         for (size_t i = 0; i < n; i++) {
             const uint64_t nb = b->n_bins[i];
             res_off[i + 1] = res_off[i] + ((nb + 15) & ~uint64_t(15)) + 16;
             dig_off[i + 1] = dig_off[i] + nb / 2 + 8;
-            const uint32_t nc = uint32_t(std::max<uint64_t>(1, (nb + AVR_CHUNK_BINS - 1) / AVR_CHUNK_BINS));
+            const uint32_t nc = uint32_t(std::max<uint64_t>(1, (nb + chunk_bins - 1) / chunk_bins));
             const uint32_t nk = uint32_t(std::max<uint64_t>(1, (nb + AVR_SORT_BLOCK_BINS - 1) / AVR_SORT_BLOCK_BINS));
             chunk_base[i + 1] = chunk_base[i] + nc;
             blk_base[i + 1] = blk_base[i] + nk;
@@ -593,7 +596,7 @@
             (rc = b->d_blk_slice.reserve(blk_slice.size())))
             return rc;
         avr_chunk_plan plan{b->d_res_off.p, b->d_chunk_base.p, b->d_chunk_slice.p, b->d_blk_base.p, b->d_blk_slice.p, b->d_dig_off.p,
-                            res_off.back(), dig_off.back(), chunk_base.back(), blk_base.back()};
+                            res_off.back(), dig_off.back(), chunk_base.back(), blk_base.back(), chunk_bins};
         const size_t ws = avr::k1p_workspace_bytes(n, uint32_t(ns), &plan);
         if ((rc = b->d_workspace.reserve(ws + 256))) return rc;
         b->plan = plan;
@@ -989,8 +992,42 @@
     return AVR_OK;
 }
 
+static bool chunk_bins_ok(const avr_chunk_plan *plan, bool any_length) {
+    const uint32_t v = plan->chunk_bins;
+    if (v == 0 || v == AVR_CHUNK_BINS) return true;
+    return any_length && v >= AVR_CHUNK_BINS_MIN && v < AVR_CHUNK_BINS && v % AVR_CHUNK_BINS_STEP == 0;
+}
+static int check_chunk_bins(const avr_chunk_plan *plan, bool any_length) {
+    if (plan && !chunk_bins_ok(plan, any_length))
+        return any_length ? fail(AVR_ERR_INVALID, "plan.chunk_bins %u: 0, or a multiple of %d in [%d, %d]", plan->chunk_bins, AVR_CHUNK_BINS_STEP,
+                                 AVR_CHUNK_BINS_MIN, AVR_CHUNK_BINS)
+                          : fail(AVR_ERR_INVALID, "plan.chunk_bins %u: this entry takes 0 or %d only", plan->chunk_bins, AVR_CHUNK_BINS);
+    return AVR_OK;
+}
+
+uint32_t avr_cabac_chunk_bins(int device, const uint32_t *n_bins, size_t n_slices, size_t n_states, int record_width, uint32_t *wave_slots) {
+    if (wave_slots) wave_slots[0] = wave_slots[1] = 0;
+    if ((n_slices && !n_bins) || (record_width != 1 && record_width != 2) || n_states > (record_width == 1 ? AVR_MAX_STATES8 : AVR_MAX_STATES)) {
+        fail(AVR_ERR_INVALID, "avr_cabac_chunk_bins: null n_bins, a record width other than 1 or 2, or too many states");
+        return 0;
+    }
+    if (device >= 0 && select_device(device)) return 0;
+    uint32_t slots[2];
+    if (avr::k1p_wave_slots(device, uint32_t(n_states), record_width == 1, slots) != hipSuccess) {
+        fail(AVR_ERR_HIP, "avr_cabac_chunk_bins: the device's wave slots");
+        return 0;
+    }
+    if (wave_slots) { wave_slots[0] = slots[0]; wave_slots[1] = slots[1]; }
+    if (const uint32_t forced = avr::test_hooks().chunk_bins) {
+        const avr_chunk_plan probe{nullptr, nullptr, nullptr, nullptr, nullptr, nullptr, 0, 0, 0, 0, forced};
+        if (check_chunk_bins(&probe, true)) return 0;
+        return forced;
+    }
+    return avr::k1p_pick_chunk_bins(n_bins, n_slices, slots);
+}
+
 size_t avr_cabac_chunked_workspace_bytes(size_t n_slices, size_t n_states, const avr_chunk_plan *plan) {
-    if (!plan || n_states > AVR_MAX_STATES) return 0;
+    if (!plan || n_states > AVR_MAX_STATES || !chunk_bins_ok(plan, true)) return 0;
     return avr::k1p_workspace_bytes(n_slices, uint32_t(n_states), plan);
 }
 
@@ -1003,6 +1040,7 @@
     if (!plan || (n_slices && (!plan->res_off || !plan->chunk_base || !plan->chunk_slice || !plan->blk_base || !plan->blk_slice ||
                                !plan->dig_off || !workspace || !status)))
         return fail(AVR_ERR_INVALID, "null plan pointer");
+    if (int rc = check_chunk_bins(plan, true)) return rc;
     if (workspace_bytes < avr::k1p_workspace_bytes(n_slices, uint32_t(n_states), plan))
         return fail(AVR_ERR_CAPACITY, "workspace of %zu bytes is smaller than avr_cabac_chunked_workspace_bytes()", workspace_bytes);
     if (int rc = select_device(device)) return rc;
@@ -1012,7 +1050,7 @@
 }
 
 size_t avr_cabac8_chunked_workspace_bytes(size_t n_slices, size_t n_states, const avr_chunk_plan *plan) {
-    if (!plan || n_states > AVR_MAX_STATES8) return 0;
+    if (!plan || n_states > AVR_MAX_STATES8 || !chunk_bins_ok(plan, true)) return 0;
     return avr::k1p_workspace_bytes(n_slices, uint32_t(n_states), plan);
 }
 
@@ -1025,6 +1063,7 @@
     if (n_slices && (!recs8 || !out || !out_len || (n_states && !init_states))) return fail(AVR_ERR_INVALID, "null device pointer");
     if (!plan || (n_slices && (!plan->res_off || !plan->chunk_base || !plan->chunk_slice || !plan->dig_off || !workspace || !status)))
         return fail(AVR_ERR_INVALID, "null plan pointer");
+    if (int rc = check_chunk_bins(plan, true)) return rc;
     if (workspace_bytes < avr::k1p_workspace_bytes(n_slices, uint32_t(n_states), plan))
         return fail(AVR_ERR_CAPACITY, "workspace of %zu bytes is smaller than avr_cabac8_chunked_workspace_bytes()", workspace_bytes);
     if (int rc = select_device(device)) return rc;
@@ -1040,6 +1079,7 @@
     if (!plan || (n_slices && (!plan->res_off || !plan->chunk_base || !plan->chunk_slice || !plan->blk_base || !plan->blk_slice ||
                                !plan->dig_off || !workspace || !status)))
         return fail(AVR_ERR_INVALID, "null plan pointer");
+    if (int rc = check_chunk_bins(plan, true)) return rc;
     if (workspace_bytes < avr::k1p_workspace_bytes(n_slices, uint32_t(n_states), plan))
         return fail(AVR_ERR_CAPACITY, "workspace of %zu bytes is smaller than avr_cabac_chunked_workspace_bytes()", workspace_bytes);
     return AVR_OK;
@@ -1164,7 +1204,7 @@
 }
 
 size_t avr_range_chunked_workspace_bytes(size_t n_slices, const avr_chunk_plan *plan, uint64_t out_total) {
-    if (!plan) return 0;
+    if (!plan || !chunk_bins_ok(plan, false)) return 0;
     return avr::k2p_workspace_bytes(n_slices, plan->total_chunks, out_total);
 }
 
@@ -1174,6 +1214,7 @@
     if (int rc = check_common(rec_off, n_bins, out_off, n_slices)) return rc;
     if (!plan || (n_slices && (!plan->chunk_base || !plan->chunk_slice || !workspace || !status || !out || !out_len)))
         return fail(AVR_ERR_INVALID, "null plan / workspace / output pointer");
+    if (int rc = check_chunk_bins(plan, false)) return rc;
     if (workspace_bytes < avr::k2p_workspace_bytes(n_slices, plan->total_chunks, out_total))
         return fail(AVR_ERR_CAPACITY, "workspace of %zu bytes is smaller than avr_range_chunked_workspace_bytes()", workspace_bytes);
     if (int rc = select_device(device)) return rc;
@@ -1183,7 +1224,7 @@
 }
 
 size_t avr_range_resolve_workspace_bytes(size_t n_slices, size_t n_groups, const avr_chunk_plan *plan) {
-    if (!plan) return 0;
+    if (!plan || !chunk_bins_ok(plan, false)) return 0;
     return avr::est_workspace_bytes(n_slices, n_groups, plan->total_chunks);
 }
 
@@ -1196,6 +1237,7 @@
         return fail(AVR_ERR_INVALID, "n_groups %zu: a batch of %zu slices has between 1 and %zu groups", n_groups, n_slices, n_slices);
     if (n_slices && (!group_first || !recs_out || !status)) return fail(AVR_ERR_INVALID, "null device pointer");
     if (!plan || (n_slices && (!plan->chunk_base || !plan->chunk_slice))) return fail(AVR_ERR_INVALID, "null plan pointer");
+    if (int rc = check_chunk_bins(plan, false)) return rc;
     if (n_slices && !workspace) return fail(AVR_ERR_INVALID, "null workspace");
     if (workspace_bytes < avr::est_workspace_bytes(n_slices, n_groups, plan->total_chunks))
         return fail(AVR_ERR_INVALID, "workspace of %zu bytes is smaller than avr_range_resolve_workspace_bytes()", workspace_bytes);
@@ -1216,11 +1258,11 @@
     if (!plan || (n_slices && (!plan->res_off || !plan->chunk_base || !plan->chunk_slice || !plan->dig_off ||
                                (need_blocks && (!plan->blk_base || !plan->blk_slice)))))
         return fail(AVR_ERR_INVALID, "null plan pointer");
-    return AVR_OK;
+    return check_chunk_bins(plan, true);
 }
 
 size_t avr_cabac_resolve_workspace_bytes(size_t n_slices, size_t n_states, const avr_chunk_plan *plan) {
-    if (!plan || n_states > AVR_MAX_STATES) return 0;
+    if (!plan || n_states > AVR_MAX_STATES || !chunk_bins_ok(plan, true)) return 0;
     return avr::k1p_resolve_workspace_bytes(n_slices, uint32_t(n_states), plan);
 }
 
@@ -1240,7 +1282,7 @@
 }
 
 size_t avr_cabac_resolved_workspace_bytes(size_t n_slices, const avr_chunk_plan *plan) {
-    return plan ? avr::k1p_code_workspace_bytes(n_slices, plan) : 0;
+    return plan && chunk_bins_ok(plan, true) ? avr::k1p_code_workspace_bytes(n_slices, plan) : 0;
 }
 
 int avr_cabac_encode_resolved_device(int device, void *stream, const uint8_t *codes, const uint32_t *n_bins, size_t n_slices,
diff --git a/avrecode-ms_amd/csrc/avr_internal.h b/avrecode-ms_amd/csrc/avr_internal.h
--- a/avrecode-ms_amd/csrc/avr_internal.h
+++ b/avrecode-ms_amd/csrc/avr_internal.h
@@ -30,6 +30,7 @@
     uint32_t k1_words8;
     uint32_t k1_waves;
     uint32_t k2p_wave;
+    uint32_t chunk_bins;
     uint32_t k1p_keep_retry;
 };
 #ifdef AVR_TEST_HOOKS
@@ -81,6 +82,8 @@
 hipError_t launch_compact(hipStream_t s, const uint8_t *out, const uint64_t *out_off, const uint32_t *out_len,
                           const uint64_t *dense_off, uint32_t n_slices, uint8_t *dense);
 
+hipError_t k1p_wave_slots(int device, uint32_t n_states, bool r8, uint32_t slots[2]);
+uint32_t k1p_pick_chunk_bins(const uint32_t *n_bins, size_t n_slices, const uint32_t slots[2]);
 size_t k1p_workspace_bytes(size_t n_slices, uint32_t n_states, const avr_chunk_plan *pl);
 hipError_t launch_k1p(hipStream_t s, const uint16_t *recs, const uint64_t *rec_off, const uint32_t *n_bins,
                       uint32_t n_slices, const uint8_t *init_states, uint32_t n_states, const avr_chunk_plan *pl,
diff --git a/avrecode-ms_amd/csrc/avr_k1p.h b/avrecode-ms_amd/csrc/avr_k1p.h
--- a/avrecode-ms_amd/csrc/avr_k1p.h
+++ b/avrecode-ms_amd/csrc/avr_k1p.h
@@ -17,6 +17,7 @@
 #endif
 
 constexpr uint32_t kChunk = 1024;
+constexpr uint32_t kChunkMin = 512, kChunkStep = 64;
 constexpr uint32_t kNone = 0xffffffffu;
 constexpr uint32_t kMaxStretch = 16 * kChunk;
 constexpr uint32_t kCodeBypass = 252;
@@ -104,6 +105,10 @@
 struct LinearCodes {
     const uint8_t *p;
     AVR_HD U4 load16(uint32_t i) const { return *reinterpret_cast<const U4 *>(p + i); }
+    AVR_HD void load64(uint32_t i, U4 &a, U4 &b, U4 &c, U4 &d) const {
+        const U4 *q = reinterpret_cast<const U4 *>(p + i);
+        a = q[0]; b = q[1]; c = q[2]; d = q[3];
+    }
     AVR_HD uint32_t byte(uint32_t i) const { return p[i]; }
 };
 
@@ -171,8 +176,8 @@
 }
 
 AVR_HD void b1_stretch(const uint8_t *res, uint32_t n, uint32_t chunk, const CodeEntry *codes, uint32_t max_stretch,
-                       Stretch *o) {
-    const uint32_t lo = chunk * kChunk, limit = lo + kChunk;
+                       Stretch *o, uint32_t chunk_bins = kChunk) {
+    const uint32_t lo = chunk * chunk_bins, limit = lo + chunk_bins;
     uint32_t R[4], T[4] = {0, 0, 0, 0};
     uint32_t i;
     o->too_long = 0;
@@ -354,11 +359,11 @@
         uint32_t base = head_end;
         for (; (base & 63) && base + 16 <= to; base += 16) group16(src.load16(base));
         U4 v0{0, 0, 0, 0}, v1 = v0, v2 = v0, v3 = v0;
-        if (base + 64 <= to) { v0 = src.load16(base); v1 = src.load16(base + 16); v2 = src.load16(base + 32); v3 = src.load16(base + 48); }
+        if (base + 64 <= to) src.load64(base, v0, v1, v2, v3);
         for (; base + 64 <= to; base += 64) {
             const uint32_t w[16] = {v0.x, v0.y, v0.z, v0.w, v1.x, v1.y, v1.z, v1.w, v2.x, v2.y, v2.z, v2.w, v3.x, v3.y, v3.z, v3.w};
             const uint32_t nb = base + 128 <= to ? base + 64 : base;
-            v0 = src.load16(nb); v1 = src.load16(nb + 16); v2 = src.load16(nb + 32); v3 = src.load16(nb + 48);
+            src.load64(nb, v0, v1, v2, v3);
 #if defined(__HIP_DEVICE_COMPILE__)
 #pragma unroll 4
 #endif
diff --git a/avrecode-ms_amd/csrc/avr_k1p.hip b/avrecode-ms_amd/csrc/avr_k1p.hip
--- a/avrecode-ms_amd/csrc/avr_k1p.hip
+++ b/avrecode-ms_amd/csrc/avr_k1p.hip
@@ -31,17 +31,31 @@
     const uint16_t *table;
     const uint16_t *index;
     const uint8_t *recs8;
+    uint32_t chunk_bins;
+    uint32_t chunk_rcp;
 };
+static inline Plan with_chunk_bins(Plan p, const avr_chunk_plan *pl) {
+    p.chunk_bins = pl->chunk_bins ? pl->chunk_bins : kChunk;
+    const uint64_t k = p.chunk_bins / kChunkStep;
+    p.chunk_rcp = uint32_t(((uint64_t(1) << 32) + k - 1) / k);
+    return p;
+}
+__device__ __forceinline__ uint32_t chunk_div(uint32_t i, uint32_t chunk_rcp) { return __umulhi(i >> 6, chunk_rcp); }
 constexpr uint32_t kNotUsed = 0xffffu;
 
 struct TileCodes {
     const uint8_t *base;
-    uint32_t chunk0;
+    uint32_t chunk0, chunk_bins, chunk_rcp;
     __device__ __forceinline__ size_t at(uint32_t i) const {
-        const uint32_t gc = chunk0 + (i >> 10), g = (i >> 4) & 63u;
+        const uint32_t c = chunk_div(i, chunk_rcp), gc = chunk0 + c, g = (i - c * chunk_bins) >> 4;
         return ((size_t(gc >> 6) * 64 + g) * 64 + (gc & 63u)) * 16;
     }
     __device__ __forceinline__ U4 load16(uint32_t i) const { return *reinterpret_cast<const U4 *>(base + at(i)); }
+    __device__ __forceinline__ void load64(uint32_t i, U4 &a, U4 &b, U4 &c, U4 &d) const {
+        const uint8_t *q = base + at(i);
+        a = *reinterpret_cast<const U4 *>(q); b = *reinterpret_cast<const U4 *>(q + 1024);
+        c = *reinterpret_cast<const U4 *>(q + 2048); d = *reinterpret_cast<const U4 *>(q + 3072);
+    }
     __device__ __forceinline__ uint32_t byte(uint32_t i) const { return base[at(i) + (i & 15u)]; }
 };
 __host__ __device__ inline uint64_t tile_codes_bytes(uint32_t total_chunks) { return (uint64_t(total_chunks) + 63) / 64 * 64 * 1024; }
@@ -194,8 +208,8 @@
         if (status[s] == AVR_SLICE_OK) {
             mine = true;
             n = p.n_bins[s];
-            i0 = (gc - p.chunk_base[s]) * kChunk;
-            i1 = i0 + kChunk < n ? i0 + kChunk : n;
+            i0 = (gc - p.chunk_base[s]) * p.chunk_bins;
+            i1 = i0 + p.chunk_bins < n ? i0 + p.chunk_bins : n;
             if (i0 > i1) i0 = i1;
             if (R8) {
                 const uint64_t off = p.rec_off[s];
@@ -341,7 +355,7 @@
     const uint32_t col = p.index ? p.index[k] : k, row4 = ((nk + 3) >> 2) << 2;
     if (col >= p.ns_full) return;
     uint32_t st = init_states[size_t(s) * p.ns_full + col] & 127u;
-    const uint32_t c0 = p.chunk_base[s], nc = (p.n_bins[s] + kChunk - 1) / kChunk;
+    const uint32_t c0 = p.chunk_base[s], nc = chunk_div(p.n_bins[s] + p.chunk_bins - 1, p.chunk_rcp);
     const uint16_t *le = lend + size_t(c0) * nk + k;
     const uint32_t *bw_ahead = lbits + size_t(c0) * 32;
     const uint32_t *bw_cur = bw_ahead;
@@ -470,7 +484,7 @@
     if (s >= n_slices || status[s] != AVR_SLICE_OK) return false;
     const uint32_t col = p.index ? p.index[k] : k;
     if (col >= p.ns_full) return false;
-    const uint32_t nc = (p.n_bins[s] + kChunk - 1) / kChunk, seg_len = (nc + n_segs - 1) / n_segs;
+    const uint32_t nc = chunk_div(p.n_bins[s] + p.chunk_bins - 1, p.chunk_rcp), seg_len = (nc + n_segs - 1) / n_segs;
     const uint32_t c_begin = seg * seg_len < nc ? seg * seg_len : nc, c_end = c_begin + seg_len < nc ? c_begin + seg_len : nc;
     *o = ChainLane{s, k, seg, c_begin, c_end, nc, col};
     return true;
@@ -619,8 +633,9 @@
     bool merged;
     Stretch o;
 
-    __device__ __forceinline__ void init(uint32_t chunk, uint32_t i0_, uint32_t i1_, uint32_t n_, uint32_t max_stretch_, const uint2 *codes2_) {
-        i0 = i0_; i1 = i1_; limit = i0_ + kChunk; n = n_; max_stretch = max_stretch_; codes2 = codes2_;
+    __device__ __forceinline__ void init(uint32_t chunk, uint32_t i0_, uint32_t i1_, uint32_t n_, uint32_t max_stretch_, const uint2 *codes2_,
+                                         uint32_t chunk_bins) {
+        i0 = i0_; i1 = i1_; limit = i0_ + chunk_bins; n = n_; max_stretch = max_stretch_; codes2 = codes2_;
         mode = 0; Rp0 = Rp1 = 0x01fe01feu; Tp0 = Tp1 = 0; T[0] = T[1] = T[2] = T[3] = 0; Rm = 510; Tm = 0; end = 0;
         merged = false;
         o.first = kNone; o.end = 0; o.exit_q = 0; o.too_long = 0; o.pad[0] = o.pad[1] = 0;
@@ -749,8 +764,8 @@
     for (int q = 0; q < 4; q++) { o.t_exit[q] = 0; o.r_exit[q] = 0; }
     if (status[s] != AVR_SLICE_OK) { stretch[gc] = o; return; }
     const uint32_t c = gc - p.chunk_base[s];
-    const uint32_t n = p.n_bins[s], i0 = c * kChunk;
-    const uint32_t i1 = i0 + kChunk < n ? i0 + kChunk : n;
+    const uint32_t n = p.n_bins[s], i0 = c * p.chunk_bins;
+    const uint32_t i1 = i0 + p.chunk_bins < n ? i0 + p.chunk_bins : n;
     {
         const uint32_t nkw = (nk + 3) >> 2;
         const uint32_t *e = est + size_t(gc) * nkw;
@@ -766,7 +781,7 @@
         else *reinterpret_cast<U4 *>(ro + i) = v;
     };
     B1Walk b1;
-    b1.init(c, i0, i1, n, max_stretch, codes2);
+    b1.init(c, i0, i1, n, max_stretch, codes2, p.chunk_bins);
     auto eight = [&](const U4 &v, uint32_t &c0, uint32_t &c1, uint4 e[8]) {
         const uint32_t w[4] = {v.x, v.y, v.z, v.w};
         uint32_t off[8];
@@ -815,7 +830,7 @@
         if (i0 < n) {
             for_record_groups8(r8, i0, i1, sixteen8);
             b1.chunk_done();
-            for (uint32_t i = i0 + kChunk; b1.mode != 3 && i < n; i += 8) {
+            for (uint32_t i = i0 + p.chunk_bins; b1.mode != 3 && i < n; i += 8) {
                 const uint2 v = *reinterpret_cast<const uint2 *>(r8 + i);
                 uint32_t c0, c1;
                 uint4 e[8];
@@ -858,7 +873,7 @@
             put16(i, a);
         }
         b1.chunk_done();
-        for (i = i0 + kChunk; b1.mode != 3 && i < n; i += 8) {
+        for (i = i0 + p.chunk_bins; b1.mode != 3 && i < n; i += 8) {
             uint32_t c0, c1;
             uint4 e[8];
             eight(*reinterpret_cast<const U4 *>(r + i), c0, c1, e);
@@ -899,11 +914,11 @@
     if (gc >= total_chunks) return;
     const uint32_t slice = p.chunk_slice[gc];
     if (status[slice] != AVR_SLICE_OK) { st[gc].first = kNone; st[gc].too_long = 0; return; }
-    const uint32_t c = gc - p.chunk_base[slice], n = p.n_bins[slice], i0 = c * kChunk;
-    const uint32_t i1 = i0 + kChunk < n ? i0 + kChunk : n;
+    const uint32_t c = gc - p.chunk_base[slice], n = p.n_bins[slice], i0 = c * p.chunk_bins;
+    const uint32_t i1 = i0 + p.chunk_bins < n ? i0 + p.chunk_bins : n;
     const uint8_t *r = res + p.res_off[slice];
     B1Walk b1;
-    b1.init(c, i0, i1, n, max_stretch, codes2);
+    b1.init(c, i0, i1, n, max_stretch, codes2, p.chunk_bins);
     auto eight = [&](uint32_t lo, uint32_t hi, uint4 e[8]) {
 #pragma unroll
         for (uint32_t j = 0; j < 8; j++) e[j] = cinfo[((j < 4 ? lo : hi) >> (8 * (j & 3))) & 0xffu];
@@ -927,7 +942,7 @@
         }
         for (; i < i1; i += 16) sixteen(i, *reinterpret_cast<const U4 *>(r + i));
         b1.chunk_done();
-        for (i = i0 + kChunk; b1.mode != 3 && i < n; i += 16) {
+        for (i = i0 + p.chunk_bins; b1.mode != 3 && i < n; i += 16) {
             const U4 v = *reinterpret_cast<const U4 *>(r + i);
             uint4 e[8];
             eight(v.x, v.y, e); b1.tail(i, e);
@@ -1082,7 +1097,7 @@
     DeviceAdder add;
     add.S = S + p.dig_off[slice];
     add.ring = ring + (threadIdx.x >> 6) * (kRing * 64) + (threadIdx.x & 63u);
-    if (TILE_CODES) c_stretch_in(TileCodes{res, p.chunk_base[slice]}, o, en[gc], gc - p.chunk_base[slice], codes, add);
+    if (TILE_CODES) c_stretch_in(TileCodes{res, p.chunk_base[slice], p.chunk_bins, p.chunk_rcp}, o, en[gc], gc - p.chunk_base[slice], codes, add);
     else c_stretch(res + p.res_off[slice], o, en[gc], gc - p.chunk_base[slice], codes, add);
 }
 
@@ -1173,7 +1188,7 @@
 __global__ __launch_bounds__(64) void k_cabac_encode_codes(const uint8_t *codes_in, const uint64_t *res_off, const uint32_t *chunk_base,
                                                            const uint32_t *n_bins, const uint32_t *order, uint32_t n_slices, uint8_t *out,
                                                            const uint64_t *out_off, uint32_t *out_len, int32_t *status,
-                                                           int32_t want_status) {
+                                                           int32_t want_status, uint32_t chunk_bins, uint32_t chunk_rcp) {
     __shared__ CodeEntry codes[256];
     for (uint32_t c = threadIdx.x; c < 256; c += 64) codes[c] = device_code_entry(c);
     __syncthreads();
@@ -1186,7 +1201,7 @@
     }
     const uint32_t n = n_bins[slice];
     const uint8_t *res = TILE ? codes_in : codes_in + res_off[slice];
-    const TileCodes tiled{codes_in, TILE ? chunk_base[slice] : 0u};
+    const TileCodes tiled{codes_in, TILE ? chunk_base[slice] : 0u, chunk_bins, chunk_rcp};
     auto load16 = [&](uint32_t i) { return TILE ? tiled.load16(i) : *reinterpret_cast<const U4 *>(res + i); };
     auto byte = [&](uint32_t i) { return TILE ? tiled.byte(i) : uint32_t(res[i]); };
     const uint64_t o0 = out_off[slice];
@@ -1268,6 +1283,32 @@
     }
     *out = x.p;
     return hipStreamWaitEvent(s, x.ready, 0);
+}
+
+struct LocalShape { uint32_t per_wave, fixed, waves, resident; bool narrow; };
+static inline LocalShape local_shape(uint32_t n_states, bool r8) {
+    LocalShape o;
+    o.per_wave = (33 + (n_states + 5) / 2) * 64 * 4;
+    o.narrow = n_states <= 500;
+    const uint32_t kLdsPerCu = 160 * 1024;
+    o.fixed = r8 ? 128 * 2 : o.narrow ? 2048 * 2 : 2048 * 4;
+    o.waves = 1; o.resident = 0;
+    for (uint32_t w = 1; w <= 8; w++) {
+        const uint32_t need = w * o.per_wave + o.fixed;
+        if (need > kLdsPerCu) break;
+        const uint32_t resident = kLdsPerCu / need * w;
+        if (resident > o.resident) { o.resident = resident; o.waves = w; }
+    }
+    return o;
+}
+struct ReplayShape { uint32_t waves, lds; };
+static inline ReplayShape replay_shape(uint32_t n_states) {
+    const uint32_t per_wave = ((n_states + 8) / 4) * 256;
+    const uint32_t waves = per_wave * 4 <= 48 * 1024 ? 4 : per_wave * 2 <= 48 * 1024 ? 2 : 1;
+    return ReplayShape{waves, waves * per_wave};
+}
+template <bool R8> static inline auto replay_kernel(bool tile_codes) {
+    return R8 ? k_k1p_replay<true, true> : tile_codes ? k_k1p_replay<true, false> : k_k1p_replay<false, false>;
 }
 
 static hipError_t launch_resolve(hipStream_t s, Plan p, uint32_t n_slices, const uint8_t *init_states,
@@ -1314,17 +1355,11 @@
     }
     p.n_states = n_states;
     {
-        const uint32_t per_wave = (33 + (n_states + 5) / 2) * 64 * 4;
-        const bool narrow = n_states <= 500;
-        const uint32_t kLdsPerCu = 160 * 1024, kStatic = r8 ? 128 * 2 : narrow ? 2048 * 2 : 2048 * 4;
+        const LocalShape shape = local_shape(n_states, r8);
+        const uint32_t per_wave = shape.per_wave;
+        const bool narrow = shape.narrow;
         auto local = r8 ? k_k1p_local<uint16_t, true> : narrow ? k_k1p_local<uint16_t, false> : k_k1p_local<uint32_t, false>;
-        uint32_t waves = 1, best = 0;
-        for (uint32_t w = 1; w <= 8; w++) {
-            const uint32_t need = w * per_wave + kStatic;
-            if (need > kLdsPerCu) break;
-            const uint32_t resident = kLdsPerCu / need * w;
-            if (resident > best) { best = resident; waves = w; }
-        }
+        uint32_t waves = shape.waves;
         if (const uint32_t v = test_hooks().local_waves) waves = v;
         uint32_t lds = waves * per_wave;
         if (lds > 60 * 1024) {
@@ -1374,10 +1409,9 @@
             hipLaunchKernelGGL(k_k1p_ctxchain, whole, block, 0, s, p, n_slices, groups, chain_lanes, status, tn, lbits, lend, init_states, est, final_states);
         }
     }
-    const uint32_t per_wave = ((n_states + 8) / 4) * 256;
-    const uint32_t replay_waves = per_wave * 4 <= 48 * 1024 ? 4 : per_wave * 2 <= 48 * 1024 ? 2 : 1;
-    const uint32_t replay_lds = replay_waves * per_wave;
-    auto replay = r8 ? k_k1p_replay<true, true> : tile_codes ? k_k1p_replay<true, false> : k_k1p_replay<false, false>;
+    const ReplayShape rshape = replay_shape(n_states);
+    const uint32_t replay_waves = rshape.waves, replay_lds = rshape.lds;
+    auto replay = r8 ? replay_kernel<true>(true) : replay_kernel<false>(tile_codes);
     if (replay_lds > 48 * 1024) {
         e = hipFuncSetAttribute(reinterpret_cast<const void *>(replay), hipFuncAttributeMaxDynamicSharedMemorySize, int(replay_lds));
         if (e != hipSuccess) return e;
@@ -1420,7 +1454,7 @@
                                      uint32_t *out_len, int32_t *status, int32_t want_status) {
     if (n_slices == 0) return hipSuccess;
     hipLaunchKernelGGL(k_cabac_encode_codes<false>, dim3((n_slices + 63) / 64), dim3(64), 0, s, codes, res_off, nullptr, n_bins, order,
-                       n_slices, out, out_off, out_len, status, want_status);
+                       n_slices, out, out_off, out_len, status, want_status, 0u, 0u);
     return hipGetLastError();
 }
 
@@ -1478,8 +1512,8 @@
     if (n_slices == 0) return hipSuccess;
     uint8_t *w = static_cast<uint8_t *>(workspace);
     uint8_t *res = w;                                        w += up256(codes_bytes(pl));
-    const Plan p{recs, rec_off, n_bins, pl->res_off, pl->chunk_base, pl->chunk_slice, pl->blk_base, pl->blk_slice,
-                 pl->dig_off, 0, n_states, nullptr, nullptr};
+    const Plan p = with_chunk_bins(Plan{recs, rec_off, n_bins, pl->res_off, pl->chunk_base, pl->chunk_slice, pl->blk_base, pl->blk_slice,
+                                        pl->dig_off, 0, n_states, nullptr, nullptr, nullptr, 0, 0}, pl);
     const uint32_t stride = census_stride();
     uint32_t retry = 0;
     if (hint && hint->host_retry) *hint->host_retry = 0;
@@ -1496,8 +1530,8 @@
     if (n_slices == 0) return hipSuccess;
     uint8_t *w = static_cast<uint8_t *>(workspace);
     uint8_t *res = w;                                        w += up256(codes_bytes(pl));
-    const Plan p{recs, rec_off, n_bins, pl->res_off, pl->chunk_base, pl->chunk_slice, pl->blk_base, pl->blk_slice,
-                 pl->dig_off, 0, n_states, nullptr, nullptr};
+    const Plan p = with_chunk_bins(Plan{recs, rec_off, n_bins, pl->res_off, pl->chunk_base, pl->chunk_slice, pl->blk_base, pl->blk_slice,
+                                        pl->dig_off, 0, n_states, nullptr, nullptr, nullptr, 0, 0}, pl);
     return k1p_second_pass(s, p, n_slices, init_states, n_states, pl, w, res, out, out_off, out_len, status, final_states, true);
 }
 
@@ -1508,8 +1542,8 @@
                               uint32_t n_slices, const uint8_t *init_states, uint32_t n_states, const avr_chunk_plan *pl,
                               void *workspace, uint8_t *codes, int32_t *status, uint8_t *final_states) {
     if (n_slices == 0) return hipSuccess;
-    const Plan p{recs, rec_off, n_bins, pl->res_off, pl->chunk_base, pl->chunk_slice, pl->blk_base, pl->blk_slice,
-                 pl->dig_off, 0, n_states, nullptr, nullptr};
+    const Plan p = with_chunk_bins(Plan{recs, rec_off, n_bins, pl->res_off, pl->chunk_base, pl->chunk_slice, pl->blk_base, pl->blk_slice,
+                                        pl->dig_off, 0, n_states, nullptr, nullptr, nullptr, 0, 0}, pl);
     uint8_t *w = static_cast<uint8_t *>(workspace);
     const uint32_t stride = census_stride();
     uint32_t retry = 0;
@@ -1525,8 +1559,8 @@
     if (n_slices == 0) return hipSuccess;
     uint8_t *w = static_cast<uint8_t *>(workspace);
     uint8_t *res = w;                                        w += up256(codes_bytes(pl));
-    const Plan p{nullptr, rec_off, n_bins, pl->res_off, pl->chunk_base, pl->chunk_slice, pl->blk_base, pl->blk_slice,
-                 pl->dig_off, n_states, n_states, nullptr, nullptr, recs8};
+    const Plan p = with_chunk_bins(Plan{nullptr, rec_off, n_bins, pl->res_off, pl->chunk_base, pl->chunk_slice, pl->blk_base, pl->blk_slice,
+                                        pl->dig_off, n_states, n_states, nullptr, nullptr, recs8, 0, 0}, pl);
     const Stretch *st = nullptr;
     hipError_t e = launch_resolve(s, p, n_slices, init_states, pl, w, res, status, final_states, kMaxStretch, &st, nullptr, 1, false,
                                   nullptr, true, true);
@@ -1535,7 +1569,7 @@
     e = launch_code(s, p, n_slices, pl, w, res, kMaxStretch, out, out_off, out_len, status, st, true);
     if (e != hipSuccess || test_hooks().k1p_keep_retry) return e;
     hipLaunchKernelGGL(k_cabac_encode_codes<true>, dim3((n_slices + 63) / 64), dim3(64), 0, s, res, nullptr, pl->chunk_base, n_bins,
-                       nullptr, n_slices, out, out_off, out_len, status, int32_t(AVR_SLICE_RETRY_SERIAL));
+                       nullptr, n_slices, out, out_off, out_len, status, int32_t(AVR_SLICE_RETRY_SERIAL), p.chunk_bins, p.chunk_rcp);
     return hipGetLastError();
 }
 
@@ -1547,12 +1581,60 @@
                            const avr_chunk_plan *pl, void *workspace, uint8_t *out, const uint64_t *out_off,
                            uint32_t *out_len, int32_t *status) {
     if (n_slices == 0) return hipSuccess;
-    const Plan p{nullptr, nullptr, n_bins, pl->res_off, pl->chunk_base, pl->chunk_slice, pl->blk_base, pl->blk_slice,
-                 pl->dig_off, 0, 0, nullptr, nullptr};
+    const Plan p = with_chunk_bins(Plan{nullptr, nullptr, n_bins, pl->res_off, pl->chunk_base, pl->chunk_slice, pl->blk_base, pl->blk_slice,
+                                        pl->dig_off, 0, 0, nullptr, nullptr, nullptr, 0, 0}, pl);
     hipError_t e = launch_code(s, p, n_slices, pl, static_cast<uint8_t *>(workspace), codes, 0xffffffffu, out, out_off, out_len, status);
     if (e != hipSuccess || test_hooks().k1p_keep_retry) return e;
     return launch_cabac_encode_codes(s, codes, pl->res_off, n_bins, nullptr, n_slices, out, out_off, out_len, status,
                                      AVR_SLICE_RETRY_SERIAL);
 }
 
-}
+
+constexpr uint32_t kModelCus = 256, kReplayWavesPerCuModel = 12;
+hipError_t k1p_wave_slots(int device, uint32_t n_states, bool r8, uint32_t slots[2]) {
+    uint32_t cus = kModelCus, replay_per_cu = kReplayWavesPerCuModel;
+    const ReplayShape rs = replay_shape(n_states);
+    if (device >= 0) {
+        int v = 0, blocks = 0;
+        if (hipDeviceGetAttribute(&v, hipDeviceAttributeMultiprocessorCount, device) == hipSuccess && v > 0) {
+            cus = uint32_t(v);
+            int cur = -1;
+            const void *fn = r8 ? reinterpret_cast<const void *>(replay_kernel<true>(true)) : reinterpret_cast<const void *>(replay_kernel<false>(true));
+            if (hipGetDevice(&cur) == hipSuccess && cur == device &&
+                hipOccupancyMaxActiveBlocksPerMultiprocessor(&blocks, fn, int(64 * rs.waves), rs.lds) == hipSuccess && blocks > 0)
+                replay_per_cu = uint32_t(blocks) * rs.waves;
+        }
+        (void)hipGetLastError();
+    }
+    slots[0] = cus * local_shape(n_states, r8).resident;
+    slots[1] = cus * replay_per_cu;
+    return hipSuccess;
+}
+
+constexpr double kLocalUs = 0.0375, kReplayUs = 0.0633;
+constexpr double kLocalFixed = 2540, kReplayFixed = 2176;
+constexpr double kChainUs = 0.19;
+constexpr double kMinGain = 0.04;
+constexpr uint32_t kRuleMinBins = 704;
+uint32_t k1p_pick_chunk_bins(const uint32_t *n_bins, size_t n_slices, const uint32_t slots[2]) {
+    if (!n_slices || !slots[0] || !slots[1]) return kChunk;
+    uint32_t best = kChunk;
+    double t_best = 0, t_full = 0;
+    for (uint32_t L = kChunk; L >= kRuleMinBins; L -= kChunkStep) {
+        uint64_t chunks = 0, longest = 0;
+        for (size_t i = 0; i < n_slices; i++) {
+            const uint64_t c = n_bins[i] ? (uint64_t(n_bins[i]) + L - 1) / L : 1;
+            chunks += c;
+            longest = c > longest ? c : longest;
+        }
+        const uint64_t waves = (chunks + 63) / 64;
+        if (L == kChunk && waves <= slots[0]) return kChunk;
+        const double t = kLocalUs * (L + kLocalFixed) * double((waves + slots[0] - 1) / slots[0]) +
+                         kReplayUs * (L + kReplayFixed) * double((waves + slots[1] - 1) / slots[1]) + kChainUs * double(longest);
+        if (L == kChunk) t_full = t_best = t;
+        else if (t < t_best) { t_best = t; best = L; }
+    }
+    return t_full - t_best >= kMinGain * t_full ? best : kChunk;
+}
+
+}
diff --git a/avrecode-ms_amd/device.py b/avrecode-ms_amd/device.py
--- a/avrecode-ms_amd/device.py
+++ b/avrecode-ms_amd/device.py
@@ -315,6 +315,7 @@
                 torch.cuda.synchronize(self.n_bins.device)
             if rows:
                 self.rows_hint = min(self.n_states, rows + 8)
+                self._replan()
             return {"rows": rows, "hint": used, "redone": redone, "parts": self.n_parts}
         rows, left, used = int(self._counts[0]), int(self._counts[1]), self.rows_hint
         redone = False
@@ -337,6 +338,7 @@
             redone = True
         if rows:
             self.rows_hint = min(self.n_states, rows + 8)
+            self._replan()
         return {"rows": rows, "hint": used, "redone": redone}
 
     def densify(self):
@@ -405,6 +407,35 @@
                 torch.cuda.synchronize(dev)
         return self.rec_flat, self.rec_off
 
+    def chunk_bins(self, force=None):
+        from . import CHUNK_BINS, CHUNK_BINS_MIN, CHUNK_BINS_STEP
+        if force is not None:
+            if not (CHUNK_BINS_MIN <= force <= CHUNK_BINS and force % CHUNK_BINS_STEP == 0):
+                raise AvrError(f"chunk_bins {force}: a multiple of {CHUNK_BINS_STEP} in [{CHUNK_BINS_MIN}, {CHUNK_BINS}]")
+            self._chunk_bins, self._plan, self._chunk_bins_forced = int(force), None, True
+            if getattr(self, "_parts_asked", None) is not None:
+                self.set_parts(*self._parts_asked)
+        if self.kind not in (KIND_CABAC, KIND_CABAC8):
+            return CHUNK_BINS
+        if getattr(self, "_chunk_bins", None) is None:
+            import numpy as np
+            nb = np.ascontiguousarray(self.n_bins.cpu().numpy()).view(np.uint32)
+            v = lib().avr_cabac_chunk_bins(self.device_index, nb.ctypes.data, self.n_slices, self.rows_hint or self.n_states,
+                                           1 if self.kind == KIND_CABAC8 else 2, None)
+            if v == 0:
+                raise AvrError(lib().avr_last_error().decode())
+            self._chunk_bins, self._planned_rows = int(v), self.rows_hint
+        return self._chunk_bins
+
+    def _replan(self):
+        if getattr(self, "_chunk_bins", None) is None or getattr(self, "_chunk_bins_forced", False) or self.rows_hint == getattr(self, "_planned_rows", None):
+            return
+        old, self._chunk_bins = self._chunk_bins, None
+        if self.chunk_bins() != old:
+            self._plan = None
+            if getattr(self, "_parts_asked", None) is not None:
+                self.set_parts(*self._parts_asked)
+
     def _plan_of(self, a, b):
         import torch
         from . import CHUNK_BINS, SORT_BLOCK_BINS, ChunkPlan
@@ -413,7 +444,8 @@
         zero = torch.zeros(1, dtype=torch.int64, device=dev)
         ar = torch.arange(b - a, device=dev)
         res_off = torch.cat([zero, torch.cumsum((nb + 15) // 16 * 16 + 16, 0)])
-        n_chunks = torch.clamp((nb + CHUNK_BINS - 1) // CHUNK_BINS, min=1)
+        chunk_bins = self.chunk_bins()
+        n_chunks = torch.clamp((nb + chunk_bins - 1) // chunk_bins, min=1)
         n_blocks = torch.clamp((nb + SORT_BLOCK_BINS - 1) // SORT_BLOCK_BINS, min=1)
         chunk_base = torch.cat([zero, torch.cumsum(n_chunks, 0)]).to(torch.int32)
         blk_base = torch.cat([zero, torch.cumsum(n_blocks, 0)]).to(torch.int32)
@@ -423,7 +455,7 @@
                  blk_slice=torch.repeat_interleave(ar, n_blocks).to(torch.int32))
         plan = ChunkPlan(t["res_off"].data_ptr(), t["chunk_base"].data_ptr(), t["chunk_slice"].data_ptr(),
                          t["blk_base"].data_ptr(), t["blk_slice"].data_ptr(), t["dig_off"].data_ptr(),
-                         int(res_off[-1]), int(dig_off[-1]), int(chunk_base[-1]), int(blk_base[-1]))
+                         int(res_off[-1]), int(dig_off[-1]), int(chunk_base[-1]), int(blk_base[-1]), chunk_bins)
         p = dict(tensors=t, plan=plan, first=a, n=b - a)
         if self.kind == KIND_CABAC:
             ws_bytes = lib().avr_cabac_chunked_workspace_bytes(b - a, self.n_states, ctypes.byref(plan))
@@ -432,9 +464,11 @@
 
     def set_parts(self, n_parts, weights=None):
         import torch
-        from . import CHUNK_BINS, MAX_PARTS
+        from . import MAX_PARTS
+        self._parts_asked = (n_parts, weights)
         nb = self.n_bins.to(torch.int64)
-        chunks = torch.clamp((nb + CHUNK_BINS - 1) // CHUNK_BINS, min=1)
+        chunk_bins = self.chunk_bins()
+        chunks = torch.clamp((nb + chunk_bins - 1) // chunk_bins, min=1)
         total = int(chunks.sum())
         if n_parts == 0:
             waves = (total + 63) // 64
@@ -463,7 +497,8 @@
             zero = torch.zeros(1, dtype=torch.int64, device=dev)
             ar = torch.arange(self.n_slices, device=dev)
             res_off = torch.cat([zero, torch.cumsum((nb + 15) // 16 * 16 + 16, 0)])
-            n_chunks = torch.clamp((nb + CHUNK_BINS - 1) // CHUNK_BINS, min=1)
+            chunk_bins = self.chunk_bins()
+            n_chunks = torch.clamp((nb + chunk_bins - 1) // chunk_bins, min=1)
             n_blocks = torch.clamp((nb + SORT_BLOCK_BINS - 1) // SORT_BLOCK_BINS, min=1)
             chunk_base = torch.cat([zero, torch.cumsum(n_chunks, 0)]).to(torch.int32)
             blk_base = torch.cat([zero, torch.cumsum(n_blocks, 0)]).to(torch.int32)
@@ -473,7 +508,7 @@
                      blk_slice=torch.repeat_interleave(ar, n_blocks).to(torch.int32))
             plan = ChunkPlan(t["res_off"].data_ptr(), t["chunk_base"].data_ptr(), t["chunk_slice"].data_ptr(),
                              t["blk_base"].data_ptr(), t["blk_slice"].data_ptr(), t["dig_off"].data_ptr(),
-                             int(res_off[-1]), int(dig_off[-1]), int(chunk_base[-1]), int(blk_base[-1]))
+                             int(res_off[-1]), int(dig_off[-1]), int(chunk_base[-1]), int(blk_base[-1]), chunk_bins)
             self._plan = dict(tensors=t, plan=plan)
             if self.kind in (KIND_CABAC, KIND_CABAC8):
                 ws_of = lib().avr_cabac8_chunked_workspace_bytes if self.kind == KIND_CABAC8 else lib().avr_cabac_chunked_workspace_bytes
diff --git a/include/avrecode_ms_amd.h b/include/avrecode_ms_amd.h
--- a/include/avrecode_ms_amd.h
+++ b/include/avrecode_ms_amd.h
@@ -118,6 +118,8 @@
                                   uint32_t *out_len, int32_t *status);
 
 #define AVR_CHUNK_BINS       1024
+#define AVR_CHUNK_BINS_MIN   512
+#define AVR_CHUNK_BINS_STEP  64
 #define AVR_SORT_BLOCK_BINS  4096
 typedef struct {
     const uint64_t *res_off;
@@ -130,7 +132,11 @@
     uint64_t dig_total;
     uint32_t total_chunks;
     uint32_t total_blocks;
+    uint32_t chunk_bins;
 } avr_chunk_plan;
+
+uint32_t avr_cabac_chunk_bins(int device, const uint32_t *n_bins, size_t n_slices, size_t n_states, int record_width,
+                              uint32_t *wave_slots);
 
 size_t avr_cabac_chunked_workspace_bytes(size_t n_slices, size_t n_states, const avr_chunk_plan *plan);
 int avr_cabac_encode_chunked_device(int device, void *stream,
```

Measured after the change: 24.86 billion, median of 3. About the same (+0.0%).
